# microsoft/GenerativeImage2Text

Hardware: AMD Instinct MI355X
Metric: captions/sec whole-node (GIT_BASE 224px bs=64/GPU greedy len=20) (higher is better)
Workload: dtype f16; 1 GPU; GIT_BASE 224px bs=64/GPU greedy max_len=20 frames=1; global_batch=64, parallelism=dp1, decode_steps_per_caption=19, seq_len_returned=20, hip_graph=True, contexts_in_flight=4, layernorm_folded=True, library=libgitmi_f16.so, encoder_chains=2, schedule=mixed

## Files before the change

### generativeimage2text_amd/csrc/abi_ops.hip

```cpp
#include "../../include/gitmi.h"
#include "abi_common.h"
#include "gitmi_common.h"
#include "launchers.h"

#include <hip/hip_runtime.h>

using namespace gitmi;

#ifdef GITMI_EXPERIMENT
#include "../../include/gitmi_experiment.h"
#define GITMI_EXP_EXPORT extern "C"
#else
#define GITMI_EXP_EXPORT [[maybe_unused]] static
#endif

static inline int round_up(int x, int m) { return (x + m - 1) / m * m; }

extern "C" int gitmi_operand_dtype(void);
static const char* dtype_name(int dtype) {
    return dtype == GITMI_DTYPE_F32 ? "fp32" : dtype == GITMI_DTYPE_BF16 ? "bf16" : dtype == GITMI_DTYPE_F16 ? "fp16" : "unknown";
}
static int check_dtype(const char* op, const char* arg, int dtype) {
    if (dtype == GITMI_DTYPE_F32 || dtype == gitmi_operand_dtype()) return 0;
    return fail("%s: %s is %s (%d), but this library's 16-bit operands are %s (libgitmi%s.so)", op, arg, dtype_name(dtype), dtype,
// ... 201 lines not shown

GITMI_EXP_EXPORT int gitmi_debug_gemm_form(const void* A, int lda, const void* W, const float* bias, const void* res, int ldr, void* C,
                                           int ldc, int M, int N, int K, int act, int in_dtype, int out_dtype, int shared,
                                           const float* ln_part, const float* colsum, float ln_eps, float* part_out,
                                           const float* res_part, const float* res_gamma, const float* res_beta, float res_eps,
                                           void* stream) {
    if (!A || !W || !C) return fail("debug_gemm_form: null argument (A, W, C)");
    if (M < 0 || N < 1 || K < 1) return fail("debug_gemm_form: M=%d N=%d K=%d", M, N, K);
    if (lda < K) return fail("debug_gemm_form: lda=%d < K=%d", lda, K);
    if (ldc < N) return fail("debug_gemm_form: ldc=%d < N=%d", ldc, N);
    if (res && ldr < N) return fail("debug_gemm_form: ldr=%d < N=%d", ldr, N);
    if (act < GITMI_ACT_NONE || act > GITMI_ACT_GELU_ERF) return fail("debug_gemm_form: act=%d", act);
    RCK(check_dtype("debug_gemm_form", "in_dtype", in_dtype));
    const bool in_f32 = in_dtype == GITMI_DTYPE_F32;
    if ((in_f32 && K % 16) || (!in_f32 && K % 64)) return fail("debug_gemm_form: K must be a multiple of %d (K=%d)", in_f32 ? 16 : 64, K);
    GemmArgs g{};
    g.A = A; g.W = W; g.bias = bias; g.res = (const float*)res; g.C = C;
    g.M = M; g.N = N; g.K = K; g.lda = lda; g.ldc = ldc; g.ldr = res ? ldr : 0; g.act = act;
    g.shared = shared ? 1 : 0;
    if (out_dtype == GITMI_DTYPE_F16_STREAM) {
        if (in_f32) return fail("debug_gemm_form: fp16 stream rows need 16-bit operands");
        g.out_f16 = 1;
    } else {
        RCK(check_dtype("debug_gemm_form", "out_dtype", out_dtype));
    }
    const bool out_f32 = out_dtype == GITMI_DTYPE_F32;
    const bool consumer = ln_part != nullptr, producer = part_out != nullptr || res_part != nullptr;
    if (colsum && !consumer) return fail("debug_gemm_form: colsum without ln_part");
    if ((res_gamma || res_beta) && !res_part) return fail("debug_gemm_form: res_gamma / res_beta without res_part");
    if (consumer || producer) {
#ifndef GITMI_OPS_F16
        return fail("debug_gemm_form: the folded-LayerNorm forms are built into the fp16-operand library only");
#endif
        if (consumer && producer) return fail("debug_gemm_form: consumer (ln_part) and producer (part_out / res_part) arguments in one launch");
        if (consumer) {
            if (!colsum) return fail("debug_gemm_form: ln_part without colsum");
            if (res || in_f32 || out_f32 || g.out_f16) return fail("debug_gemm_form: the consumer writes operand-type rows and takes no residual");
            if (K > 1024) return fail("debug_gemm_form: row partials cover K <= 1024 (K=%d)", K);
            g.ln_part = (const float2*)ln_part; g.ln_nparts = (K + 255) / 256; g.ln_colsum = colsum; g.ln_inv_d = 1.0f / (float)K; g.ln_eps = ln_eps;
        } else {
            if (!g.out_f16 || act != GITMI_ACT_NONE) return fail("debug_gemm_form: the producer writes fp16 stream rows and has no activation");
            if (N > 1024) return fail("debug_gemm_form: row partials cover N <= 1024 (N=%d)", N);
            g.part_out = (float2*)part_out;
            if (res_part) {
                if (!res || !res_gamma || !res_beta) return fail("debug_gemm_form: res_part without res / res_gamma / res_beta");
                g.res_part = (const float2*)res_part; g.res_nparts = (N + 255) / 256; g.res_gamma = res_gamma; g.res_beta = res_beta;
                g.res_inv_d = 1.0f / (float)N; g.res_eps = res_eps;
            }
        }
        if (!gemm_uses_p8(g, false, false))
            return fail("debug_gemm_form: the folded forms exist in gemm_p8_kernel only (more than 512 rows, N %% 256 == 0, K >= 128, 16-byte aligned rows)");
    }
    HIPCK(launch_gemm(g, in_f32, out_f32, (hipStream_t)stream));
    return 0;
}

extern "C" int gitmi_op_attn_decode(const void* qkv, const void* img_k, const void* img_v, void* txt_k, void* txt_v,
                                    const int* kv_src, void* out, int B, int H, int N_img, int T_max, int pos, int beams,
                                    int dtype, int dbg, void* stream) {
    RCK(check_dtype("op_attn_decode", "dtype", dtype));
    AttnDecodeArgs a{};
    a.qkv = qkv; a.img_k = img_k; a.img_v = img_v; a.txt_k = txt_k; a.txt_v = txt_v; a.out = out;
    a.kv_src = kv_src; a.ld_src = T_max; a.d = H * 64; a.N_img = N_img; a.T_max = T_max; a.pos = pos; a.beams = beams;
    a.scale = 0.125f; a.dbg = dbg & 0xffff; a.waves_per_pair = (dbg >> 16) & 3; a.stream_wgs = dbg >> 18;
    if (dtype == GITMI_DTYPE_F32) {
        HIPCK(launch_attn_decode(a, B, H, (hipStream_t)stream));
        return 0;
    }
    a.N_pad = round_up(N_img, 32);
    HIPCK(launch_attn_decode_mfma(a, B, H, (hipStream_t)stream));
    return 0;
}
extern "C" int gitmi_op_kv_repack(const void* qkv_rows, void* kf, void* vt, int B, int N, int H, void* stream) {
    HIPCK(launch_kv_repack_frag(qkv_rows, kf, vt, B, N, round_up(N, 32), H, H * 64, (hipStream_t)stream));
    return 0;
}

GITMI_EXP_EXPORT int gitmi_debug_attention_ragged(const void* qkv, void* out, const int* ntok, int B, int N, int H, int dtype, int impl,
                                                  void* stream) {
    if (!ntok) return fail("debug_attention_ragged: ntok is required");
    const size_t esz = dtype == GITMI_DTYPE_F32 ? 4 : 2;
    const int D = H * 64;
    AttnFullArgs a{};
    a.q = qkv;
    a.k = (const char*)qkv + (size_t)D * esz;
    a.v = (const char*)qkv + (size_t)2 * D * esz;
    a.out = out;
    a.ldq = a.ldk = a.ldv = 3 * D;
    a.ldo = D;
    a.N = N; a.H = H; a.scale = 0.125f; a.ntok = ntok;
    HIPCK(launch_attn_full(a, B, dtype == GITMI_DTYPE_F32, impl, (hipStream_t)stream));
    return 0;
}
GITMI_EXP_EXPORT int gitmi_debug_attn_decode_form(const void* qkv, const void* img_k, const void* img_v, void* txt_k, void* txt_v,
                                                  const int* kv_src, void* out, const int* ntok, const int* img_of, int n_images,
                                                  int B, int H, int N_img, int T_max, int pos, int beams, int dtype, int out_frag,
                                                  int pairs_per_wg, int waves_per_pair, int stream_wgs, void* stream) {
    RCK(check_dtype("debug_attn_decode_form", "dtype", dtype));
    if (!qkv || !img_k || !img_v || !txt_k || !txt_v || !kv_src || !out) return fail("debug_attn_decode_form: null argument");
    if (beams < 1 || beams > 8) return fail("debug_attn_decode_form: beams=%d outside [1, 8]", beams);
    if (n_images < 1) return fail("debug_attn_decode_form: n_images=%d", n_images);
    if (B < 1 || H < 1 || N_img < 1 || pos < 0 || pos >= T_max)
        return fail("debug_attn_decode_form: B=%d H=%d N_img=%d pos=%d T_max=%d", B, H, N_img, pos, T_max);
    if (out_frag && dtype == GITMI_DTYPE_F32) return fail("debug_attn_decode_form: out_frag needs 16-bit rows");
    if (ntok && stream_wgs > 0) return fail("debug_attn_decode_form: the streaming kernel does not serve ragged batches (ntok)");
    AttnDecodeArgs a{};
// ... 214 lines not shown
```

### generativeimage2text_amd/csrc/engine.hip

```cpp
#include "../../include/gitmi.h"
#include "engine_state.h"

#include <algorithm>
#include <cmath>
#include <cstdarg>
#include <cstdio>
#include <cstring>

using namespace gitmi;

#ifdef GITMI_EXPERIMENT
#include "../../include/gitmi_experiment.h"
#define GITMI_EXP_EXPORT extern "C"
#else
#define GITMI_EXP_EXPORT [[maybe_unused]] static
#endif

static thread_local char g_err[1024] = "";
int gitmi::fail(const char* fmt, ...) {
    va_list ap;
    va_start(ap, fmt);
    vsnprintf(g_err, sizeof(g_err), fmt, ap);
    va_end(ap);
    return 1;
// ... 10 lines not shown
struct SpanGuard {
    gitmi_engine* e; hipStream_t s; size_t idx; bool on;
    SpanGuard(gitmi_engine* e_, hipStream_t s_, int tag, double flops) : e(e_), s(s_), idx(0), on(e_->profiling) {
        if (!on) return;
        TimedSpan sp{get_event(e), get_event(e), tag, flops};
        hipEventRecord(sp.a, s);
        idx = e->spans.size();
        e->spans.push_back(sp);
    }
    ~SpanGuard() { if (on) hipEventRecord(e->spans[idx].b, s); }
};

static bool gemm_tall_tiles(const gitmi_engine* e, int N) {
    if (!e->pol.shared_device) return false;
    return e->pol.gemm_tall == 1 || (e->pol.gemm_tall == 2 && N >= 2048) || (e->pol.gemm_tall == 3 && N < 2048);
}

static double gemm_flops(int M, int N, int K) { return 2.0 * (double)M * (double)N * (double)K; }
static GemmArgs gemm_args(const void* A, int lda, const void* W, const float* bias, const void* res, int ldr, void* C, int ldc,
                          int M, int N, int K, int act) {
    GemmArgs g{};
    g.A = A; g.W = W; g.bias = bias; g.res = (const float*)res; g.C = C;
    g.M = M; g.N = N; g.K = K; g.lda = lda; g.ldc = ldc; g.ldr = ldr; g.act = act;
    return g;
}
static int gemm_run(gitmi_engine* e, hipStream_t s, GemmArgs g, bool in_f32, bool out_f32, int tag) {
    g.shared = gemm_tall_tiles(e, g.N) ? 1 : 0;
    SpanGuard sp(e, s, tag, gemm_flops(g.M, g.N, g.K));
    HIPCK(launch_gemm(g, in_f32, out_f32, s));
    return 0;
}
static int gemm(gitmi_engine* e, hipStream_t s, const void* A, int lda, const void* W, const float* bias,
                const float* res, int ldr, void* C, int ldc, bool out_f32, int M, int N, int K, int act, int tag) {
    return gemm_run(e, s, gemm_args(A, lda, W, bias, res, ldr, C, ldc, M, N, K, act), e->pol.f32, out_f32, tag);
}
static bool on_p8(const void* A, int lda, const void* W, const void* C, int ldc, int M, int N, int K, bool stream_out) {
    GemmArgs g = gemm_args(A, lda, W, nullptr, nullptr, 0, const_cast<void*>(C), ldc, M, N, K, 0);
    g.out_f16 = stream_out ? 1 : 0;
    return gemm_uses_p8(g, false, false);
}
struct Stream {
    void* x = nullptr; int M = 0, D = 0, tag = 0;
    bool fold = false;
    void* t = nullptr;
    float* xn = nullptr;
    float2* parts[2] = {nullptr, nullptr};
    const float2* part = nullptr; const float* gamma = nullptr; const float* beta = nullptr; float eps = 0.f;
};
static float2* stream_part_out(const Stream& st) { return st.part == st.parts[0] ? st.parts[1] : st.parts[0]; }
static void stream_written(Stream& st, const float2* part, const float* gamma, const float* beta, float eps) {
    st.part = part; st.gamma = gamma; st.beta = beta; st.eps = eps;
}
static int ln_gemm(gitmi_engine* e, hipStream_t s, const Stream& st, const Folded& f, const void* W, const float* bias, void* C,
                   int ldc, int col0, int N, int act) {
    const int D = st.D;
    const size_t woff = (size_t)col0 * D * e->pol.esz;
    C = (char*)C + (size_t)col0 * e->pol.esz;
    if (st.fold) {
        GemmArgs g = gemm_args(st.x, D, (const char*)f.w + woff, f.bias + col0, nullptr, 0, C, ldc, st.M, N, D, act);
        g.ln_part = st.part; g.ln_nparts = D / 256; g.ln_colsum = f.colsum + col0; g.ln_inv_d = 1.0f / (float)D; g.ln_eps = st.eps;
        return gemm_run(e, s, g, false, false, st.tag);
    }
    if (e->pol.stream_f16)
        HIPCK(launch_layernorm_s16(st.x, D, st.gamma, st.beta, st.eps, nullptr, st.t, D, false, st.xn, st.xn ? D : 0, st.M, D, 0, 0, 0, s));
    else
        HIPCK(launch_layernorm((const float*)st.x, D, st.gamma, st.beta, st.eps, nullptr, st.t, D, e->pol.f32, st.xn, st.xn ? D : 0, st.M,
                               D, 0, 0, 0, s));
    return gemm(e, s, st.t, D, (const char*)W + woff, bias + col0, nullptr, 0, C, ldc, e->pol.f32, st.M, N, D, act, st.tag);
}
static int gemm_to_stream(gitmi_engine* e, hipStream_t s, Stream& st, const void* A, int lda, const void* W, const float* bias, int K,
                          bool residual, const float* gamma, const float* beta, float eps) {
    const int D = st.D;
    float2* part = gamma ? stream_part_out(st) : nullptr;
    const void* res = !residual ? nullptr : st.xn && !st.fold ? st.xn : st.x;
    GemmArgs g = gemm_args(A, lda, W, bias, res, residual ? D : 0, st.x, D, st.M, D, K, 0);
    g.out_f16 = e->pol.stream_f16 ? 1 : 0;
    if (st.fold) {
        g.part_out = part;
        if (residual && st.xn) {
            g.res_part = st.part; g.res_nparts = D / 256; g.res_gamma = st.gamma; g.res_beta = st.beta;
            g.res_inv_d = 1.0f / (float)D; g.res_eps = st.eps;
        }
    }
    RCK(gemm_run(e, s, g, e->pol.f32, !e->pol.stream_f16, st.tag));
    stream_written(st, part, gamma, beta, eps);
    return 0;
}
static int attn_full_packed(gitmi_engine* e, const void* qkv, void* out, int width, int heads, int N, int batch, const int* ntok,
                            hipStream_t s) {
    AttnFullArgs a{};
    a.q = qkv;
    a.k = (const char*)qkv + (size_t)width * e->pol.esz;
    a.v = (const char*)qkv + (size_t)2 * width * e->pol.esz;
    a.out = out;
    a.ldq = a.ldk = a.ldv = 3 * width;
    a.ldo = width;
    a.N = N; a.H = heads; a.scale = 0.125f;
    a.ntok = ntok;
    HIPCK(launch_attn_full(a, batch, e->pol.f32, e->pol.attn_impl, s));
    return 0;
}
static int dec_layer_tail(gitmi_engine* e, hipStream_t s, const DecLayerW& L, const void* ctx, float* hf, void* ht, float* y, void* u,
                          int M) {
    const int d = e->cfg.dec_hidden, ffn = e->cfg.dec_ffn;
    RCK(gemm(e, s, ctx, d, L.wo, L.bo, hf, d, y, d, true, M, d, d, 0, TAG_GEMM_OTHER));
    HIPCK(launch_layernorm(y, d, L.lnag, L.lnab, 1e-12f, nullptr, ht, d, e->pol.f32, hf, d, M, d, 0, 0, 0, s));
    RCK(gemm(e, s, ht, d, L.w1, L.b1, nullptr, 0, u, ffn, e->pol.f32, M, ffn, d, 2, TAG_GEMM_OTHER));
    RCK(gemm(e, s, u, ffn, L.w2, L.b2, hf, d, y, d, true, M, d, ffn, 0, TAG_GEMM_OTHER));
    HIPCK(launch_layernorm(y, d, L.lnog, L.lnob, 1e-12f, nullptr, ht, d, e->pol.f32, hf, d, M, d, 0, 0, 0, s));
    return 0;
}

extern "C" int gitmi_abi_version(void) { return GITMI_ABI_VERSION; }
extern "C" int gitmi_operand_dtype(void) {
#ifdef GITMI_OPS_F16
    return GITMI_DTYPE_F16;
#else
    return GITMI_DTYPE_BF16;
#endif
}
extern "C" const char* gitmi_last_error(void) { return g_err; }

extern "C" int gitmi_create(const gitmi_config* cfg, int device, gitmi_engine** out) {
    if (!cfg || !out) return fail("gitmi_create: null argument");
    int ndev = 0;
    if (hipGetDeviceCount(&ndev) != hipSuccess || ndev <= 0)
        return fail("gitmi_create: no HIP device available (this engine has no CPU fallback)");
    if (device < 0 || device >= ndev) return fail("gitmi_create: device %d out of range (%d devices)", device, ndev);
    HIPCK(hipSetDevice(device));
    hipDeviceProp_t prop;
    HIPCK(hipGetDeviceProperties(&prop, device));
    if (strncmp(prop.gcnArchName, "gfx950", 6) != 0)
        return fail("gitmi_create: device %d is %s; this library is built for gfx950 (MI355X) only", device,
                    prop.gcnArchName);
    const gitmi_config& c = *cfg;
    if (c.vit_width % c.vit_heads || c.vit_width / c.vit_heads != 64) return fail("ViT head_dim must be 64");
    if (c.dec_hidden % c.dec_heads || c.dec_hidden / c.dec_heads != 64) return fail("decoder head_dim must be 64");
    if (c.image_size % c.patch) return fail("image_size must be a multiple of patch");
    if (c.max_image_pixels < 0 || c.max_image_tokens < 0) return fail("negative image capacity");
    if (c.vit_width > 1024 || c.dec_hidden > 1024) return fail("hidden sizes above 1024 are not supported");
    if (c.vit_width % 64 || c.dec_hidden % 64 || c.dec_ffn % 64) return fail("hidden sizes must be multiples of 64");
    if (c.max_batch < 1 || c.max_beams < 1 || c.max_beams > 8 || c.max_frames < 1 || c.max_text_len < 2)
        return fail("bad capacity (max_batch>=1, 1<=max_beams<=8, max_frames>=1, max_text_len>=2)");
    if (c.max_text_len > c.max_pos) return fail("max_text_len exceeds max_pos");
    if (c.precision != GITMI_PREC_BF16 && c.precision != GITMI_PREC_F32) return fail("bad precision");

    gitmi_engine* e = new gitmi_engine();
    e->cfg = c;
    e->device = device;
    e->pol.f32 = c.precision == GITMI_PREC_F32;
    e->pol.esz = e->pol.f32 ? 4 : 2;
    e->pol.attn_impl = e->pol.f32 ? 0 : 1;
    init_geometry(e);
    e->pol.stream_f16 = !e->pol.f32;
#ifdef GITMI_OPS_F16
    e->pol.ln_fold = !e->pol.f32 && c.vit_width % 256 == 0 && c.dec_hidden % 256 == 0;
#endif
#ifdef GITMI_EXPERIMENT
    if (const char* env = getenv("GITMI_ATTN_IMPL")) e->pol.attn_impl = e->pol.f32 ? 0 : atoi(env);
    if (const char* env = getenv("GITMI_GRAPH")) e->pol.use_graph = atoi(env) != 0;
    if (const char* env = getenv("GITMI_ATTN_DBG")) e->pol.attn_dbg = atoi(env);
    if (const char* env = getenv("GITMI_ATTN_PW")) e->pol.attn_pw = atoi(env);
    if (const char* env = getenv("GITMI_ATTN_NH")) e->pol.attn_nh = atoi(env);
    if (const char* env = getenv("GITMI_ATTN_STREAM")) e->pol.attn_stream = atoi(env);
    if (const char* env = getenv("GITMI_DECODE_SKIP")) e->pol.decode_skip = atoi(env);
    if (const char* env = getenv("GITMI_GEMM_TALL")) e->pol.gemm_tall = atoi(env);
    if (const char* env = getenv("GITMI_DGEMM_ROWS")) e->pol.dgemm_rows = atoi(env);
    if (const char* env = getenv("GITMI_DGEMM_STRIPS")) e->pol.dgemm_strips = atoi(env);
    if (const char* env = getenv("GITMI_DGEMM_NO_ROW_WALK")) e->pol.dgemm_no_row_walk = atoi(env);
    if (const char* env = getenv("GITMI_DGEMM_DBG")) e->pol.dgemm_dbg = atoi(env);
    if (const char* env = getenv("GITMI_VOCAB_WGS")) e->pol.vocab_wgs = atoi(env);
    if (const char* env = getenv("GITMI_SKINNY")) e->pol.skinny = atoi(env) != 0;
    if (const char* env = getenv("GITMI_STREAM_F16")) e->pol.stream_f16 = !e->pol.f32 && atoi(env) != 0;
    if (const char* env = getenv("GITMI_GEMM_IMPL")) set_gemm_impl(atoi(env));
#endif
    e->pol.ln_fold = e->pol.ln_fold && e->pol.stream_f16;
    e->pol.ln_fold_ready = e->pol.ln_fold;
    *out = e;
    return 0;
}

int CapturedGraph::capture(hipStream_t s, const std::function<int()>& fn) {
    reset();
    HIPCK(hipStreamBeginCapture(s, hipStreamCaptureModeThreadLocal));
    const int rc = fn();
    const hipError_t ce = hipStreamEndCapture(s, &graph);
    if (rc != 0 || ce != hipSuccess) reset();
    RCK(rc);
    HIPCK(ce);
    HIPCK(hipGraphInstantiate(&exec, graph, nullptr, nullptr, 0));
    return 0;
}
static void destroy_graph(gitmi_engine* e) {
    for (CapturedGraph* g : {&e->graph_full, &e->graph_decode, &e->graph_follow}) g->reset();
    e->full_slot.valid = e->follow_slot.valid = false;
}
static void drop_resident(gitmi_engine* e) { e->have_feats = e->have_prefill = false; }
static void set_resident(gitmi_engine* e, int B, int F_eff, int stride = 0) {
    e->cur_B = B; e->cur_F = F_eff; e->cur_Nimg = stride > 0 ? stride : F_eff * e->N;
    e->have_feats = true; e->have_prefill = false;
    e->keyed = e->ragged; e->has_context = false;
}
static void set_context(gitmi_engine* e) { e->keyed = e->has_context = true; }
static const int* key_counts(const gitmi_engine* e) { return e->keyed ? e->rg_ntok : nullptr; }
static void set_prefilled(gitmi_engine* e) { e->have_prefill = true; }
static int settle_residency(gitmi_engine* e, const Request& rq, int rc) {
    if (rc != 0 && rq.frames) drop_resident(e);
    return rc;
}

extern "C" void gitmi_destroy(gitmi_engine* e) {
    if (!e) return;
    hipSetDevice(e->device);
    hipDeviceSynchronize();
    if (e->enc_after) {
        auto& w = e->enc_after->enc_watchers;
        w.erase(std::remove(w.begin(), w.end(), e), w.end());
    }
    for (gitmi_engine* w : e->enc_watchers) w->enc_after = nullptr;
    destroy_graph(e);
    if (e->own_stream) hipStreamDestroy(e->own_stream);
    if (e->fence_in) hipEventDestroy(e->fence_in);
    if (e->fence_out) hipEventDestroy(e->fence_out);
    for (auto ev : e->gev)
        if (ev) hipEventDestroy(ev);
    if (e->enc_done) hipEventDestroy(e->enc_done);
    for (auto ev : e->event_pool) hipEventDestroy(ev);
    for (void* p : e->allocs) hipFree(p);
    for (void* p : e->sc_allocs) hipFree(p);
    hipFree(e->at_out); hipFree(e->at_stats); hipFree(e->ctx_tab);
    if (e->trie_off) hipFree(e->trie_off);
    if (e->trie_tok) hipFree(e->trie_tok);
    if (e->trie_child) hipFree(e->trie_child);
    delete e;
}

extern "C" int gitmi_set_image_shape(gitmi_engine* e, int H, int W, void* stream) {
    if (!e) return fail("null engine");
    if (!e->finalized) return fail("weights not finalized");
    const gitmi_config& c = e->cfg;
    if (H == 0 && W == 0) {
        if (!e->ragged) {
            e->ragged = true;
            e->H = e->W = e->gh = e->gw = 0;
            e->N = e->Nmax;
            drop_resident(e);
        }
        return 0;
    }
    if (H < c.patch || W < c.patch) return fail("image %dx%d is smaller than one %d-pixel patch", H, W, c.patch);
    const int gh = H / c.patch, gw = W / c.patch;
    if ((size_t)H * W > e->max_pixels)
        return fail("image %dx%d exceeds the max_image_pixels capacity (%zu)", H, W, e->max_pixels);
    if (gh * gw + 1 > e->Nmax)
        return fail("a %dx%d token grid exceeds the max_image_tokens capacity (%d)", gh, gw, e->Nmax);
    if (H == e->H && W == e->W && !e->ragged) return 0;
    e->ragged = false;
    HIPCK(hipSetDevice(e->device));
    if (gh == e->g_nat && gw == e->g_nat) {
        e->pos_cur = e->w.pos;
    } else {
        HIPCK(launch_pos_bicubic(e->w.pos, e->pos_var, e->g_nat, gh, gw, c.vit_width, (hipStream_t)stream));
        e->pos_cur = e->pos_var;
    }
    e->H = H; e->W = W; e->gh = gh; e->gw = gw; e->N = gh * gw + 1;
    drop_resident(e);
    return 0;
}

static Stream vit_stream(gitmi_engine* e, int M) {
    const int D = e->cfg.vit_width;
    const VitLayerW& L = e->w.vit[0];
    Stream st;
    st.x = e->v_x; st.M = M; st.D = D; st.tag = TAG_GEMM_VIT; st.t = e->v_h;
    st.fold = e->pol.ln_fold && on_p8(e->v_x, D, L.qkv_f.w, e->v_qkv, 3 * D, M, 3 * D, D, false) &&
              on_p8(e->v_x, D, L.ffn1_f.w, e->v_u, 4 * D, M, 4 * D, D, false) && on_p8(e->v_ctx, D, L.wo, e->v_x, D, M, D, D, true) &&
              on_p8(e->v_u, 4 * D, L.w2, e->v_x, D, M, D, 4 * D, true);
    if (st.fold) st.parts[0] = st.parts[1] = e->v_part;
    return st;
}
static Stream prefill_stream(gitmi_engine* e, int M) {
    const int d = e->cfg.dec_hidden, ffn = e->cfg.dec_ffn, D = e->cfg.vit_width;
    const DecLayerW& L = e->w.dec[0];
    Stream st;
    st.x = e->p_y; st.M = M; st.D = d; st.tag = TAG_GEMM_OTHER; st.t = e->p_ht; st.xn = e->p_hf;
    st.fold = e->pol.ln_fold && on_p8(e->feats, D, e->w.vp_w, e->p_y, d, M, d, D, true) &&
              on_p8(e->p_y, d, L.qkv_pf.w, e->img_kv[0], 3 * d, M, 3 * d, d, false) &&
              on_p8(e->p_y, d, L.qkv_pf.w, e->img_kv[0], 3 * d, M, 2 * d, d, false) &&
              (e->cfg.dec_layers < 2 || (on_p8(e->p_y, d, L.ffn1_pf.w, e->p_u, ffn, M, ffn, d, false) &&
                                         on_p8(e->p_ctx, d, L.wo, e->p_y, d, M, d, d, true) && on_p8(e->p_u, ffn, L.w2, e->p_y, d, M, d, ffn, true)));
    if (st.fold) { st.parts[0] = e->p_part[0]; st.parts[1] = e->p_part[1]; }
    return st;
}

static int encode_frames_impl(gitmi_engine* e, const float* const* frames, int F, int B, float* feats_out,
                              hipStream_t s, int stride = 0) {
    const gitmi_config& c = e->cfg;
    const int D = c.vit_width, N = e->N;
    const int F_eff = c.num_frames > 0 ? std::min(F, c.num_frames) : F;
    const int Nimg = stride > 0 ? stride : F_eff * N;
    drop_resident(e);
    SpanGuard phase(e, s, TAG_VIT, 0);
    const int BI = F_eff * B;
    const int M = BI * N;
    const int g2 = N - 1;
    const size_t slot = (size_t)3 * e->max_pixels;
    if (e->ragged)
        HIPCK(launch_im2col_ragged(e->frame_stage[0], slot, e->rg_meta, e->patches, e->pol.f32, B, N, c.patch, e->Kp, e->Kp_pad, s));
    else
    for (int fr = 0; fr < F_eff; ++fr)
        HIPCK(launch_im2col(frames[fr], (char*)e->patches + (size_t)fr * B * g2 * e->Kp_pad * e->pol.esz, e->pol.f32, B,
                            e->H, e->W, c.patch, e->Kp, e->Kp_pad, s));
    RCK(gemm(e, s, e->patches, e->Kp_pad, e->w.conv_w, nullptr, nullptr, 0, e->patch_out, D, true, BI * g2, D, e->Kp_pad, 0,
             TAG_GEMM_VIT));
    Stream x = vit_stream(e, M);
    float2* part = stream_part_out(x);
    if (e->ragged)
        HIPCK(launch_vit_assemble_ragged(e->patch_out, e->w.cls, e->w.pos, e->g_nat, e->rg_meta, e->w.lnpre_g, e->w.lnpre_b, 1e-5f, e->v_x,
                                         e->pol.stream_f16, BI, N, c.patch, D, part, s));
    else
    HIPCK(launch_vit_assemble_ln(e->patch_out, e->w.cls, e->pos_cur, e->w.lnpre_g, e->w.lnpre_b, 1e-5f, e->v_x, e->pol.stream_f16, BI, N, D,
                                 part, D / 256, s));
    stream_written(x, part, e->w.vit[0].ln1g, e->w.vit[0].ln1b, 1e-5f);
    for (int l = 0; l < c.vit_layers; ++l) {
        const VitLayerW& L = e->w.vit[l];
        const VitLayerW* Ln = l + 1 < c.vit_layers ? &e->w.vit[l + 1] : nullptr;
        RCK(ln_gemm(e, s, x, L.qkv_f, L.wqkv, L.bqkv, e->v_qkv, 3 * D, 0, 3 * D, 0));
        RCK(attn_full_packed(e, e->v_qkv, e->v_ctx, D, c.vit_heads, N, BI, e->ragged ? e->rg_ntok : nullptr, s));
        RCK(gemm_to_stream(e, s, x, e->v_ctx, D, L.wo, L.bo, D, true, L.ln2g, L.ln2b, 1e-5f));
        RCK(ln_gemm(e, s, x, L.ffn1_f, L.w1, L.b1, e->v_u, 4 * D, 0, 4 * D, 1));
        RCK(gemm_to_stream(e, s, x, e->v_u, 4 * D, L.w2, L.b2, 4 * D, true, Ln ? Ln->ln1g : nullptr, Ln ? Ln->ln1b : nullptr, 1e-5f));
    }
    for (int fr = 0; fr < F_eff; ++fr) {
        const float* te = (c.num_frames > 0 && e->pol.use_temb) ? e->w.temb[fr] : nullptr;
        if (e->pol.stream_f16) {
            const char* xs = (const char*)e->v_x + (size_t)fr * B * N * D * 2;
            HIPCK(launch_layernorm_s16(xs, D, e->w.lnpost_g, e->w.lnpost_b, 1e-5f, te, e->feats, D, false, nullptr, 0, B * N, D, N,
                                       Nimg, fr * N, s));
            if (feats_out)
                HIPCK(launch_layernorm_s16(xs, D, e->w.lnpost_g, e->w.lnpost_b, 1e-5f, te, feats_out, D, true, nullptr, 0, B * N, D,
                                           N, Nimg, fr * N, s));
        } else {
            HIPCK(launch_layernorm(e->v_x + (size_t)fr * B * N * D, D, e->w.lnpost_g, e->w.lnpost_b, 1e-5f, te, e->feats, D, e->pol.f32,
                                   feats_out, D, B * N, D, N, Nimg, fr * N, s));
        }
    }
    if (e->ragged) {
        HIPCK(launch_zero_pad_rows(e->feats, e->pol.f32, D, e->rg_ntok, B, N, s));
        if (feats_out) HIPCK(launch_zero_pad_rows(feats_out, true, D, e->rg_ntok, B, N, s));
    }

    set_resident(e, B, F_eff, stride);
    return 0;
}

static int kv_repack(gitmi_engine* e, int l, int B, int Nimg, hipStream_t s) {
    const gitmi_config& c = e->cfg;
    void* kh = e->img_kh[l];
    void* vh = e->img_vh[l];
    if (e->pol.f32) HIPCK(launch_kv_repack(e->img_kv[l], kh, vh, B, Nimg, c.dec_heads, c.dec_hidden, s));
    else HIPCK(launch_kv_repack_frag(e->img_kv[l], kh, vh, B, Nimg, round_up(Nimg, 32), c.dec_heads, c.dec_hidden, s));
    return 0;
}

static int prefill_impl(gitmi_engine* e, hipStream_t s) {
    const gitmi_config& c = e->cfg;
    const int d = c.dec_hidden, ffn = c.dec_ffn, D = c.vit_width;
    const int B = e->cur_B, Nimg = e->cur_Nimg, M = B * Nimg;
    e->have_prefill = false;
    SpanGuard phase(e, s, TAG_PREFILL, 0);
    Stream y = prefill_stream(e, M);
    RCK(gemm_to_stream(e, s, y, e->feats, D, e->w.vp_w, e->w.vp_b, D, false, e->w.vp_lng, e->w.vp_lnb, 1e-5f));
    for (int l = 0; l < c.dec_layers; ++l) {
        const DecLayerW& L = e->w.dec[l];
        const bool last = l + 1 == c.dec_layers;
        const int col0 = last ? d : 0;
        RCK(ln_gemm(e, s, y, L.qkv_pf, L.wqkv, L.bqkv, e->img_kv[l], 3 * d, col0, 3 * d - col0, 0));
        RCK(kv_repack(e, l, B, Nimg, s));
        if (last) break;
        RCK(attn_full_packed(e, e->img_kv[l], e->p_ctx, d, c.dec_heads, Nimg, B, key_counts(e), s));
        RCK(gemm_to_stream(e, s, y, e->p_ctx, d, L.wo, L.bo, d, true, L.lnag, L.lnab, 1e-12f));
        RCK(ln_gemm(e, s, y, L.ffn1_pf, L.w1, L.b1, e->p_u, ffn, 0, ffn, 2));
        RCK(gemm_to_stream(e, s, y, e->p_u, ffn, L.w2, L.b2, ffn, true, L.lnog, L.lnob, 1e-12f));
    }
    set_prefilled(e);
    return 0;
}

#ifdef GITMI_EXPERIMENT
#define GITMI_SKIPPED(e, bit) (((e)->pol.decode_skip & (bit)) != 0)
#else
#define GITMI_SKIPPED(e, bit) false
#endif
static int dgemm(gitmi_engine* e, hipStream_t s, const DGemmArgs& g_in) {
    DGemmArgs g = g_in;
    g.dbg = e->pol.dgemm_dbg;
    g.no_row_walk = e->pol.dgemm_no_row_walk >= 0 ? e->pol.dgemm_no_row_walk : e->pol.shared_device ? 0 : 1;
    g.strips_per_wg = e->pol.dgemm_strips >= 0 ? e->pol.dgemm_strips : e->pol.shared_device ? 2 : 1;
    g.rows_per_wg = e->pol.dgemm_rows > 0 ? e->pol.dgemm_rows : g.M > 64 ? 64 : e->pol.shared_device ? 32 : 16;
    SpanGuard sp(e, s, TAG_GEMM_OTHER, gemm_flops(g.M, g.N, g.K));
    HIPCK(launch_dgemm(g, s));
    return 0;
}

static DGemmArgs dgemm_ln(const void* A, const Folded& f, const DLn* ln, void* C, int c_frag, int act, int M, int N, int K) {
    return dgemm_ln(A, f.w, f.bias, f.colsum, ln, C, c_frag, act, M, N, K);
}

static int decode_layers_impl(gitmi_engine* e, const int* kv_src, int ld_ids, int pos, int R, int beams, hipStream_t s) {
    const gitmi_config& c = e->cfg;
    const int d = c.dec_hidden, ffn = c.dec_ffn;
    const int B = R / beams;
    const bool chain = e->pol.skinny && !e->pol.f32;
    for (int l = 0; l < c.dec_layers; ++l) {
        const DecLayerW& L = e->w.dec[l];
        const DecLayerW* Lp = l > 0 ? &e->w.dec[l - 1] : nullptr;
        const DLn ln_prev{e->stats_o, d / 16, 1.0f / (float)d, 1e-12f, Lp ? Lp->lnog : nullptr, Lp ? Lp->lnob : nullptr};
        const DLn ln_a{e->stats_a, d / 16, 1.0f / (float)d, 1e-12f, L.lnag, L.lnab};
        const DLn* ln_o = Lp ? &ln_prev : nullptr;
        if (chain) {
            if (!GITMI_SKIPPED(e, 2)) RCK(dgemm(e, s, dgemm_ln(l == 0 ? e->d_ht : e->xo_b, L.qkv_f, ln_o, e->d_qkv, 0, 0, R, 3 * d, d)));
        } else {
            RCK(gemm(e, s, e->d_ht, d, L.wqkv, L.bqkv, nullptr, 0, e->d_qkv, 3 * d, e->pol.f32, R, 3 * d, d, 0, TAG_GEMM_OTHER));
        }
        AttnDecodeArgs a{};
        a.qkv = e->d_qkv; a.img_k = e->img_kh[l]; a.img_v = e->img_vh[l]; a.txt_k = e->txt_k[l]; a.txt_v = e->txt_v[l]; a.out = e->d_ctx;
        a.kv_src = kv_src; a.ld_src = ld_ids; a.d = d; a.N_img = e->cur_Nimg; a.T_max = c.max_text_len;
        a.img_of = e->img_identity ? nullptr : e->img_of_dev;
        a.pos = pos; a.beams = beams; a.scale = 0.125f;
        a.out_frag = chain ? 1 : 0;
        a.N_pad = round_up(e->cur_Nimg, 32);
        a.dbg = e->pol.attn_dbg;
        a.waves_per_pair = e->pol.attn_nh;
        a.pairs_per_wg = e->pol.attn_pw > 0 ? e->pol.attn_pw : e->pol.shared_device ? 8 : 4;
        const bool stream_ok = !e->pol.shared_device && a.N_pad <= 8 * 32 && B * c.dec_heads >= 384 && e->pol.attn_nh != 2;
        a.stream_wgs = e->pol.attn_stream >= 0 ? e->pol.attn_stream : stream_ok ? 192 : 0;
        if (e->keyed) { a.ntok = e->rg_ntok; a.stream_wgs = 0; }
        if (e->pol.f32) HIPCK(launch_attn_decode(a, B, c.dec_heads, s));
// ... 329 lines not shown
    RCK(check_ready(e));
    if (!done_out) return fail("search_done_count: null argument");
    int h = 0;
    HIPCK(hipMemcpyAsync(&h, e->ss.info, sizeof(int), hipMemcpyDeviceToHost, (hipStream_t)stream));
    HIPCK(hipStreamSynchronize((hipStream_t)stream));
    *done_out = h;
    return 0;
}

extern "C" int gitmi_search_finish(gitmi_engine* e, int64_t* tokens_out, float* logprob_out, int32_t* info_out,
                                   void* stream) {
    RCK(check_ready(e));
    const SearchState& st = e->ss;
    HIPCK(launch_search_finish(st, e->ss_cur, e->ss_len, (long long*)tokens_out, logprob_out, info_out, nullptr,
                               (hipStream_t)stream));
    return 0;
}

GITMI_EXP_EXPORT int gitmi_debug_search_begin_prefixed(gitmi_engine* e, const gitmi_search* sp, int B, const int64_t* start_host,
                                                       int ld, const int32_t* plen_host, int vocab, void* stream) {
    if (!plen_host) return fail("debug_search_begin_prefixed: null prefix lengths");
    return search_begin_host(e, "debug_search_begin_prefixed", sp, B, start_host, ld, plen_host, vocab, stream);
}
GITMI_EXP_EXPORT int gitmi_debug_search_advance_lists(gitmi_engine* e, const float* part_val, const int* part_idx,
                                                      const float* part_lse, int nparts, int slots, int embed, void* stream) {
    RCK(check_ready(e));
    if (!part_val || !part_idx || !part_lse) return fail("debug_search_advance_lists: null argument");
    const SearchState& st = e->ss;
    if (st.B < 1 || st.T < 1) return fail("debug_search_advance_lists: no search has begun");
    if (st.sampled || e->trie_search) return fail("debug_search_advance_lists: the sampling and trie searches select from whole logit rows");
    if (nparts < 1 || nparts > 256) return fail("debug_search_advance_lists: nparts=%d outside [1,256]", nparts);
    if (slots != 1 && slots != 2 && slots != 4 && slots != 8 && slots != 16)
        return fail("debug_search_advance_lists: slots=%d is not one of 1, 2, 4, 8, 16", slots);
    if (slots < search_mtop(st)) return fail("debug_search_advance_lists: slots=%d, but the step reads %d candidates per row", slots, search_mtop(st));
    const StepCands cands{part_val, part_idx, (const float2*)part_lse, nparts, slots};
    return search_step_impl(e, cands, embed != 0, (hipStream_t)stream);
}
GITMI_EXP_EXPORT int gitmi_debug_read_hidden(gitmi_engine* e, int R, float* hf_out, void* ht_out, int* ht_frag, int* ht_dtype,
                                             void* stream) {
    RCK(check_ready(e));
    const gitmi_config& c = e->cfg;
    if (R < 1 || R > c.max_batch * c.max_beams) return fail("debug_read_hidden: R=%d outside the capacity", R);
    if (!hf_out || !ht_out || !ht_frag || !ht_dtype) return fail("debug_read_hidden: null argument");
    hipStream_t s = (hipStream_t)stream;
    const size_t D = (size_t)c.dec_hidden, Rp = (size_t)(R + 15) / 16 * 16;
    HIPCK(hipMemcpyAsync(hf_out, e->d_hf, (size_t)R * D * sizeof(float), hipMemcpyDefault, s));
    HIPCK(hipMemcpyAsync(ht_out, e->d_ht, Rp * D * e->pol.esz, hipMemcpyDefault, s));
    HIPCK(hipStreamSynchronize(s));
    *ht_frag = (e->pol.skinny && !e->pol.f32) ? 1 : 0;
    *ht_dtype = e->pol.f32 ? GITMI_DTYPE_F32 : gitmi_operand_dtype();
    return 0;
}

static int generate_encode(gitmi_engine* e, const Request& rq, hipStream_t s) {
    RCK(encode_frames_impl(e, rq.frames, rq.F, rq.B, nullptr, s));
    return prefill_impl(e, s);
}
static int images_ready(gitmi_engine* e, const Request& rq, hipStream_t s) {
    if (rq.frames) return generate_encode(e, rq, s);
    return e->have_prefill ? 0 : prefill_impl(e, s);
}

static int generate_decode(gitmi_engine* e, const Request& rq, hipStream_t s, bool allow_poll) {
    const gitmi_config& c = e->cfg;
    const gitmi_search* sp = rq.sp;
    RCK(search_begin_impl(e, rq, c.vocab, s));
    const int Q = rq.Q, minP = rq.minP, maxP = rq.maxP, T = sp->max_steps, k = sp->beam_size, R = Q * k;
    const SearchState& st = e->ss;
    const int M = search_mtop(st);
    const int suppress = sp->kind != GITMI_SEARCH_GENERATOR ? 1 : 0;
    {
        SpanGuard phase(e, s, TAG_DECODE, 0);
        RCK(embed_position(e, st.ids[0], T, 0, R, s));
        e->ss_len = 1;
        StepCands cands{e->part_val, e->part_idx, e->part_lse, 1, 1};
        while (e->ss_len < T) {
            const int cur_len = e->ss_len;
            SpanGuard step(e, s, TAG_STEP, 0);
            RCK(decode_layers_impl(e, st.kv_src[e->ss_cur], T, cur_len - 1, R, k, s));
            if (cur_len >= minP)
                RCK(decode_head_impl(e, st.ids[e->ss_cur], T, cur_len, R, k, suppress, M, nullptr, 0, s, &cands));
            RCK(search_step_impl(e, cands, true, s));
            if (allow_poll && e->ss_len > maxP && (e->ss_len - maxP) % 8 == 0 && e->ss_len < T) {
                int h[4];
                HIPCK(hipMemcpyAsync(h, st.info, sizeof(h), hipMemcpyDeviceToHost, s));
                HIPCK(hipStreamSynchronize(s));
                if (h[0] >= Q) break;
            }
        }
    }
    HIPCK(launch_search_finish(st, e->ss_cur, e->ss_len, rq.tokens, rq.logprob, rq.info, rq.sent, s));
    if (e->ragged)
        HIPCK(launch_ragged_report(e->rg_meta, e->img_identity ? nullptr : e->img_of_dev, Q, keep_best(*sp), rq.logprob, rq.info,
                                   nullptr, s));
    const double kv = (double)Q * c.dec_layers * 2.0 * ((double)e->cur_Nimg + k * 0.5 * (minP + T)) * c.dec_hidden * e->pol.esz;
    e->last_decode_step_bytes = e->w.dec_weight_bytes + kv;
    return 0;
}

static int generate_body(gitmi_engine* e, const Request& rq, hipStream_t s, bool allow_poll) {
    SpanGuard total(e, s, 99, 0);
    RCK(images_ready(e, rq, s));
    return generate_decode(e, rq, s, allow_poll);
}

static GraphKey graph_key_of(const gitmi_engine* e, const Request& rq, int F_eff) {
    const gitmi_search& sp = *rq.sp;
    const bool resident = rq.frames == nullptr;
    return {rq.B, rq.Q, F_eff, rq.minP, sp.kind, sp.beam_size, sp.per_node_beam_size, sp.max_steps, e->H, e->W,
            rq.prefixed ? 1 : 0, e->img_identity ? 1 : 0, e->pol.use_temb ? 1 : 0, resident ? 1 : 0,
            resident ? e->cur_Nimg : 0, resident && e->keyed ? 1 : 0, sp.length_penalty,
            sp.do_sample, sp.top_k, keep_best(sp), sp.top_p, sp.temperature, sp.repetition_penalty, sp.seed};
}
// ... 13 lines not shown
        else if (e->enc_done && !e->enc_watchers.empty()) HIPCK(hipEventRecord(e->enc_done, x));
    }
    if (dec) HIPCK(dec->launch(x));
    if (!timed) return 0;
    HIPCK(hipEventRecord(e->gev[2], x));
    HIPCK(hipStreamSynchronize(x));
    float a = 0, b = 0;
    if (enc) HIPCK(hipEventElapsedTime(&a, e->gev[0], e->gev[1]));
    HIPCK(hipEventElapsedTime(&b, e->gev[1], e->gev[2]));
    e->split_encode_ms += a; e->split_decode_ms += b; e->split_calls += 1; e->split_steps += rq.sp->max_steps - 1;
    return 0;
}

static int generate_graphed(gitmi_engine* e, const Request& rq, hipStream_t s) {
    const gitmi_config& c = e->cfg;
    const bool resident = rq.frames == nullptr;
    hipStream_t x = s ? s : e->own_stream;
    if (x != s) {
        HIPCK(hipEventRecord(e->fence_in, s));
        HIPCK(hipStreamWaitEvent(x, e->fence_in, 0));
    }
    const size_t frame_bytes = (size_t)rq.B * 3 * e->H * e->W * sizeof(float);
    const int F_eff = resident ? e->cur_F : c.num_frames > 0 ? std::min(rq.F, c.num_frames) : rq.F;
    if (!e->ragged && !resident)
    for (int f = 0; f < F_eff; ++f)
        HIPCK(hipMemcpyAsync(e->frame_stage[f], rq.frames[f], frame_bytes, hipMemcpyDeviceToDevice, x));
    Request own = rq;
    if (!resident) { own.frames = e->frame_stage.data(); own.F = F_eff; }
    own.tokens = e->out_tokens; own.logprob = e->out_lp; own.info = e->out_info; own.sent = e->out_sent;
    const GraphKey key = graph_key_of(e, rq, F_eff);
    const CapturedGraph *enc = nullptr, *dec = nullptr;
    if (resident) {
        RCK(images_ready(e, rq, x));
        if (!e->follow_slot.valid || !(key == e->follow_slot.key)) {
            e->follow_slot.valid = false;
            RCK(e->graph_follow.capture(x, [&] { return generate_decode(e, own, x, false); }));
            e->follow_slot = {key, true};
        }
        dec = &e->graph_follow;
    } else {
        const bool split = e->profile_mode == 2 || e->enc_after != nullptr || !e->enc_watchers.empty();
        if (!e->full_slot.valid || !(key == e->full_slot.key) || split != e->graph_is_split) {
            e->full_slot.valid = false;
            e->graph_decode.reset();
            if (!split) {
                RCK(e->graph_full.capture(x, [&] { return generate_body(e, own, x, false); }));
            } else {
                RCK(e->graph_full.capture(x, [&] { return generate_encode(e, own, x); }));
                RCK(e->graph_decode.capture(x, [&] { return generate_decode(e, own, x, false); }));
            }
            e->full_slot = {key, true}; e->graph_is_split = split;
        } else {
            set_resident(e, rq.B, F_eff);
            set_prefilled(e);
        }
        enc = &e->graph_full;
        if (split) dec = &e->graph_decode;
    }
    RCK(replay(e, rq, x, enc, dec));
    const size_t nout = (size_t)rq.Q * (size_t)keep_best(*rq.sp);
    HIPCK(hipMemcpyAsync(rq.tokens, e->out_tokens, nout * rq.sp->max_steps * sizeof(long long), hipMemcpyDefault, x));
    HIPCK(hipMemcpyAsync(rq.logprob, e->out_lp, nout * sizeof(float), hipMemcpyDefault, x));
    HIPCK(hipMemcpyAsync(rq.info, e->out_info, 4 * sizeof(int), hipMemcpyDefault, x));
    if (rq.sent != e->out_sent) HIPCK(hipMemcpyAsync(rq.sent, e->out_sent, (size_t)rq.Q * 2 * sizeof(int), hipMemcpyDefault, x));
    if (x != s) {
        HIPCK(hipEventRecord(e->fence_out, x));
        HIPCK(hipStreamWaitEvent(s, e->fence_out, 0));
    }
    return 0;
}

static int generate_run(gitmi_engine* e, const Request& rq, hipStream_t s) {
    const bool long_budget = rq.sp->max_steps - rq.minP > 32;
    const bool graph = e->pol.use_graph && !e->profiling && !long_budget;
    return settle_residency(e, rq, graph ? generate_graphed(e, rq, s) : generate_body(e, rq, s, long_budget && !e->profiling));
}

extern "C" int gitmi_generate(gitmi_engine* e, const float* const* frames, int F, int B, const int64_t* prefix, int P,
                              const gitmi_search* sp, int64_t* tokens_out, float* logprob_out, int32_t* info_out,
                              void* stream) {
    RCK(check_ready(e));
    const gitmi_config& c = e->cfg;
    if (sp && sp->kind == GITMI_SEARCH_SCORE) return fail("generate: GITMI_SEARCH_SCORE scores given sentences: call gitmi_generate_prefixed");
    if (sp && sp->kind == GITMI_SEARCH_ATTEND) return fail("generate: GITMI_SEARCH_ATTEND maps given sentences: call gitmi_generate_prefixed");
    if (sp && sp->kind == GITMI_SEARCH_CONTEXT) return fail("generate: GITMI_SEARCH_CONTEXT takes context segments: call gitmi_generate_prefixed");
    if (!frames) RCK(check_resident(e, "generate", B));
    if (!sp || !tokens_out || !logprob_out || !info_out) return fail("generate: null argument");
    if (frames) RCK(check_frames(e, "generate", frames, F, B));
    if (!prefix) P = 1;
    if (P < 1 || P > c.max_text_len) return fail("generate: prefix length %d outside [1,%d]", P, c.max_text_len);
    if (sp->max_steps < P || sp->max_steps > c.max_text_len) return fail("generate: max_steps %d outside [P,%d]", sp->max_steps, c.max_text_len);
    hipStream_t s = (hipStream_t)stream;
    if (frames) RCK(ragged_prepare(e, frames, F, B, s));
    RCK(fill_uniform_sentences(e, B, (const long long*)prefix, P, s));
    const Request rq{frames, F, B, B, P, P, false, sp, (long long*)tokens_out, logprob_out, info_out, e->out_sent};
    return generate_run(e, rq, s);
}

static void score_free(gitmi_engine* e) {
    for (void* p : e->sc_allocs) hipFree(p);
    e->sc_allocs.clear();
    e->sc_rows = 0;
}
static int score_alloc(gitmi_engine* e, size_t rows_needed) {
    const size_t rows = (size_t)round_up((int)rows_needed, 128);
    if (e->sc_rows >= rows) return 0;
    score_free(e);
// ... 23 lines not shown
    e->sc_rows = rows;
    return 0;
}

static int attend_alloc(gitmi_engine* e, size_t floats, size_t stat_rows) {
    if (e->at_floats < floats) {
        hipFree(e->at_out);
        e->at_out = nullptr; e->at_floats = 0;
        if (hipMalloc(&e->at_out, floats * sizeof(float)) != hipSuccess) {
            (void)hipGetLastError();
            return fail("attend: out of device memory for the %zu floats of the maps", floats);
        }
        e->at_floats = floats;
    }
    if (e->at_stat_rows < stat_rows) {
        hipFree(e->at_stats);
        e->at_stats = nullptr; e->at_stat_rows = 0;
        if (hipMalloc(&e->at_stats, stat_rows * sizeof(float2)) != hipSuccess) {
            (void)hipGetLastError();
            return fail("attend: out of device memory for the softmax statistics of %zu rows", stat_rows);
        }
        e->at_stat_rows = stat_rows;
    }
    return 0;
}
static int call_Nimg(const gitmi_engine* e, const float* const* frames, int F) {
    if (!frames) return e->cur_Nimg;
    return (e->cfg.num_frames > 0 ? std::min(F, (int)e->cfg.num_frames) : F) * e->N;
}

static int score_head_impl(gitmi_engine* e, int M, hipStream_t s, int* ntiles) {
    const gitmi_config& c = e->cfg;
    const int d = c.dec_hidden, V = c.vocab;
    *ntiles = 1;
    if (e->pol.f32) {
        const int chunk = round_up(c.max_batch * c.max_beams, 64);
        for (int r0 = 0; r0 < M; r0 += chunk) {
            const int rows = std::min(chunk, M - r0);
            RCK(gemm(e, s, (const float*)e->sc_ht + (size_t)r0 * d, d, e->w.out_w, e->w.out_b, nullptr, 0, e->logits, e->ldl, true, rows,
                     V, d, 0, TAG_GEMM_OTHER));
            HIPCK(launch_score_rowstats(e->logits, e->ldl, V, e->sc_tgt, r0, rows, e->sc_part, e->sc_zt, s));
        }
    } else {
        SpanGuard sp(e, s, TAG_GEMM_OTHER, gemm_flops(M, V, d));
        *ntiles = score_head_tiles(V);
        HIPCK(launch_score_head(e->sc_ht, d, e->w.out_w, e->w.out_b, e->sc_tgt, M, V, d, e->sc_part, e->sc_zt, s));
    }
    return 0;
}
static int text_pass_impl(gitmi_engine* e, const Request& rq, const long long* tokens, int ld, hipStream_t s) {
    const gitmi_config& c = e->cfg;
    const int d = c.dec_hidden, V = c.vocab, Q = rq.Q, L = c.dec_layers;
    const bool attend = rq.sp->kind == GITMI_SEARCH_ATTEND;
    RCK(images_ready(e, rq, s));
    const int Lp = round_up(rq.maxP, 16), M = Q * Lp;
    const int Nk = e->cur_Nimg, Kc = Nk + ld;
    void* const out = attend ? (void*)e->at_out : (void*)e->sc_out;
    const size_t out_bytes = attend ? (size_t)Q * ld * L * Kc * sizeof(float) : (size_t)Q * ld * sizeof(float2);
    auto zero_outputs = [&]() -> int {
        HIPCK(hipMemsetAsync(out, 0, out_bytes, s));
        HIPCK(hipMemsetAsync(e->sc_bad, 0, (size_t)Q * sizeof(int), s));
        return 0;
    };
    SpanGuard phase(e, s, TAG_DECODE, 0);
    if (attend) RCK(zero_outputs());
    HIPCK(launch_score_embed_ln(tokens, ld, Q, Lp, e->w.words_f, e->w.positions_f, e->w.emb_lng, e->w.emb_lnb, 1e-8f, e->sc_hf, e->sc_ht,
                                e->pol.f32, d, V, c.max_pos, s));
    const int* ntok = key_counts(e);
    for (int l = 0; l < L; ++l) {
        const DecLayerW& W = e->w.dec[l];
        RCK(gemm(e, s, e->sc_ht, d, W.wqkv, W.bqkv, nullptr, 0, e->sc_qkv, 3 * d, e->pol.f32, M, 3 * d, d, 0, TAG_GEMM_OTHER));
        HIPCK(launch_score_attn(e->sc_qkv, e->img_kv[l], e->sc_img, e->sc_ctx, Q, c.dec_heads, d, Nk, Lp, 0.125f, e->pol.f32, s, ntok,
                                attend ? e->at_stats : nullptr));
        if (attend)
            HIPCK(launch_score_attn_map(e->sc_qkv, e->img_kv[l], e->sc_img, ntok, e->at_stats, e->sc_lens, e->at_out + (size_t)l * Kc,
                                        (size_t)ld * L * Kc, (size_t)L * Kc, ld, Q, c.dec_heads, Nk, Lp, 0.125f, e->pol.f32, e->sc_bad, s));
        if (!attend || l + 1 < L) RCK(dec_layer_tail(e, s, W, e->sc_ctx, e->sc_hf, e->sc_ht, e->sc_y, e->sc_u, M));
    }
    if (int ntiles = 1; !attend) {
        HIPCK(launch_score_targets(tokens, ld, Lp, e->sc_lens, V, M, e->sc_tgt, s));
        RCK(score_head_impl(e, M, s, &ntiles));
        RCK(zero_outputs());
        HIPCK(launch_score_combine(e->sc_part, ntiles, e->sc_zt, e->sc_tgt, M, Lp, ld, V, e->sc_out, e->sc_bad, s));
    }
    if (e->ragged) HIPCK(launch_ragged_report(e->rg_meta, e->sc_img, Q, 0, nullptr, nullptr, e->sc_bad, s));
    HIPCK(launch_score_info(e->sc_bad, Q, ld, e->sc_info, s, attend ? Kc : 0, attend ? L : 0));
    HIPCK(hipMemcpyAsync(rq.logprob, out, out_bytes, hipMemcpyDefault, s));
    HIPCK(hipMemcpyAsync(rq.info, e->sc_info, 4 * sizeof(int), hipMemcpyDefault, s));
    return 0;
}

struct SentenceSpan { int minP, maxP; bool ident; };
static int read_sentences(gitmi_engine* e, const char* who, const int32_t* plen, const int32_t* image_of, int ld, int B, int Q,
                          int Qmax, const char* cap, SentenceSpan* span) {
    if (Q < 1 || Q > Qmax) return fail("%s: Q=%d sentences outside [1,%d] (%s)", who, Q, Qmax, cap);
    if (!image_of && Q != B) return fail("%s: without image_of, Q must equal B", who);
    *span = {1 << 30, 0, true};
    e->plen_host.assign(plen, plen + Q);
    e->img_of_host.resize(Q);
    for (int q = 0; q < Q; ++q) {
        const int p = plen[q];
        if (p < 1 || p > ld) return fail("%s: length %d of sentence %d outside [1,%d]", who, p, q, ld);
        span->minP = std::min(span->minP, p); span->maxP = std::max(span->maxP, p);
        const int im = image_of ? image_of[q] : q;
        if (im < 0 || im >= B) return fail("%s: sentence %d names image %d of %d", who, q, im, B);
        e->img_of_host[q] = im;
        span->ident = span->ident && im == q;
// ... 166 lines not shown
    e->pol.use_graph = on != 0;
    return 0;
}
extern "C" int gitmi_profile_read(gitmi_engine* e, gitmi_profile* out) {
    if (!e || !out) return fail("null argument");
    HIPCK(hipSetDevice(e->device));
    HIPCK(hipDeviceSynchronize());
    memset(out, 0, sizeof(*out));
    if (e->profile_mode == 2) {
        const double n = e->split_calls ? (double)e->split_calls : 1.0;
        out->vit_ms = (float)(e->split_encode_ms / n);
        out->decode_ms = (float)(e->split_decode_ms / n);
        out->total_ms = out->vit_ms + out->decode_ms;
        out->decode_steps = e->split_calls ? e->split_steps / e->split_calls : 0;
        out->decode_step_ms = e->split_steps ? (float)(e->split_decode_ms / e->split_steps) : 0.f;
        out->decode_step_bytes = e->last_decode_step_bytes;
        e->split_encode_ms = e->split_decode_ms = 0; e->split_calls = e->split_steps = 0;
        return 0;
    }
    double step_ms = 0;
    for (const TimedSpan& sp : e->spans) {
        float ms = 0;
        if (hipEventElapsedTime(&ms, sp.a, sp.b) != hipSuccess) continue;
        switch (sp.tag) {
            case TAG_VIT: out->vit_ms += ms; break;
            case TAG_PREFILL: out->prefill_ms += ms; break;
            case TAG_DECODE: out->decode_ms += ms; break;
            case 99: out->total_ms += ms; break;
            case TAG_STEP: step_ms += ms; out->decode_steps += 1; break;
            case TAG_GEMM_VIT:
                out->vit_gemm_ms += ms; out->vit_gemm_launches += 1; out->vit_gemm_flops += sp.flops;
            case TAG_GEMM_OTHER:
                out->gemm_ms += ms; out->gemm_launches += 1; out->gemm_flops += sp.flops;
                break;
            default: break;
        }
    }
    out->decode_step_ms = out->decode_steps ? (float)(step_ms / out->decode_steps) : 0.f;
    out->decode_step_bytes = e->last_decode_step_bytes;
    e->spans.clear();
    e->event_next = 0;
    return 0;
}

GITMI_EXP_EXPORT int gitmi_debug_import_stage(gitmi_engine* dst, gitmi_engine* src, int stage, void* stream) {
    RCK(check_ready(dst));
    if (!src || !src->finalized) return fail("debug_import_stage: bad source");
    if (stage != 1 && stage != 2) return fail("debug_import_stage: stage must be 1 or 2");
    const gitmi_config &a = dst->cfg, &b = src->cfg;
    if (a.vit_width != b.vit_width || a.dec_hidden != b.dec_hidden || a.dec_layers != b.dec_layers || a.dec_heads != b.dec_heads)
        return fail("debug_import_stage: the two contexts are different models");
    if (!src->have_feats || (stage == 2 && !src->have_prefill)) return fail("debug_import_stage: the source has not run that stage");
    if (src->has_context) return fail("debug_import_stage: the source's resident images carry context rows");
    if (src->cur_B > a.max_batch || src->cur_F > a.max_frames || src->N != dst->N) return fail("debug_import_stage: capacity / resolution mismatch");
    hipStream_t s = (hipStream_t)stream;
    const size_t M = (size_t)src->cur_B * src->cur_Nimg;
    HIPCK(launch_convert(src->feats, src->pol.f32, dst->feats, dst->pol.f32, M * a.vit_width, s));
    set_resident(dst, src->cur_B, src->cur_F);
    if (stage == 2) {
        for (int l = 0; l < a.dec_layers; ++l) {
            HIPCK(launch_convert(src->img_kv[l], src->pol.f32, dst->img_kv[l], dst->pol.f32, M * 3 * a.dec_hidden, s));
            RCK(kv_repack(dst, l, dst->cur_B, dst->cur_Nimg, s));
        }
        set_prefilled(dst);
    }
    return 0;
}
GITMI_EXP_EXPORT int gitmi_debug_head_from(gitmi_engine* dst, gitmi_engine* src, int R, float* logits_out, void* stream) {
    RCK(check_ready(dst));
    if (!src || !src->pol.f32 || !logits_out) return fail("debug_head_from: the source must be an fp32 context");
    if (dst->pol.f32 || !dst->pol.skinny) return fail("debug_head_from: the destination must run the bf16 decode chain");
    const gitmi_config& c = dst->cfg;
    if (c.dec_hidden != src->cfg.dec_hidden || c.vocab != src->cfg.vocab) return fail("debug_head_from: different models");
    if (R < 1 || R > c.max_batch * c.max_beams) return fail("debug_head_from: R outside the capacity");
    hipStream_t s = (hipStream_t)stream;
    HIPCK(launch_chain_input(src->d_y, dst->xo_b, dst->stats_o, R, c.dec_hidden, s));
    StepCands cands{};
    return decode_head_impl(dst, nullptr, c.max_text_len, 1, R, 1, 0, 1, logits_out, c.vocab, s, &cands);
}
```

### generativeimage2text_amd/csrc/engine_state.h

```cpp
#pragma once
#include "../../include/gitmi.h"
#include "abi_common.h"
#include "launchers.h"

#include <hip/hip_runtime.h>

#include <functional>
#include <map>
#include <string>
#include <tuple>
#include <vector>

static inline int round_up(int x, int m) { return (x + m - 1) / m * m; }
static inline int keep_best(const gitmi_search& sp) { return sp.num_keep_best > 1 ? sp.num_keep_best : 1; }

struct HostTensor {
    std::vector<float> data;
    std::vector<int64_t> shape;
    float amax = 0.f;
    size_t numel() const { size_t n = 1; for (auto s : shape) n *= (size_t)s; return n; }
};

struct Folded { void* w = nullptr; float* bias = nullptr; float* colsum = nullptr; };

// ... 34 lines not shown
    void reset() {
        if (exec) hipGraphExecDestroy(exec);
        if (graph) hipGraphDestroy(graph);
        exec = nullptr, graph = nullptr;
    }
    int capture(hipStream_t s, const std::function<int()>& fn);
    hipError_t launch(hipStream_t s) const { return hipGraphLaunch(exec, s); }
};

struct Request {
    const float* const* frames;
    int F, B, Q, minP, maxP;
    bool prefixed;
    const gitmi_search* sp;
    long long* tokens; float* logprob; int32_t* info;
    int32_t* sent;
};

struct ModelWeights {
    void* conv_w = nullptr;
    float *cls = nullptr, *pos = nullptr, *lnpre_g = nullptr, *lnpre_b = nullptr, *lnpost_g = nullptr, *lnpost_b = nullptr;
    std::vector<VitLayerW> vit;
    std::vector<float*> temb;
    void* vp_w = nullptr;
    float *vp_b = nullptr, *vp_lng = nullptr, *vp_lnb = nullptr;
    float *words_f = nullptr, *positions_f = nullptr, *emb_lng = nullptr, *emb_lnb = nullptr;
    std::vector<DecLayerW> dec;
    void* out_w = nullptr;
    float* out_b = nullptr;
    Folded out_f;
    double dec_weight_bytes = 0;
};

struct Policy {
    bool f32 = false;
    size_t esz = 2;
    int attn_impl = 1;
    bool stream_f16 = false;
    bool ln_fold = false;
    bool ln_fold_ready = false;
    bool skinny = true;
    bool use_graph = true;
    bool use_temb = true;
    bool shared_device = false;
    int attn_dbg = 0, dgemm_dbg = 0;
    int attn_pw = 0;
    int attn_nh = 0;
    int attn_stream = -1;
    int dgemm_no_row_walk = -1;
    int dgemm_strips = -1;
    int vocab_wgs = -1;
    int gemm_tall = 1;
    int dgemm_rows = 0;
    int decode_skip = 0;
};

struct gitmi_engine {
    gitmi_config cfg{};
    ModelWeights w;
    Policy pol;
    int device = 0;
    bool finalized = false;
    gitmi_engine* parent = nullptr;

    std::map<std::string, HostTensor> host_w;
    std::vector<void*> allocs;

    int N = 0, gh = 0, gw = 0, H = 0, W = 0, Kp = 0, Kp_pad = 0;
    int N_nat = 0, g_nat = 0, Nmax = 0;
    size_t max_pixels = 0;
    float* pos_var = nullptr;
    const float* pos_cur = nullptr;
    bool ragged = false;
    int4* rg_meta = nullptr;
    int* rg_ntok = nullptr;
    bool keyed = false;
    bool has_context = false;
    int* ctx_tab = nullptr;
    size_t ctx_tab_ints = 0;

    void *patches = nullptr, *v_h = nullptr, *v_qkv = nullptr, *v_ctx = nullptr, *v_u = nullptr;
    float *patch_out = nullptr, *v_x = nullptr;
    void* feats = nullptr;
    float *p_y = nullptr, *p_hf = nullptr;
    void *p_ht = nullptr, *p_ctx = nullptr, *p_u = nullptr;
    std::vector<void*> img_kv;
    std::vector<void*> img_kh, img_vh;
    float *d_y = nullptr, *d_hf = nullptr, *logits = nullptr;
    void *d_ht = nullptr, *d_qkv = nullptr, *d_ctx = nullptr, *d_u = nullptr;
    std::vector<void*> txt_k, txt_v;
    int ldl = 0;
    float *xa_f = nullptr, *xo_f = nullptr;
    void *xa_b = nullptr, *xo_b = nullptr;
    float2 *stats_a = nullptr, *stats_o = nullptr;
    float* part_val = nullptr; int* part_idx = nullptr; float2* part_lse = nullptr;
    int vocab_cols = 128, vocab_nparts = 1;
    gitmi::SearchState ss{};
    int ss_cur = 0, ss_len = 0;
    long long* start_dev = nullptr;
    int *plen_dev = nullptr, *img_of_dev = nullptr;
    bool img_identity = true;
    int *trie_off = nullptr, *trie_tok = nullptr, *trie_child = nullptr, *trie_cursor = nullptr;
    bool trie_search = false;
    gitmi_search sample{};
    std::vector<int> plen_host, img_of_host;

    int cur_B = 0, cur_F = 0, cur_Nimg = 0;
    bool have_feats = false, have_prefill = false;

    int profile_mode = 0;
    bool profiling = false;
    float2 *v_part = nullptr, *p_part[2] = {nullptr, nullptr};
    hipEvent_t gev[3] = {nullptr, nullptr, nullptr};
    gitmi_engine* enc_after = nullptr;
    std::vector<gitmi_engine*> enc_watchers;
    hipEvent_t enc_done = nullptr;
    double split_encode_ms = 0, split_decode_ms = 0;
    int split_calls = 0, split_steps = 0;
    std::vector<TimedSpan> spans;
    std::vector<hipEvent_t> event_pool;
    size_t event_next = 0;
    double last_decode_step_bytes = 0;

    CapturedGraph graph_full, graph_decode, graph_follow;
    GraphSlot full_slot, follow_slot;
    bool graph_is_split = false;
    std::vector<float*> frame_stage;
    long long* out_tokens = nullptr;
    float* out_lp = nullptr;
    int* out_info = nullptr;
    int* out_sent = nullptr;
    hipStream_t own_stream = nullptr;
    hipEvent_t fence_in = nullptr, fence_out = nullptr;

    size_t sc_rows = 0;
    std::vector<void*> sc_allocs;
    float *sc_hf = nullptr, *sc_y = nullptr, *sc_zt = nullptr;
    void *sc_ht = nullptr, *sc_qkv = nullptr, *sc_ctx = nullptr, *sc_u = nullptr;
    float4* sc_part = nullptr;
    int *sc_tgt = nullptr, *sc_lens = nullptr, *sc_img = nullptr, *sc_bad = nullptr, *sc_info = nullptr;
    float2* sc_out = nullptr;
    size_t at_floats = 0, at_stat_rows = 0;
    float* at_out = nullptr;
    float2* at_stats = nullptr;
};

namespace gitmi {
void init_geometry(gitmi_engine* e);
}
```

### generativeimage2text_amd/csrc/kernels_attn.hip

```cpp
#include "gitmi_common.h"
#include "launchers.h"
#include <type_traits>

namespace gitmi {

constexpr int HD = 64;

template <typename T>
__global__ __launch_bounds__(256) void attn_full_valu_kernel(AttnFullArgs a) {
    __shared__ float Ks[64][HD + 1];
    __shared__ float Vs[64][HD + 1];
    __shared__ float qs[16][HD];
    __shared__ float ps[16][64];

    const int tid = threadIdx.x, lane = tid & 63, wave = tid >> 6;
    const int h = blockIdx.y, b = blockIdx.z;
    const int q0 = blockIdx.x * 16;
    const T* Q = reinterpret_cast<const T*>(a.q);
    const T* K = reinterpret_cast<const T*>(a.k);
    const T* V = reinterpret_cast<const T*>(a.v);
    T* O = reinterpret_cast<T*>(a.out);
    const size_t base_row = (size_t)b * a.N;
    const int n = a.ntok ? a.ntok[b] : a.N;
    if (q0 >= n) {
// ... 149 lines not shown
                    const float p = fast_exp(s_acc[st_][r] - m_new);
                    s_acc[st_][r] = p;
                    psum += p;
                }
            psum += __shfl_xor(psum, 16, 64);
            psum += __shfl_xor(psum, 32, 64);
            l_run[t] = l_run[t] * alpha + psum;
            m_run[t] = m_new;
#pragma unroll
            for (int dt = 0; dt < 4; ++dt)
#pragma unroll
                for (int r = 0; r < 4; ++r) o_acc[t][dt][r] *= alpha;

#pragma unroll
            for (int hf = 0; hf < 2; ++hf) {
                bf16x8_t pf;
                {
                    union { bf16x8_t v; uint32_t u[4]; } pk;
                    pk.u[0] = pack2bf(s_acc[2 * hf][0], s_acc[2 * hf][1]);
                    pk.u[1] = pack2bf(s_acc[2 * hf][2], s_acc[2 * hf][3]);
                    pk.u[2] = pack2bf(s_acc[2 * hf + 1][0], s_acc[2 * hf + 1][1]);
                    pk.u[3] = pack2bf(s_acc[2 * hf + 1][2], s_acc[2 * hf + 1][3]);
                    pf = pk.v;
                }
#pragma unroll
                for (int dt = 0; dt < 4; ++dt) {
                    union { bf16x8_t v; uint2 h2[2]; } vf;
                    const bf16_t* vp = Vt + (dt * 16 + l15) * FA_LDV + hf * 32 + lg * 4;
                    vf.h2[0] = *reinterpret_cast<const uint2*>(vp);
                    vf.h2[1] = *reinterpret_cast<const uint2*>(vp + 16);
                    o_acc[t][dt] = mfma16(vf.v, pf, o_acc[t][dt]);
                }
            }
        }
    }

#pragma unroll
    for (int t = 0; t < QT; ++t) {
        const int qr = qbase + (t * 4 + wave) * 16 + l15;
        if (qr < a.N) {
            const float inv = qr < n ? 1.0f / l_run[t] : 0.f;
            bf16_t* op = O + (base_row + qr) * a.ldo + h * HD;
#pragma unroll
            for (int dt = 0; dt < 4; ++dt) {
                uint2 tt;
                tt.x = pack2bf(o_acc[t][dt][0] * inv, o_acc[t][dt][1] * inv);
                tt.y = pack2bf(o_acc[t][dt][2] * inv, o_acc[t][dt][3] * inv);
                *reinterpret_cast<uint2*>(op + dt * 16 + lg * 4) = tt;
            }
        }
    }
}

template <int NSUB, bool RAGGED = false>
__global__ __launch_bounds__(256, 2) void attn_full_mfma_short_kernel(AttnFullArgs a) {
    constexpr int NK = NSUB * 16;
    constexpr int NB = (NSUB + 1) / 2;
    constexpr int LDV = NB * 32 + 8;
    static_assert((LDV / 8) % 2 == 1, "V^T row stride must be an odd multiple of 16 bytes");
    __shared__ __attribute__((aligned(16))) bf16_t Ks[NK * FA_LDK];
    __shared__ __attribute__((aligned(16))) bf16_t Vt[HD * LDV];

    const int tid = threadIdx.x, lane = tid & 63, wave = tid >> 6;
    const int l15 = lane & 15, lg = lane >> 4;
    const int h = blockIdx.x, b = blockIdx.y;
    const bf16_t* Q = reinterpret_cast<const bf16_t*>(a.q);
    const bf16_t* K = reinterpret_cast<const bf16_t*>(a.k);
    const bf16_t* V = reinterpret_cast<const bf16_t*>(a.v);
    bf16_t* O = reinterpret_cast<bf16_t*>(a.out);
    const size_t base_row = (size_t)b * a.N;
    const int n = RAGGED ? a.ntok[b] : a.N;
    if constexpr (RAGGED) {
        for (int i = tid; i < (a.N - n) * 8; i += 256) {
            const int qr = n + (i >> 3);
            *reinterpret_cast<u32x4_t*>(O + (base_row + qr) * a.ldo + h * HD + (i & 7) * 8) = u32x4_t{0u, 0u, 0u, 0u};
        }
    }

#pragma unroll
    for (int it = 0; it < (NK * 8 + 255) / 256; ++it) {
        int idx = tid + it * 256;
        const bool ok = idx < NK * 8;
        idx = ok ? idx : NK * 8 - 1;
        const int key = idx >> 3, c = idx & 7;
        const int kr = key < n ? key : n - 1;
        const u32x4_t kc = *reinterpret_cast<const u32x4_t*>(K + (base_row + kr) * a.ldk + h * HD + c * 8);
        if (ok) *reinterpret_cast<u32x4_t*>(Ks + key * FA_LDK + c * 8) = kc;
    }
#pragma unroll
    for (int it = 0; it < (NB * 8 * 8 + 255) / 256; ++it) {
        int task = tid + it * 256;
        const bool ok = task < NB * 8 * 8;
        task = ok ? task : NB * 8 * 8 - 1;
        const int kg = task % (NB * 8), c = task / (NB * 8);
        u32x4_t vc[4];
#pragma unroll
        for (int e = 0; e < 4; ++e) {
            const int key = kg * 4 + e;
            const int kr = key < n ? key : n - 1;
            vc[e] = *reinterpret_cast<const u32x4_t*>(V + (base_row + kr) * a.ldv + h * HD + c * 8);
            if (key >= n) vc[e] = u32x4_t{0u, 0u, 0u, 0u};
        }
        if (ok) {
#pragma unroll
            for (int w = 0; w < 4; ++w) {
                uint2 even, odd;
                even.x = (vc[0][w] & 0xffffu) | (vc[1][w] << 16);
                even.y = (vc[2][w] & 0xffffu) | (vc[3][w] << 16);
                odd.x = (vc[0][w] >> 16) | (vc[1][w] & 0xffff0000u);
                odd.y = (vc[2][w] >> 16) | (vc[3][w] & 0xffff0000u);
                *reinterpret_cast<uint2*>(Vt + (c * 8 + 2 * w) * LDV + kg * 4) = even;
                *reinterpret_cast<uint2*>(Vt + (c * 8 + 2 * w + 1) * LDV + kg * 4) = odd;
            }
        }
    }
    __syncthreads();

    const int nqt = (n + 15) >> 4;
    const float c2 = a.scale * 1.4426950408889634f;

    auto process = [&](auto nt_c, int t0) {
        constexpr int NT = decltype(nt_c)::value;
        bf16x8_t qf[NT][2];
#pragma unroll
        for (int u = 0; u < NT; ++u) {
            int qr = (t0 + 4 * u) * 16 + l15;
            qr = qr < n ? qr : n - 1;
            const bf16_t* qp = Q + (base_row + qr) * a.ldq + h * HD + lg * 8;
            qf[u][0] = *reinterpret_cast<const bf16x8_t*>(qp);
            qf[u][1] = *reinterpret_cast<const bf16x8_t*>(qp + 32);
        }
        f32x4_t sacc[NT][NSUB];
#pragma unroll
        for (int st_ = 0; st_ < NSUB; ++st_) {
            const bf16x8_t kf0 = *reinterpret_cast<const bf16x8_t*>(Ks + (st_ * 16 + l15) * FA_LDK + lg * 8);
            const bf16x8_t kf1 = *reinterpret_cast<const bf16x8_t*>(Ks + (st_ * 16 + l15) * FA_LDK + 32 + lg * 8);
#pragma unroll
            for (int u = 0; u < NT; ++u) {
                sacc[u][st_] = mfma16(kf0, qf[u][0], f32x4_t{0.f, 0.f, 0.f, 0.f});
                sacc[u][st_] = mfma16(kf1, qf[u][1], sacc[u][st_]);
            }
            if constexpr (NSUB > 13) { if (st_ % 4 == 3) __builtin_amdgcn_sched_barrier(0); }
        }
        float inv_l[NT];
#pragma unroll
        for (int u = 0; u < NT; ++u) {
            if constexpr (RAGGED) {
#pragma unroll
                for (int st_ = 0; st_ < NSUB; ++st_)
#pragma unroll
                    for (int r = 0; r < 4; ++r)
                        if (st_ * 16 + lg * 4 + r >= n) sacc[u][st_][r] = -INFINITY;
            } else {
#pragma unroll
                for (int r = 0; r < 4; ++r)
                    if ((NSUB - 1) * 16 + lg * 4 + r >= a.N) sacc[u][NSUB - 1][r] = -INFINITY;
            }
            float m = -INFINITY;
#pragma unroll
            for (int st_ = 0; st_ < NSUB; ++st_)
#pragma unroll
                for (int r = 0; r < 4; ++r) m = fmaxf(m, sacc[u][st_][r]);
            m = fmaxf(m, __shfl_xor(m, 16, 64));
            m = fmaxf(m, __shfl_xor(m, 32, 64));
            const float mc = m * c2;
            float psum = 0.f;
#pragma unroll
            for (int st_ = 0; st_ < NSUB; ++st_)
#pragma unroll
                for (int r = 0; r < 4; ++r) {
                    const float p = __builtin_amdgcn_exp2f(sacc[u][st_][r] * c2 - mc);
                    sacc[u][st_][r] = p;
                    psum += p;
                }
            psum += __shfl_xor(psum, 16, 64);
            psum += __shfl_xor(psum, 32, 64);
            inv_l[u] = 1.0f / psum;
        }
        uint32_t pk2[NT][NSUB][2];
#pragma unroll
        for (int u = 0; u < NT; ++u)
#pragma unroll
            for (int st_ = 0; st_ < NSUB; ++st_) {
                pk2[u][st_][0] = pack2bf(sacc[u][st_][0], sacc[u][st_][1]);
                pk2[u][st_][1] = pack2bf(sacc[u][st_][2], sacc[u][st_][3]);
            }
        f32x4_t o_acc[NT][4];
#pragma unroll
        for (int u = 0; u < NT; ++u)
#pragma unroll
            for (int dt = 0; dt < 4; ++dt) o_acc[u][dt] = f32x4_t{0.f, 0.f, 0.f, 0.f};
#pragma unroll
        for (int blk = 0; blk < NB; ++blk) {
            bf16x8_t pf[NT];
#pragma unroll
            for (int u = 0; u < NT; ++u) {
                union { bf16x8_t v; uint32_t w[4]; } pk;
                pk.w[0] = pk2[u][2 * blk][0];
                pk.w[1] = pk2[u][2 * blk][1];
                const bool has1 = 2 * blk + 1 < NSUB;
                const int s1 = has1 ? 2 * blk + 1 : 0;
                pk.w[2] = has1 ? pk2[u][s1][0] : 0u;
                pk.w[3] = has1 ? pk2[u][s1][1] : 0u;
                pf[u] = pk.v;
            }
#pragma unroll
            for (int dt = 0; dt < 4; ++dt) {
                union { bf16x8_t v; uint2 h2[2]; } vf;
                const bf16_t* vp = Vt + (dt * 16 + l15) * LDV + blk * 32 + lg * 4;
                vf.h2[0] = *reinterpret_cast<const uint2*>(vp);
                vf.h2[1] = *reinterpret_cast<const uint2*>(vp + 16);
#pragma unroll
                for (int u = 0; u < NT; ++u)
                    o_acc[u][dt] = mfma16(vf.v, pf[u], o_acc[u][dt]);
            }
        }
#pragma unroll
        for (int u = 0; u < NT; ++u) {
            const int qr = (t0 + 4 * u) * 16 + l15;
            if (qr < n) {
                bf16_t* op = O + (base_row + qr) * a.ldo + h * HD;
#pragma unroll
                for (int dt = 0; dt < 4; ++dt) {
                    uint2 tt;
                    tt.x = pack2bf(o_acc[u][dt][0] * inv_l[u], o_acc[u][dt][1] * inv_l[u]);
                    tt.y = pack2bf(o_acc[u][dt][2] * inv_l[u], o_acc[u][dt][3] * inv_l[u]);
                    *reinterpret_cast<uint2*>(op + dt * 16 + lg * 4) = tt;
                }
            }
        }
    };

    for (int t0 = wave; t0 < nqt; t0 += 8) {
        if (t0 + 4 < nqt) process(std::integral_constant<int, 2>{}, t0);
        else process(std::integral_constant<int, 1>{}, t0);
    }
}

template <typename T>
__global__ void kv_repack_kernel(const T* __restrict__ qkv, T* __restrict__ kh, T* __restrict__ vh, int B, int N, int H,
                                 int d) {
    constexpr int CH = 16 / (int)sizeof(T);
    constexpr int CPH = HD / CH;
    const size_t per = (size_t)B * H * N * CPH;
    for (size_t i = blockIdx.x * (size_t)blockDim.x + threadIdx.x; i < 2 * per; i += (size_t)gridDim.x * blockDim.x) {
        const int kv = i >= per;
        size_t r = kv ? i - per : i;
        const int c = (int)(r % CPH); r /= CPH;
        const int n = (int)(r % N); r /= N;
        const int h = (int)(r % H);
        const int b = (int)(r / H);
        const T* src = qkv + ((size_t)b * N + n) * 3 * d + (kv ? 2 : 1) * d + h * HD + c * CH;
        T* dst = (kv ? vh : kh) + (((size_t)b * H + h) * N + n) * HD + c * CH;
        *reinterpret_cast<u32x4_t*>(dst) = *reinterpret_cast<const u32x4_t*>(src);
    }
}

template <typename T> struct Raw8;
template <> struct Raw8<bf16_t> {
    u32x4_t r;
    __device__ __forceinline__ void load(const bf16_t* p) { r = *reinterpret_cast<const u32x4_t*>(p); }
    __device__ __forceinline__ void load_nt(const bf16_t* p) { r = __builtin_nontemporal_load(reinterpret_cast<const u32x4_t*>(p)); }
    __device__ __forceinline__ void store(bf16_t* p) const { *reinterpret_cast<u32x4_t*>(p) = r; }
    __device__ __forceinline__ void zero() { r = u32x4_t{0u, 0u, 0u, 0u}; }
// ... 197 lines not shown
            const int srow = KB == 1 ? row0 : a.kv_src[(size_t)(row0 + j) * a.ld_src + sidx];
            ld8(TK + ((size_t)srow * a.T_max + sidx) * a.d + h * HD + sub * 8, kv);
            ld8(TV + ((size_t)srow * a.T_max + sidx) * a.d + h * HD + sub * 8, vv);
        }
        text_item(j, kv, vv);
    }

#pragma unroll
    for (int j = 0; j < KB; ++j) {
#pragma unroll
        for (int off = 8; off < 64; off <<= 1) {
            const float m2 = __shfl_xor(m[j], off, 64);
            const float l2 = __shfl_xor(l[j], off, 64);
            const float mn = fmaxf(m[j], m2);
            const float a1 = m[j] == -INFINITY ? 0.f : fast_exp(m[j] - mn);
            const float a2 = m2 == -INFINITY ? 0.f : fast_exp(m2 - mn);
            l[j] = l[j] * a1 + l2 * a2;
#pragma unroll
            for (int e = 0; e < 8; ++e) {
                const float o2 = __shfl_xor(o[j][e], off, 64);
                o[j][e] = o[j][e] * a1 + o2 * a2;
            }
            m[j] = mn;
        }
        if ((tid & 63) < 8 && j < k) {
#pragma unroll
            for (int e = 0; e < 8; ++e) part[wave][j][sub * 8 + e] = o[j][e];
            if (sub == 0) { part[wave][j][HD] = m[j]; part[wave][j][HD + 1] = l[j]; }
        }
    }
    __syncthreads();
    for (int i = tid; i < k * HD; i += 256) {
        const int j = i / HD, dd = i % HD;
        float mm = -INFINITY;
#pragma unroll
        for (int w = 0; w < 4; ++w) mm = fmaxf(mm, part[w][j][HD]);
        float num = 0.f, den = 0.f;
#pragma unroll
        for (int w = 0; w < 4; ++w) {
            const float mw = part[w][j][HD];
            const float aw = mw == -INFINITY ? 0.f : fast_exp(mw - mm);
            num += aw * part[w][j][dd];
            den += aw * part[w][j][HD + 1];
        }
        if constexpr (sizeof(T) == 2) {
            if (a.out_frag) { O[frag_offset(row0 + j, h * HD + dd, a.d >> 5)] = f2bf(num / den); continue; }
        }
        st<T>(O + (size_t)(row0 + j) * a.d + h * HD + dd, num / den);
    }
}

hipError_t launch_attn_full(const AttnFullArgs& a, int B, bool is_f32, int impl, hipStream_t s) {
    if (B <= 0 || a.N <= 0) return hipSuccess;
    if (impl == 1) {
        if (is_f32) return hipErrorInvalidValue;
        const int nsub = (a.N + 15) / 16;
        if (nsub == 13 && a.ntok) hipLaunchKernelGGL((attn_full_mfma_short_kernel<13, true>), dim3(a.H, B), dim3(256), 0, s, a);
        else if (nsub == 13) hipLaunchKernelGGL(attn_full_mfma_short_kernel<13>, dim3(a.H, B), dim3(256), 0, s, a);
        else if (nsub == 17 && a.ntok) hipLaunchKernelGGL((attn_full_mfma_short_kernel<17, true>), dim3(a.H, B), dim3(256), 0, s, a);
        else if (nsub == 17) hipLaunchKernelGGL(attn_full_mfma_short_kernel<17>, dim3(a.H, B), dim3(256), 0, s, a);
        else hipLaunchKernelGGL(attn_full_mfma_kernel, dim3((a.N + 255) / 256, a.H, B), dim3(256), 0, s, a);
    } else if (impl == 2) {
        if (is_f32) return hipErrorInvalidValue;
        hipLaunchKernelGGL(attn_full_mfma_kernel, dim3((a.N + 255) / 256, a.H, B), dim3(256), 0, s, a);
    } else if (is_f32) {
        hipLaunchKernelGGL(attn_full_valu_kernel<float>, dim3((a.N + 15) / 16, a.H, B), dim3(256), 0, s, a);
    } else {
        hipLaunchKernelGGL(attn_full_valu_kernel<bf16_t>, dim3((a.N + 15) / 16, a.H, B), dim3(256), 0, s, a);
    }
    return hipGetLastError();
}

hipError_t launch_kv_repack(const void* qkv, void* kh, void* vh, int B, int N, int H, int d, hipStream_t s) {
    if (B <= 0 || N <= 0) return hipSuccess;
    const size_t total = 2 * (size_t)B * H * N * 16;
    size_t grid = (total + 255) / 256;
    grid = grid > 8192 ? 8192 : grid;
    hipLaunchKernelGGL(kv_repack_kernel<float>, dim3((int)grid), dim3(256), 0, s, (const float*)qkv, (float*)kh, (float*)vh, B, N,
                       H, d);
    return hipGetLastError();
}

hipError_t launch_attn_decode(const AttnDecodeArgs& a, int B, int H, hipStream_t s) {
    if (B <= 0) return hipSuccess;
    if (a.beams > 8) return hipErrorInvalidValue;
    if (a.beams <= 1) hipLaunchKernelGGL((attn_decode_kernel<float, 1>), dim3(H, B), dim3(256), 0, s, a);
    else if (a.beams <= 2) hipLaunchKernelGGL((attn_decode_kernel<float, 2>), dim3(H, B), dim3(256), 0, s, a);
    else if (a.beams <= 4) hipLaunchKernelGGL((attn_decode_kernel<float, 4>), dim3(H, B), dim3(256), 0, s, a);
    else hipLaunchKernelGGL((attn_decode_kernel<float, 8>), dim3(H, B), dim3(256), 0, s, a);
    return hipGetLastError();
}

}
```

### generativeimage2text_amd/csrc/kernels_gemm10.hip

```cpp
#include "gitmi_common.h"
#include "launchers.h"
#include <type_traits>

namespace gitmi {

namespace {

constexpr int BN = 256, BK = 64;
constexpr int HALF_BYTES = 128 * BK * 2;
constexpr int BUF_BYTES = 4 * HALF_BYTES;
constexpr int LDS_BYTES = 2 * BUF_BYTES;
constexpr int SLOT_A0 = 0, SLOT_A1 = HALF_BYTES, SLOT_B0 = 2 * HALF_BYTES, SLOT_B1 = 3 * HALF_BYTES;

typedef __attribute__((address_space(3))) void lds_void_t;

#define P8_BARRIER()                           \
    do {                                       \
        __builtin_amdgcn_sched_barrier(0);     \
        __builtin_amdgcn_s_barrier();          \
        asm volatile("" ::: "memory");         \
        __builtin_amdgcn_sched_barrier(0);     \
    } while (0)

__device__ __forceinline__ float add_unfused(float a, float b) {
#pragma clang fp contract(off)
    return a + b;
}

__device__ __forceinline__ void half_wave_sum2_hi(float& a, float& b) {
    asm volatile(
        "s_nop 1\n\t"
        "v_add_f32_dpp %0, %0, %0 quad_perm:[1,0,3,2] row_mask:0xf bank_mask:0xf\n\t"
        "v_add_f32_dpp %1, %1, %1 quad_perm:[1,0,3,2] row_mask:0xf bank_mask:0xf\n\t"
        "s_nop 0\n\t"
        "v_add_f32_dpp %0, %0, %0 quad_perm:[2,3,0,1] row_mask:0xf bank_mask:0xf\n\t"
        "v_add_f32_dpp %1, %1, %1 quad_perm:[2,3,0,1] row_mask:0xf bank_mask:0xf\n\t"
        "s_nop 0\n\t"
        "v_add_f32_dpp %0, %0, %0 row_ror:4 row_mask:0xf bank_mask:0xf\n\t"
        "v_add_f32_dpp %1, %1, %1 row_ror:4 row_mask:0xf bank_mask:0xf\n\t"
        "s_nop 0\n\t"
        "v_add_f32_dpp %0, %0, %0 row_ror:8 row_mask:0xf bank_mask:0xf\n\t"
        "v_add_f32_dpp %1, %1, %1 row_ror:8 row_mask:0xf bank_mask:0xf\n\t"
        "s_nop 0\n\t"
        "v_add_f32_dpp %0, %0, %0 row_bcast:15 row_mask:0xa bank_mask:0xf\n\t"
        "v_add_f32_dpp %1, %1, %1 row_bcast:15 row_mask:0xa bank_mask:0xf\n\t"
        "s_nop 1"
        : "+v"(a), "+v"(b));
}

#define P8_LDS_BARRIER()                                   \
    do {                                                   \
        asm volatile("s_waitcnt lgkmcnt(0)" ::: "memory"); \
        __builtin_amdgcn_s_barrier();                      \
        asm volatile("" ::: "memory");                     \
    } while (0)

template <typename T> __device__ __forceinline__ uint32_t pack2o(float lo, float hi) {
    if constexpr (std::is_same<T, f16_t>::value) return pack2h(lo, hi);
    else return pack2bf(lo, hi);
}
template <typename T> __device__ __forceinline__ void unpack2o(uint32_t u, float& lo, float& hi) {
    if constexpr (std::is_same<T, f16_t>::value) unpack2h(u, lo, hi);
    else unpack2op(u, lo, hi);
}

template <int N> __device__ __forceinline__ void wait_vm() {
    if constexpr (N == 8) asm volatile("s_waitcnt vmcnt(8)" ::: "memory");
    else if constexpr (N == 4) asm volatile("s_waitcnt vmcnt(4)" ::: "memory");
    else if constexpr (N == 2) asm volatile("s_waitcnt vmcnt(2)" ::: "memory");
    else if constexpr (N == 0) asm volatile("s_waitcnt vmcnt(0)" ::: "memory");
}

template <typename TOut, int ACT, int DBG = 0, int MH = 128, int EPI = 1, int MH1 = MH, int LNF = 0>
__global__ __launch_bounds__(512) void gemm_p8_kernel(GemmArgs g) {
    static_assert(LNF == 0 || sizeof(TOut) == 2, "LayerNorm folding: 16-bit outputs only");
    static_assert(MH % 32 == 0 && MH1 % 32 == 0 && MH1 <= MH && MH <= 128, "half tiles: multiples of 32 rows, second <= first");
    constexpr int BM = MH + MH1, MI = MH / 32, MI1 = MH1 / 32;
    __shared__ __attribute__((aligned(16))) unsigned char smem[LDS_BYTES];

    const int tid = threadIdx.x;
    const int lane = tid & 63;
    const int wave = __builtin_amdgcn_readfirstlane(tid >> 6);
    const int grp = wave >> 2, wc = wave & 3;
    const int l15 = lane & 15, lg = lane >> 4;
    uint64_t ts[8];
    auto stamp = [&](int i) {
        if constexpr ((DBG & 16) != 0) {
            __builtin_amdgcn_sched_barrier(0);
            ts[2 * i] = __builtin_amdgcn_s_memtime();
            ts[2 * i + 1] = __builtin_amdgcn_s_memrealtime();
            __builtin_amdgcn_sched_barrier(0);
        }
    };
    auto stamps_out = [&]() {
        if constexpr ((DBG & 16) != 0) {
            if (tid == 0) {
                uint64_t* o = reinterpret_cast<uint64_t*>(const_cast<float*>(g.res)) + (size_t)blockIdx.x * 8;
#pragma unroll
                for (int i = 0; i < 8; ++i) o[i] = ts[i];
            }
        }
    };
    stamp(0);

    int tile_m, tile_n;
    {
        const int x = blockIdx.x & 7, idx = blockIdx.x >> 3;
        const int ng = g.ng, mg = 8 / ng;
        const int gn = x % ng, gm = x / ng;
        const int tiles_m = (g.M + BM - 1) / BM;
        const int n_lo = gn * g.tiles_n / ng, n_hi = (gn + 1) * g.tiles_n / ng;
        const int nn = n_hi - n_lo;
        const int tg = tiles_m * nn;
        const int lo_t = gm * tg / mg, hi_t = (gm + 1) * tg / mg;
        if (idx >= hi_t - lo_t) return;
        const int L = lo_t + idx;
        tile_m = L / nn;
        tile_n = n_lo + L % nn;
    }
    const int m0 = tile_m * BM, n0 = tile_n * BN;

    const char* __restrict__ Ab = reinterpret_cast<const char*>(g.A);
    const char* __restrict__ Wb = reinterpret_cast<const char*>(g.W);

    const int Rl = lane >> 4, hi = (lane >> 3) & 1, lo = lane & 7;
    uint32_t a_off[2][2], w_off[2][2];
#pragma unroll
    for (int h = 0; h < 2; ++h)
// ... 185 lines not shown
            for (int j = 0; j < 2; ++j)
                cs4[qn][j] = *reinterpret_cast<const f32x4_t*>(g.ln_colsum + n0 + qn * 128 + wc * 32 + j * 16 + lg * 4);
    }
    auto ln_apply = [&](float a, int qm, int qn, int j, int i, int r) -> float {
        if constexpr (LNF == 1) return lrstd[qm][i] * fmaf(-lmean[qm][i], cs4[qn][j][r], a);
        else return a;
    };

    if constexpr (sizeof(TOut) == 4 && EPI == 1) {
        float* Cf = reinterpret_cast<float*>(g.C);
        const float* R = g.res;
        const int col0 = n0 + wc * 32 + lg * 4;
        const bool has_res = R != nullptr && !(DBG & 1);
#pragma unroll
        for (int qm = 0; qm < 2; ++qm) {
            const int MIq = qm ? MI1 : MI, MHq = qm ? MH1 : MH;
            f32x4_t rr[MI][2][2];
            if (has_res) {
#pragma unroll
                for (int i = 0; i < MIq; ++i) {
                    const int m = m0 + qm * MH + grp * (MHq / 2) + i * 16 + l15;
                    const int mc = m < g.M ? m : g.M - 1;
                    const float* rp = R + (size_t)mc * g.ldr + col0;
#pragma unroll
                    for (int qn = 0; qn < 2; ++qn)
#pragma unroll
                        for (int j = 0; j < 2; ++j)
                            rr[i][qn][j] = *reinterpret_cast<const f32x4_t*>(rp + qn * 128 + j * 16);
                }
            }
#pragma unroll
            for (int i = 0; i < MIq; ++i) {
                const int m = m0 + qm * MH + grp * (MHq / 2) + i * 16 + l15;
                float* cp = Cf + (size_t)m * g.ldc + col0;
                const bool ok = m < g.M && !(DBG & 1);
#pragma unroll
                for (int qn = 0; qn < 2; ++qn)
#pragma unroll
                    for (int j = 0; j < 2; ++j) {
                        f32x4_t v;
#pragma unroll
                        for (int r = 0; r < 4; ++r) v[r] = apply_act_t<ACT>(acc[qm][qn][j][i][r] + bias4[qn][j][r]);
                        if (has_res) {
#pragma unroll
                            for (int r = 0; r < 4; ++r) v[r] = add_unfused(v[r], rr[i][qn][j][r]);
                        }
                        if (ok) *reinterpret_cast<f32x4_t*>(cp + qn * 128 + j * 16) = v;
                    }
            }
        }
        return;
    }

    float rgm[8], rbt[8];
    if constexpr (LNF == 2) {
        if (g.res_part) {
            ld8(g.res_gamma + n0 + (tid & 31) * 8, rgm);
            ld8(g.res_beta + n0 + (tid & 31) * 8, rbt);
        }
    }
#pragma unroll
    for (int qm = 0; qm < 2; ++qm)
#pragma unroll
        for (int s = 0; s < 2 / NQN; ++s) {
            const int MIq = qm ? MI1 : MI, MHq = qm ? MH1 : MH;
#pragma unroll
            for (int u = 0; u < NQN; ++u) {
                const int qn = s * NQN + u;
#pragma unroll
                for (int j = 0; j < 2; ++j) {
                    const int nl = u * 128 + wc * 32 + j * 16 + lg * 4;
#pragma unroll
                    for (int i = 0; i < MIq; ++i) {
                        float v[4];
#pragma unroll
                        for (int r = 0; r < 4; ++r) v[r] = apply_act_t<ACT>(ln_apply(acc[qm][qn][j][i][r], qm, qn, j, i, r) + bias4[qn][j][r]);
                        TOut* p = ep + (grp * (MHq / 2) + i * 16 + l15) * EPS + nl;
                        if constexpr (sizeof(TOut) == 4) {
                            *reinterpret_cast<f32x4_t*>(p) = f32x4_t{v[0], v[1], v[2], v[3]};
                        } else {
                            uint2 t2;
                            t2.x = pack2o<TOut>(v[0], v[1]);
                            t2.y = pack2o<TOut>(v[2], v[3]);
                            *reinterpret_cast<uint2*>(p) = t2;
                        }
                    }
                }
            }
            P8_LDS_BARRIER();
#pragma unroll 4
            for (int q = 0; q < MHq * CPR / 512; ++q) {
                const int chunk = tid + q * 512;
                const int row = chunk / CPR, cc = chunk % CPR;
                const int m = m0 + qm * MH + row;
                const int n = n0 + s * WCOL + cc * EPC;
                if (m < g.M && !(DBG & 1)) {
                    if constexpr (sizeof(TOut) == 4) {
                        f32x4_t v = *reinterpret_cast<const f32x4_t*>(ep + row * EPS + cc * EPC);
                        if (g.res && !(DBG & 16)) {
                            const f32x4_t rr = *reinterpret_cast<const f32x4_t*>(g.res + (size_t)m * g.ldr + n);
                            v[0] += rr[0]; v[1] += rr[1]; v[2] += rr[2]; v[3] += rr[3];
                        }
                        *reinterpret_cast<f32x4_t*>(C + (size_t)m * g.ldc + n) = v;
                    } else if constexpr (LNF == 2) {
                    } else {
                        u32x4_t v = *reinterpret_cast<const u32x4_t*>(ep + row * EPS + cc * EPC);
                        if (g.res && !(DBG & 16)) {
                            float f[8], rs[8];
#pragma unroll
                            for (int e = 0; e < 4; ++e) unpack2o<TOut>(v[e], f[2 * e], f[2 * e + 1]);
                            if constexpr (std::is_same<TOut, f16_t>::value) {
                                const u32x4_t rr = *reinterpret_cast<const u32x4_t*>(reinterpret_cast<const f16_t*>(g.res) + (size_t)m * g.ldr + n);
#pragma unroll
                                for (int e = 0; e < 4; ++e) unpack2h(rr[e], rs[2 * e], rs[2 * e + 1]);
                            } else {
                                const float* rp = g.res + (size_t)m * g.ldr + n;
                                const f32x4_t r0 = *reinterpret_cast<const f32x4_t*>(rp);
                                const f32x4_t r1 = *reinterpret_cast<const f32x4_t*>(rp + 4);
#pragma unroll
                                for (int e = 0; e < 4; ++e) { rs[e] = r0[e]; rs[4 + e] = r1[e]; }
                            }
#pragma unroll
                            for (int e = 0; e < 8; ++e) f[e] += rs[e];
#pragma unroll
                            for (int e = 0; e < 4; ++e) v[e] = pack2o<TOut>(f[2 * e], f[2 * e + 1]);
                        }
                        TOut* cp = C + (size_t)m * g.ldc + n;
                        if (g.dbg & 512)
                            *reinterpret_cast<u32x4_t*>(cp) = v;
                        else
                            asm volatile("global_store_dwordx4 %0, %1, off sc1\n\ts_nop 1" ::"v"(cp), "v"(v) : "memory");
                    }
                }
                if constexpr (LNF == 2) {
                    static_assert(LNF != 2 || CPR == 32, "one stream row per half wave");
                    const bool ok = m < g.M;
                    const int mc = ok ? m : g.M - 1;
                    u32x4_t v = *reinterpret_cast<const u32x4_t*>(ep + row * EPS + cc * EPC);
                    float f[8];
#pragma unroll
                    for (int e = 0; e < 4; ++e) unpack2h(v[e], f[2 * e], f[2 * e + 1]);
                    if (g.res) {
                        float rs[8];
                        const u32x4_t rr = *reinterpret_cast<const u32x4_t*>(reinterpret_cast<const f16_t*>(g.res) + (size_t)mc * g.ldr + n);
#pragma unroll
                        for (int e = 0; e < 4; ++e) unpack2h(rr[e], rs[2 * e], rs[2 * e + 1]);
                        if (g.res_part) {
                            const f32x4_t* pp = reinterpret_cast<const f32x4_t*>(g.res_part + (size_t)mc * 4);
                            const f32x4_t p0 = pp[0], p1 = pp[1];
                            const float mean = ((p0[0] + p0[2]) + (p1[0] + p1[2])) * g.res_inv_d;
                            const float rstd = rsqrtf(fmaxf(((p0[1] + p0[3]) + (p1[1] + p1[3])) * g.res_inv_d - mean * mean, 0.f) + g.res_eps);
#pragma unroll
                            for (int e = 0; e < 8; ++e) rs[e] = fmaf((rs[e] - mean) * rstd, rgm[e], rbt[e]);
                        }
#pragma unroll
                        for (int e = 0; e < 8; ++e) f[e] += rs[e];
#pragma unroll
                        for (int e = 0; e < 4; ++e) v[e] = pack2h(f[2 * e], f[2 * e + 1]);
                    }
                    if (g.part_out) {
                        typedef __attribute__((ext_vector_type(2))) float f32x2_t;
                        f32x2_t s2 = {0.f, 0.f}, q2 = {0.f, 0.f};
#pragma unroll
                        for (int e = 0; e < 4; ++e) {
                            float x0, x1;
                            unpack2h(v[e], x0, x1);
                            const f32x2_t x = {x0, x1};
                            s2 += x;
                            q2 = __builtin_elementwise_fma(x, x, q2);
                        }
                        float sx = s2[0] + s2[1], sq = q2[0] + q2[1];
                        half_wave_sum2_hi(sx, sq);
                        if (ok && cc == 16 && !(DBG & 1)) g.part_out[(size_t)m * 4 + tile_n] = float2{sx, sq};
                    }
                    if (ok && !(DBG & 1)) {
                        TOut* cp = C + (size_t)m * g.ldc + n;
                        asm volatile("global_store_dwordx4 %0, %1, off sc1\n\ts_nop 1" ::"v"(cp), "v"(v) : "memory");
                    }
                }
            }
            P8_LDS_BARRIER();
        }
    if constexpr ((DBG & 16) != 0) {
        asm volatile("s_waitcnt vmcnt(0)" ::: "memory");
        stamp(3);
        stamps_out();
    }
}

}

template <typename TOut, int MH, int EPI = 1, int MH1 = MH, int LNF = 0>
static void launch_p8_t(const GemmArgs& g, hipStream_t s) {
    if constexpr (LNF == 2) {
        hipLaunchKernelGGL((gemm_p8_kernel<TOut, GITMI_ACT_NONE, 0, MH, EPI, MH1, LNF>), dim3(g.nwg), dim3(512), 0, s, g);
        return;
    } else {
    if (g.dbg && LNF == 0) {
        if constexpr (MH == 128 && MH1 == 128) {
            switch (g.dbg) {
                case 1: hipLaunchKernelGGL((gemm_p8_kernel<TOut, 0, 1>), dim3(g.nwg), dim3(512), 0, s, g); return;
                case 2: hipLaunchKernelGGL((gemm_p8_kernel<TOut, 0, 2>), dim3(g.nwg), dim3(512), 0, s, g); return;
                case 6: hipLaunchKernelGGL((gemm_p8_kernel<TOut, 0, 6>), dim3(g.nwg), dim3(512), 0, s, g); return;
                case 10: hipLaunchKernelGGL((gemm_p8_kernel<TOut, 0, 10>), dim3(g.nwg), dim3(512), 0, s, g); return;
#ifdef GITMI_PROBE
                case 16: hipLaunchKernelGGL((gemm_p8_kernel<TOut, 0, 16>), dim3(g.nwg), dim3(512), 0, s, g); return;
                case 17: hipLaunchKernelGGL((gemm_p8_kernel<TOut, 0, 17>), dim3(g.nwg), dim3(512), 0, s, g); return;
                case 18: hipLaunchKernelGGL((gemm_p8_kernel<TOut, 0, 18>), dim3(g.nwg), dim3(512), 0, s, g); return;
                case 22: hipLaunchKernelGGL((gemm_p8_kernel<TOut, 0, 22>), dim3(g.nwg), dim3(512), 0, s, g); return;
                case 26: hipLaunchKernelGGL((gemm_p8_kernel<TOut, 0, 26>), dim3(g.nwg), dim3(512), 0, s, g); return;
#endif
                default: break;
            }
        }
    }
    switch (g.act) {
        case GITMI_ACT_QUICKGELU:
            hipLaunchKernelGGL((gemm_p8_kernel<TOut, GITMI_ACT_QUICKGELU, 0, MH, EPI, MH1, LNF>), dim3(g.nwg), dim3(512), 0, s, g); break;
        case GITMI_ACT_GELU_ERF:
            hipLaunchKernelGGL((gemm_p8_kernel<TOut, GITMI_ACT_GELU_ERF, 0, MH, EPI, MH1, LNF>), dim3(g.nwg), dim3(512), 0, s, g); break;
        default:
            hipLaunchKernelGGL((gemm_p8_kernel<TOut, GITMI_ACT_NONE, 0, MH, EPI, MH1, LNF>), dim3(g.nwg), dim3(512), 0, s, g); break;
    }
    }
}

bool gemm_p8_supports(const GemmArgs& g) {
    return g.K % BK == 0 && g.K >= 2 * BK && g.N % BN == 0 &&
           (double)g.M * g.lda * 2.0 < 4.0e9 && (double)g.N * g.K * 2.0 < 4.0e9;
}

static int p8_xcd_count(const GemmArgs& g, int bm, int ng, int* max_nn_out) {
    const int tiles_m = (g.M + bm - 1) / bm, tiles_n = g.N / BN, mg = 8 / ng;
    int max_cnt = 0, max_nn = 0;
    for (int x = 0; x < 8; ++x) {
        const int gn = x % ng, gm = x / ng;
        const int nn = (gn + 1) * tiles_n / ng - gn * tiles_n / ng;
        const int tg = tiles_m * nn;
        const int cnt = (gm + 1) * tg / mg - gm * tg / mg;
        max_cnt = cnt > max_cnt ? cnt : max_cnt;
        max_nn = nn > max_nn ? nn : max_nn;
    }
    if (max_nn_out) *max_nn_out = max_nn;
    return max_cnt;
}
static int p8_plan(const GemmArgs& g, int bm, int* ng_out, int* max_cnt_out) {
    const int tiles_n = g.N / BN;
    int best_ng = 1, best_rounds = 1 << 30, best_cnt = 0, best_panels = 1 << 30;
    for (int ng = 1; ng <= 8 && ng <= tiles_n; ng *= 2) {
        int max_nn = 0;
        const int max_cnt = p8_xcd_count(g, bm, ng, &max_nn);
        const int rounds = (max_cnt + 31) / 32;
        const int panels = (32 + max_nn - 1) / max_nn + (max_nn < 32 ? max_nn : 32);
        if (rounds < best_rounds || (rounds == best_rounds && panels < best_panels)) {
            best_ng = ng; best_rounds = rounds; best_cnt = max_cnt; best_panels = panels;
        }
    }
    if (ng_out) *ng_out = best_ng;
    if (max_cnt_out) *max_cnt_out = best_cnt;
    return best_rounds;
}

int gemm_p8_cost(const GemmArgs& g, int bm) {
    const int rounds = p8_plan(g, bm, nullptr, nullptr);
    const int ktile = 1450 * (90 + 166 * bm / 256) / 256;
    return rounds * (1450 + (g.K / BK) * ktile + 4700 * bm / 256);
}

template <int MH, int MH1>
static void launch_p8_height(const GemmArgs& g, bool out_f32, bool staged, hipStream_t s) {
#ifdef GITMI_OPS_F16
    if (g.ln_part) { launch_p8_t<bf16_t, MH, 1, MH1, 1>(g, s); return; }
    if (g.part_out || g.res_part) { launch_p8_t<f16_t, MH, 1, MH1, 2>(g, s); return; }
#endif
    if (g.out_f16) launch_p8_t<f16_t, MH, 1, MH1>(g, s);
    else if (!out_f32) launch_p8_t<bf16_t, MH, 1, MH1>(g, s);
    else if (staged) launch_p8_t<float, MH, 0, MH1>(g, s);
    else launch_p8_t<float, MH, 1, MH1>(g, s);
}

hipError_t launch_gemm_p8(GemmArgs g, bool out_f32, hipStream_t s) {
    if (g.ln_part || g.part_out || g.res_part) {
#ifndef GITMI_OPS_F16
        return hipErrorInvalidValue;
#endif
        if (g.ln_part && (out_f32 || g.out_f16 || g.res || !g.ln_colsum || g.ln_nparts < 1 || g.part_out || g.res_part)) return hipErrorInvalidValue;
        if ((g.part_out || g.res_part) && (!g.out_f16 || out_f32 || g.act != 0 || g.N > 1024)) return hipErrorInvalidValue;
        if (g.res_part && (!g.res || !g.res_gamma || !g.res_beta || g.res_nparts < 1)) return hipErrorInvalidValue;
    }
    static const int heights[5] = {256, 224, 192, 160, 128};
    int bm = 256;
    if (!g.shared) {
        int best = gemm_p8_cost(g, 256);
        for (int h = 1; h < 5; ++h) {
            const int c = gemm_p8_cost(g, heights[h]);
            if (c < best) { best = c; bm = heights[h]; }
        }
    }
    if (g.dbg & 64) bm = 192;
    if (g.dbg & 128) bm = 256;
    if (g.dbg & 16384) bm = 160;
    if (g.dbg & 32768) bm = 224;
    if (g.dbg & 65536) bm = 128;
    g.dbg &= ~(64 | 128 | 16384 | 32768 | 65536);
    g.tiles_n = g.N / BN;
    int max_cnt = 0;
    p8_plan(g, bm, &g.ng, &max_cnt);
    if (g.dbg & (1024 | 2048 | 4096 | 8192)) {
        const int ng = (g.dbg & 1024) ? 1 : (g.dbg & 2048) ? 2 : (g.dbg & 4096) ? 4 : 8;
        g.dbg &= ~(1024 | 2048 | 4096 | 8192);
        if (ng <= g.tiles_n) { g.ng = ng; max_cnt = p8_xcd_count(g, bm, ng, nullptr); }
    }
    g.nwg = 8 * max_cnt;
    const bool staged = (g.dbg & 256) != 0;
    g.dbg &= ~256;
    switch (bm) {
        case 224: launch_p8_height<128, 96>(g, out_f32, staged, s); break;
        case 192: launch_p8_height<96, 96>(g, out_f32, staged, s); break;
        case 160: launch_p8_height<96, 64>(g, out_f32, staged, s); break;
        case 128: launch_p8_height<64, 64>(g, out_f32, staged, s); break;
        default: launch_p8_height<128, 128>(g, out_f32, staged, s); break;
    }
    return hipGetLastError();
}

}
```

### generativeimage2text_amd/csrc/launchers.h

```cpp
#pragma once
#include <hip/hip_runtime.h>
#include <stddef.h>

namespace gitmi {

struct GemmArgs {
    const void* A; const void* W; const float* bias; const float* res; void* C;
    int M, N, K;
    int lda, ldc, ldr;
    int act;
    int tiles_n, nwg;
    int ng;
    int dbg;
    int out_f16;
    int shared;
    const float2* ln_part; int ln_nparts; const float* ln_colsum; float ln_inv_d, ln_eps;
    float2* part_out;
    const float2* res_part; int res_nparts; const float* res_gamma; const float* res_beta; float res_inv_d, res_eps;
};
bool gemm_uses_p8(const GemmArgs& g, bool in_f32, bool out_f32);
hipError_t launch_gemm(const GemmArgs& g, bool in_f32, bool out_f32, hipStream_t s);
hipError_t launch_gemm_p8(GemmArgs g, bool out_f32, hipStream_t s);
bool gemm_p8_supports(const GemmArgs& g);
int gemm_p8_cost(const GemmArgs& g, int bm);
bool set_gemm_impl(int impl);

struct DGemmArgs {
    const unsigned short* A; const unsigned short* W;
    const float* bias;
    const float* colsum;
    const float2* stats_in;
    int strips_in; float inv_d, eps_in;
    void* C;
    int c_frag;
    const float* res_x;
    const float2* res_stats; int res_strips; const float* res_gamma; const float* res_beta; float res_inv_d, res_eps;
    float* x_out; unsigned short* xb_out; float2* stats_out;
    int M, N, K, lda, ldc, act;
    int dbg;
    int rows_per_wg;
    int strips_per_wg;
    int no_row_walk;
};
hipError_t launch_dgemm(const DGemmArgs& g, hipStream_t s);
struct DLn { const float2* stats; int strips; float inv_d, eps; const float* gamma; const float* beta; };
inline DGemmArgs dgemm_ln(const void* A, const void* W, const float* bias, const float* colsum, const DLn* ln, void* C, int c_frag,
                          int act, int M, int N, int K) {
    DGemmArgs g{};
    g.A = (const unsigned short*)A; g.lda = K; g.W = (const unsigned short*)W; g.bias = bias;
    if (ln) { g.colsum = colsum; g.stats_in = ln->stats; g.strips_in = ln->strips; g.inv_d = ln->inv_d; g.eps_in = ln->eps; }
    g.C = C; g.ldc = N; g.c_frag = c_frag; g.act = act; g.M = M; g.N = N; g.K = K;
    return g;
}
inline DGemmArgs dgemm_to_stream(const void* A, const void* W, const float* bias, const float* res_x, const DLn* res_ln, float* x_out,
                                 void* xb_out, float2* stats_out, int M, int N, int K) {
    DGemmArgs g{};
    g.A = (const unsigned short*)A; g.lda = K; g.W = (const unsigned short*)W; g.bias = bias; g.res_x = res_x;
    if (res_ln) {
        g.res_stats = res_ln->stats; g.res_strips = res_ln->strips; g.res_gamma = res_ln->gamma; g.res_beta = res_ln->beta;
        g.res_inv_d = res_ln->inv_d; g.res_eps = res_ln->eps;
    }
    g.x_out = x_out; g.xb_out = (unsigned short*)xb_out; g.stats_out = stats_out; g.M = M; g.N = N; g.K = K;
    return g;
}

struct VocabArgs {
    const unsigned short* A; int lda; const unsigned short* W; const float* bias; const float* colsum;
    const float2* stats_in; int strips_in; float inv_d, eps_in;
    int M, N, K, cols_per_wg;
    const int* ids; int ld_ids, cur_len; const int* plen; int beams, suppress_kind;
    float rep_penalty;
    float* part_val; int* part_idx; float2* part_lse;
    float* logits_out; int ld_logits;
    int max_wgs;
    int nblk;
};
hipError_t launch_vocab_topm(const VocabArgs& g, int mtop, hipStream_t s);
int vocab_parts(int V, int cols_per_wg);
int vocab_mtop_slots(int mtop);

hipError_t launch_layernorm(const float* x, int ldx, const float* gamma, const float* beta, float eps,
                            const float* add_after, void* y_t, int ld_t, bool t_is_f32, float* y_f, int ld_f,
                            int rows, int D, int map_n_in, int map_n_out, int map_off, hipStream_t s);
hipError_t launch_im2col(const float* img, void* out, bool out_f32, int B, int H, int W, int p, int K, int Kpad,
                         hipStream_t s);
hipError_t launch_pos_bicubic(const float* pos, float* out, int g, int gh, int gw, int D, hipStream_t s);
hipError_t launch_ragged_stage(const float* src, float* dst, size_t slot, int4* meta, int* ntok, int B, int p, size_t max_pixels,
                               int Nmax, hipStream_t s);
hipError_t launch_im2col_ragged(const float* stage, size_t slot, const int4* meta, void* out, bool out_f32, int B, int Nmax,
                                int p, int K, int Kpad, hipStream_t s);
hipError_t launch_vit_assemble_ragged(const float* patch_out, const float* cls, const float* pos, int g, const int4* meta,
                                      const float* gamma, const float* beta, float eps, void* X, bool x_f16, int B, int Nmax,
                                      int p, int D, float2* part, hipStream_t s);
hipError_t launch_zero_pad_rows(void* x, bool is_f32, int ld, const int* ntok, int B, int Nmax, hipStream_t s);
hipError_t launch_ragged_report(const int4* meta, const int* image_of, int Q, int nout_per, float* logprob, int* info,
                                int* bad, hipStream_t s);
hipError_t launch_vit_assemble_ln(const float* patch_out, const float* cls, const float* pos, const float* gamma,
                                  const float* beta, float eps, void* X, bool x_f16, int B, int N, int D, float2* part,
                                  int nparts, hipStream_t s);
hipError_t launch_layernorm_s16(const void* x, int ldx, const float* gamma, const float* beta, float eps,
                                const float* add_after, void* y_t, int ld_t, bool t_is_f32, void* y_s, int ld_s,
                                int rows, int D, int map_n_in, int map_n_out, int map_off, hipStream_t s);
hipError_t launch_embed_ln(const int* ids, int ld_ids, int pos, const float* words, const float* positions,
                           const float* gamma, const float* beta, float eps, float* h_f, void* h_t, bool t_is_f32,
                           int R, int D, int vocab, bool frag, hipStream_t s);
hipError_t launch_context_embed(const long long* tokens, int ld, const int4* seg, int Q, const int* cnt, const float* words,
                                const float* positions, const float* gamma, const float* beta, float eps, void* feats, bool t_is_f32,
                                float* feats_f, int* ntok, int B, int n_img, int stride, int D, int vocab, int max_pos, hipStream_t s);
hipError_t launch_frag_pack(const void* src_bf16, void* dst_bf16, int rows, int rows_out, int K, hipStream_t s);
hipError_t launch_convert_pad(const float* src, void* dst, bool dst_f32, size_t rows, int K, int Kpad,
                              hipStream_t s);
hipError_t launch_convert(const void* src, bool src_f32, void* dst, bool dst_f32, size_t n, hipStream_t s);
hipError_t launch_chain_input(const float* x, void* xb_frag, float2* stats, int R, int d, hipStream_t s);
hipError_t launch_copy_f32(const float* src, int lds, float* dst, int ldd, int rows, int cols, hipStream_t s);
hipError_t launch_fill_i32(int* dst, int value, int n, hipStream_t s);

struct AttnFullArgs {
    const void* q; const void* k; const void* v; void* out;
    int ldq, ldk, ldv, ldo;
    int N, H;
    float scale;
    const int* ntok;
};
hipError_t launch_attn_full(const AttnFullArgs& a, int B, bool is_f32, int impl, hipStream_t s);

struct AttnDecodeArgs {
    const void* qkv; const void* img_k; const void* img_v; void* txt_k; void* txt_v; void* out;
    const int* kv_src;
    const int* img_of;
    int ld_src;
    int d;
    int N_img, T_max, pos, beams;
    int N_pad;
    int out_frag;
    float scale;
    int dbg;
    int pairs_per_wg;
    int stream_wgs;
    int waves_per_pair;
    int n_pairs;
    const int* ntok;
};
hipError_t launch_kv_repack(const void* qkv, void* kh, void* vh, int B, int N, int H, int d, hipStream_t s);
hipError_t launch_attn_decode(const AttnDecodeArgs& a, int B, int H, hipStream_t s);
hipError_t launch_kv_repack_frag(const void* qkv, void* kf, void* vt, int B, int N, int N_pad, int H, int d, hipStream_t s);
hipError_t launch_attn_decode_mfma(const AttnDecodeArgs& a, int B, int H, hipStream_t s);

constexpr int SS_NHMAX = 8;
struct SearchState {
    int B, k, pn, T, V, eos, kind;
    int prefixed;
    int sampled;
    double length_penalty;
    double* len_norm;
    const long long* start;
    int ld_start;
    const int* plen;
    int* ids[2];
    int* kv_src[2];
    float* score[2];
    int* done;
    int nh;
    int* hyp_n;
    int* hyp_cnt;
    double* hyp_worst;
    double* hyp_score;
    int* hyp_len;
    int* hyp_seq;
    int* hyp_tok;
    int* stop;
    int* early;
    int* info;
};
struct StepCands {
    const float* part_val; const int* part_idx; const float2* part_lse;
// ... 61 lines not shown
```

### generativeimage2text_amd/engine.py

```python
from __future__ import annotations

import ctypes as C
import os
from typing import Dict, List, Mapping, Optional, Sequence, Tuple

import torch

_HERE = os.path.dirname(os.path.abspath(__file__))
LIB_PATH = os.path.join(_HERE, "libgitmi.so")
LIB_PATH_F16 = os.path.join(_HERE, "libgitmi_f16.so")
LIB_PATH_EXP = os.path.join(_HERE, "libgitmi_exp.so")
LIB_PATH_F16_EXP = os.path.join(_HERE, "libgitmi_f16_exp.so")

PREC_BF16, PREC_F32 = 0, 1
DTYPE_F32, DTYPE_BF16, DTYPE_F16 = 0, 1, 2
DTYPE_F16_STREAM = 3
SEARCH_AUTOREGRESSIVE, SEARCH_GENERATOR, SEARCH_TRIE = 0, 1, 2
SEARCH_SCORE = 3
SEARCH_ATTEND = 4
SEARCH_CONTEXT = 5
ACT_NONE, ACT_QUICKGELU, ACT_GELU_ERF = 0, 1, 2

EXPORTED_SYMBOLS = [
    "gitmi_abi_version", "gitmi_last_error", "gitmi_create", "gitmi_destroy", "gitmi_load_tensor",
    "gitmi_finalize_weights", "gitmi_encode_frames", "gitmi_prefill", "gitmi_step_logits",
    "gitmi_generate", "gitmi_search_begin", "gitmi_search_rows", "gitmi_search_advance",
    "gitmi_search_finish", "gitmi_profile_enable", "gitmi_profile_read", "gitmi_set_graph",
    "gitmi_op_gemm", "gitmi_op_layernorm", "gitmi_op_attention", "gitmi_op_dgemm", "gitmi_op_dgemm_res",
    "gitmi_op_vocab_topm", "gitmi_clone", "gitmi_op_attn_decode", "gitmi_preprocess_image",
    "gitmi_set_image_shape", "gitmi_preprocess_image_to", "gitmi_generate_prefixed", "gitmi_set_temporal_embedding", "gitmi_op_kv_repack", "gitmi_set_encode_after", "gitmi_op_sample_rows",
    "gitmi_search_done_count", "gitmi_set_trie", "gitmi_operand_dtype", "gitmi_set_shared_device", "gitmi_preprocess_batch",
    "gitmi_set_ln_fold", "gitmi_op_gemm_ln",
]
EXPERIMENT_SYMBOLS = [
    "gitmi_debug_import_stage", "gitmi_debug_head_from", "gitmi_debug_set_gemm_impl", "gitmi_debug_set_dgemm",
    "gitmi_debug_score_attn", "gitmi_debug_score_head", "gitmi_debug_attention_ragged", "gitmi_debug_attn_decode_ragged",
    "gitmi_debug_vocab_topm_rules", "gitmi_debug_search_begin_prefixed", "gitmi_debug_search_advance_lists", "gitmi_debug_read_hidden",
    "gitmi_debug_im2col", "gitmi_debug_pos_resize", "gitmi_debug_vit_assemble", "gitmi_debug_ragged_front", "gitmi_debug_zero_pad_rows",
    "gitmi_debug_layernorm_map", "gitmi_debug_score_attn_map", "gitmi_debug_attn_decode_form", "gitmi_debug_dgemm_form",
    "gitmi_debug_gemm_form", "gitmi_debug_context_embed",
]


class GitmiConfig(C.Structure):
    _fields_ = [(n, C.c_int32) for n in (
        "image_size", "patch", "vit_width", "vit_layers", "vit_heads", "dec_hidden", "dec_layers",
        "dec_heads", "dec_ffn", "vocab", "max_pos", "num_frames", "sos", "eos", "precision",
        "max_batch", "max_beams", "max_frames", "max_text_len", "max_image_pixels", "max_image_tokens")]


class GitmiSearch(C.Structure):
    _fields_ = [("kind", C.c_int32), ("beam_size", C.c_int32), ("per_node_beam_size", C.c_int32),
                ("max_steps", C.c_int32), ("length_penalty", C.c_double),
                ("do_sample", C.c_int32), ("top_k", C.c_int32), ("top_p", C.c_double), ("temperature", C.c_double),
                ("seed", C.c_uint64), ("repetition_penalty", C.c_double),
                ("num_keep_best", C.c_int32), ("reserved_", C.c_int32)]


class GitmiProfile(C.Structure):
    _fields_ = [("vit_ms", C.c_float), ("prefill_ms", C.c_float), ("decode_ms", C.c_float),
                ("total_ms", C.c_float), ("gemm_ms", C.c_float), ("gemm_launches", C.c_int32),
                ("gemm_flops", C.c_double), ("vit_gemm_ms", C.c_float), ("vit_gemm_launches", C.c_int32),
                ("vit_gemm_flops", C.c_double), ("decode_step_ms", C.c_float), ("decode_steps", C.c_int32),
                ("decode_step_bytes", C.c_double)]

    def as_dict(self) -> Dict[str, float]:
        return {n: getattr(self, n) for n, _ in self._fields_}


class GitmiError(RuntimeError):
    pass


_libs: Dict[str, C.CDLL] = {}
_experiment = False
_MEASUREMENT_LIBS = ("exp", "f16_exp")
_gemm_impl = -1


def use_experiment_build(on: bool = True) -> None:
    global _experiment
    _experiment = bool(on)


def load_library(operands: str = "bf16") -> C.CDLL:
    if operands == "bf16" and _experiment:
        operands = "exp"
    if operands in _libs:
        return _libs[operands]
    path = {"bf16": LIB_PATH, "f16": LIB_PATH_F16, "exp": LIB_PATH_EXP, "f16_exp": LIB_PATH_F16_EXP}[operands]
    if not os.path.exists(path):
        raise GitmiError(
            f"{path} not found: build it with `python -c 'import __graft_entry__ as g; g.build()'` "
# ... 21 lines not shown
    lib.gitmi_profile_read.argtypes = [vp, C.POINTER(GitmiProfile)]
    lib.gitmi_set_graph.argtypes = [vp, i32]
    lib.gitmi_set_temporal_embedding.argtypes = [vp, i32]
    lib.gitmi_set_encode_after.argtypes = [vp, vp]
    lib.gitmi_set_shared_device.argtypes = [vp, i32]
    lib.gitmi_set_ln_fold.argtypes = [vp, i32]
    lib.gitmi_op_gemm.argtypes = [vp, vp, vp, vp, vp, i32, i32, i32, i32, i32, i32, i32, i32, vp]
    lib.gitmi_op_gemm_ln.argtypes = [vp, vp, vp, vp, vp, C.c_float, vp, vp, vp, vp, C.c_float, vp, vp, i32, i32, i32, i32, vp]
    lib.gitmi_op_layernorm.argtypes = [vp, vp, vp, C.c_float, vp, vp, i32, i32, i32, vp]
    lib.gitmi_op_attention.argtypes = [vp, vp, i32, i32, i32, i32, i32, vp]
    lib.gitmi_op_dgemm.argtypes = [vp, vp, vp, vp, vp, i32, C.c_float, vp, i32, i32, i32, i32, i32, i32, vp]
    lib.gitmi_op_dgemm_res.argtypes = [vp, vp, vp, vp, vp, i32, vp, vp, C.c_float, vp, vp, vp, i32, i32, i32, vp]
    lib.gitmi_op_vocab_topm.argtypes = [vp, vp, vp, vp, vp, i32, C.c_float, i32, i32, i32, i32, i32, vp, vp, vp, vp, vp, i32, vp]
    lib.gitmi_generate_prefixed.argtypes = [vp, C.POINTER(vp), i32, i32, vp, i32, C.POINTER(C.c_int32), C.POINTER(C.c_int32),
                                            i32, C.POINTER(GitmiSearch), vp, vp, vp, vp, vp]
    lib.gitmi_clone.argtypes = [vp, C.POINTER(vp)]
    lib.gitmi_preprocess_image.argtypes = [vp, i32, i32, i32, vp, C.c_size_t, vp, vp]
    lib.gitmi_preprocess_image_to.argtypes = [vp, i32, i32, i32, i32, vp, C.c_size_t, vp, vp]
    lib.gitmi_preprocess_batch.argtypes = [vp, C.c_size_t, i64p, i32, i32, vp, C.c_size_t, vp, vp]
    lib.gitmi_set_image_shape.argtypes = [vp, i32, i32, vp]
    lib.gitmi_op_attn_decode.argtypes = [vp, vp, vp, vp, vp, vp, vp, i32, i32, i32, i32, i32, i32, i32, i32, vp]
    lib.gitmi_op_kv_repack.argtypes = [vp, vp, vp, i32, i32, i32, vp]
    lib.gitmi_op_sample_rows.argtypes = [vp, i32, i32, C.c_float, i32, C.c_float, i32, C.c_uint64, i32, vp, vp, vp, vp]
    if operands in _MEASUREMENT_LIBS:
        lib.gitmi_debug_import_stage.argtypes = [vp, vp, i32, vp]
        lib.gitmi_debug_head_from.argtypes = [vp, vp, i32, vp, vp]
        lib.gitmi_debug_set_gemm_impl.argtypes = [i32]
        lib.gitmi_debug_set_dgemm.argtypes = [i32]
        lib.gitmi_debug_dgemm_form.argtypes = [vp, i32, vp, vp, vp, vp, i32, C.c_float, vp, i32, i32, vp, vp, i32, vp, vp, C.c_float,
                                               vp, vp, vp, i32, i32, i32, i32, i32, i32, vp]
        lib.gitmi_debug_gemm_form.argtypes = [vp, i32, vp, vp, vp, i32, vp, i32, i32, i32, i32, i32, i32, i32, i32, vp, vp, C.c_float,
                                              vp, vp, vp, vp, C.c_float, vp]
        lib.gitmi_debug_score_attn.argtypes = [vp, vp, vp, vp, i32, i32, i32, i32, i32, vp]
        lib.gitmi_debug_score_head.argtypes = [vp, vp, vp, vp, i32, i32, i32, i32, vp, vp]
        lib.gitmi_debug_score_attn_map.argtypes = [vp, vp, vp, vp, vp, i32, i32, i32, i32, i32, vp]
        lib.gitmi_debug_attention_ragged.argtypes = [vp, vp, vp, i32, i32, i32, i32, i32, vp]
        lib.gitmi_debug_attn_decode_ragged.argtypes = [vp, vp, vp, vp, vp, vp, vp, vp, i32, i32, i32, i32, i32, i32, i32, vp]
        lib.gitmi_debug_attn_decode_form.argtypes = [vp, vp, vp, vp, vp, vp, vp, vp, vp, i32, i32, i32, i32, i32, i32, i32, i32, i32,
                                                     i32, i32, i32, vp]
        lib.gitmi_debug_vocab_topm_rules.argtypes = [vp, vp, vp, vp, vp, i32, C.c_float, i32, i32, i32, i32, i32, vp, i32, i32, vp, i32,
                                                     i32, C.c_float, vp, vp, vp, vp, i32, vp]
        lib.gitmi_debug_search_begin_prefixed.argtypes = [vp, C.POINTER(GitmiSearch), i32, vp, i32, vp, i32, vp]
        lib.gitmi_debug_search_advance_lists.argtypes = [vp, vp, vp, vp, i32, i32, i32, vp]
        lib.gitmi_debug_read_hidden.argtypes = [vp, i32, vp, vp, C.POINTER(C.c_int), C.POINTER(C.c_int), vp]
        lib.gitmi_debug_im2col.argtypes = [vp, vp, i32, i32, i32, i32, i32, i32, i32, vp]
        lib.gitmi_debug_pos_resize.argtypes = [vp, vp, i32, i32, i32, i32, vp]
        lib.gitmi_debug_vit_assemble.argtypes = [vp, vp, vp, vp, vp, C.c_float, vp, i32, i32, i32, i32, vp, vp]
        lib.gitmi_debug_ragged_front.argtypes = [i32, vp, vp, vp, vp, vp, i32, vp, vp, vp, i32, vp, vp, C.c_float, vp, i32, vp, i32, i32,
                                                 C.c_longlong, i32, i32, i32, i32, vp]
        lib.gitmi_debug_zero_pad_rows.argtypes = [vp, i32, i32, vp, i32, i32, vp]
        lib.gitmi_debug_layernorm_map.argtypes = [vp, i32, vp, vp, C.c_float, vp, vp, i32, vp, i32, i32, i32, i32, i32, vp]
        lib.gitmi_debug_context_embed.argtypes = [vp, i32, vp, vp, i32, vp, i32, vp, i32, vp, vp, C.c_float, vp, i32, vp, vp, i32, i32,
                                                  i32, i32, vp]
    for name in EXPORTED_SYMBOLS + (EXPERIMENT_SYMBOLS if operands in _MEASUREMENT_LIBS else []):
        if name not in ("gitmi_last_error", "gitmi_destroy"):
            getattr(lib, name).restype = C.c_int
    if lib.gitmi_abi_version() != 10:
        raise GitmiError("libgitmi.so ABI version mismatch")
    lib.gitmi_operand_dtype.restype = C.c_int
    if lib.gitmi_operand_dtype() != {"bf16": DTYPE_BF16, "f16": DTYPE_F16, "exp": DTYPE_BF16, "f16_exp": DTYPE_F16}[operands]:
        raise GitmiError(f"{path} was not built for {operands} operands")
    if operands in _MEASUREMENT_LIBS and _gemm_impl != -1:
        _ck(lib.gitmi_debug_set_gemm_impl(_gemm_impl), lib)
    _libs[operands] = lib
    return lib


def _experiment_only(lib, name: str):
    try:
        return getattr(lib, name)
    except AttributeError:
        raise GitmiError(f"{name} is exported by the measurement build only (libgitmi_exp.so, libgitmi_f16_exp.so): call "
                         f"generativeimage2text_amd.engine.use_experiment_build() before creating the engine") from None


def _ck(rc: int, lib=None) -> None:
    if rc != 0:
        libs = [lib] if lib is not None else list(_libs.values())
        msgs = [m for m in ((l.gitmi_last_error() or b"").decode("utf-8", "replace") for l in libs) if m]
        raise GitmiError(" | ".join(msgs) or "gitmi call failed")


def _stream() -> int:
    return int(torch.cuda.current_stream().cuda_stream)


def _ptr(t: Optional[torch.Tensor]) -> Optional[int]:
    return None if t is None else int(t.data_ptr())


def _torch_dtype_code(t: torch.Tensor) -> int:
    return {torch.float32: DTYPE_F32, torch.bfloat16: DTYPE_BF16, torch.float16: DTYPE_F16}[t.dtype]


_OPERAND_LIBS = {torch.bfloat16: "bf16", torch.float16: "f16"}


def _op_library(*dtypes: torch.dtype, fp32_ok: bool = False) -> C.CDLL:
    dts = set(dtypes) - {torch.float32}
    if not dts and fp32_ok:
        return load_library()
    if len(dts) != 1 or next(iter(dts)) not in _OPERAND_LIBS:
        raise GitmiError(f"operands must all be bf16 or all fp16, got {sorted(str(d) for d in dts) or ['float32']}")
    return load_library(_OPERAND_LIBS[dts.pop()])


# ... 64 lines not shown
def context_capacity(image_size: int, patch: int, max_image_tokens: int, max_frames: int, max_context: int) -> int:
    if max_context <= 0:
        return int(max_image_tokens)
    n_nat = (int(image_size) // int(patch)) ** 2 + 1
    return max(n_nat, int(max_image_tokens)) + -(-int(max_context) // max(1, int(max_frames)))


class RaggedImages:

    def __init__(self, buffer: torch.Tensor, shapes: Sequence[Tuple[int, int]]):
        self.buffer, self.shapes = buffer, [tuple(int(v) for v in hw) for hw in shapes]

    def __len__(self) -> int:
        return len(self.shapes)


def pack_ragged(images: Sequence[torch.Tensor], patch: int, max_pixels: int, max_tokens: int, max_batch: int,
                device=None) -> RaggedImages:
    images = list(images)
    B = len(images)
    if not 1 <= B <= max_batch:
        raise ValueError(f"{B} images: a ragged call takes 1 .. max_batch={max_batch}")
    shapes = []
    for b, im in enumerate(images):
        if not isinstance(im, torch.Tensor) or im.dim() != 3 or int(im.shape[0]) != 3:
            raise ValueError(f"image {b}: expected a [3, h, w] tensor, got {getattr(im, 'shape', type(im))}")
        h, w = int(im.shape[1]), int(im.shape[2])
        if h < patch or w < patch:
            raise ValueError(f"image {b}: {h}x{w} is smaller than one {patch}-pixel patch")
        if h * w > max_pixels:
            raise ValueError(f"image {b}: {h}x{w} exceeds the max_image_pixels capacity ({max_pixels})")
        if (h // patch) * (w // patch) + 1 > max_tokens:
            raise ValueError(f"image {b}: a {h // patch}x{w // patch} token grid exceeds the max_image_tokens capacity "
                             f"({max_tokens})")
        shapes.append((h, w))
    desc_floats = (B * 16 + RAGGED_DESC_BYTES - 1) // RAGGED_DESC_BYTES * (RAGGED_DESC_BYTES // 4)
    offsets, off = [], desc_floats
    for h, w in shapes:
        offsets.append(off)
        off += (3 * h * w + 3) // 4 * 4
    dev = torch.device(device) if device is not None else images[0].device
    buf = torch.zeros(off, dtype=torch.float32, device=dev)
    desc = torch.tensor([[h, w, o, 0] for (h, w), o in zip(shapes, offsets)], dtype=torch.int32)
    buf[:4 * B].view(torch.int32).copy_(desc.reshape(-1))
    for im, (h, w), o in zip(images, shapes, offsets):
        buf[o:o + 3 * h * w].copy_(im.detach().to(dtype=torch.float32).reshape(-1))
    return RaggedImages(buf, shapes)


class Engine:

    def __init__(self, model_cfg, precision: str = "bf16", max_batch: int = 64, max_beams: int = 4,
                 max_frames: int = 1, max_text_len: int = 40, device: Optional[int] = None,
                 max_image_hw: Optional[Tuple[int, int]] = None, max_context: int = 0):
        if not torch.cuda.is_available():
            raise GitmiError("no GPU visible: the GIT engine runs on MI355X (gfx950) only, there is no CPU fallback")
        self.lib = load_library("f16" if precision in ("f16", "fp16") else "bf16")
        self.device = torch.cuda.current_device() if device is None else int(device)
        self.cfg = model_cfg
        self.precision = precision
        c = GitmiConfig()
        for name in ("image_size", "patch", "vit_width", "vit_layers", "vit_heads", "dec_hidden", "dec_layers",
                     "dec_heads", "dec_ffn", "vocab", "max_pos", "num_frames", "sos", "eos"):
            setattr(c, name, int(getattr(model_cfg, name)))
        c.precision = {"bf16": PREC_BF16, "f16": PREC_BF16, "fp16": PREC_BF16, "f32": PREC_F32, "fp32": PREC_F32}[precision]
        c.max_batch, c.max_beams = int(max_batch), int(max_beams)
        c.max_frames, c.max_text_len = int(max_frames), int(max_text_len)
        if max_image_hw is None:
            max_image_hw = getattr(model_cfg, "max_image_hw", None)
        if max_image_hw is not None:
            mh, mw = int(max_image_hw[0]), int(max_image_hw[1])
            c.max_image_pixels = mh * mw
            c.max_image_tokens = (mh // c.patch) * (mw // c.patch) + 1
        c.max_image_tokens = context_capacity(c.image_size, c.patch, c.max_image_tokens, c.max_frames, max_context)
        self.max_context = int(max_context)
        self.c = c
        self.n_tok = (c.image_size // c.patch) ** 2 + 1
        self._hw = (int(c.image_size), int(c.image_size))
        self._h = C.c_void_p()
        self._ck(self.lib.gitmi_create(C.byref(c), self.device, C.byref(self._h)))
        self._finalized = False
        self._init_resident()
        self._temb = True
        self._ln_fold = precision in ("f16", "fp16") and c.vit_width % 256 == 0 and c.dec_hidden % 256 == 0

    def _ck(self, rc: int) -> None:
        _ck(rc, self.lib)

    def clone(self) -> "Engine":
        other = object.__new__(Engine)
        other.lib, other.device, other.cfg, other.precision = self.lib, self.device, self.cfg, self.precision
        other.c = GitmiConfig.from_buffer_copy(self.c)
        other.max_context = self.max_context
        other.n_tok = (self.c.image_size // self.c.patch) ** 2 + 1
        other._hw = (int(self.c.image_size), int(self.c.image_size))
        other._h = C.c_void_p()
        self._ck(self.lib.gitmi_clone(self._h, C.byref(other._h)))
        other._finalized = True
        other._parent = self
        other._init_resident()
        other._temb, other._ln_fold = self._temb, self._ln_fold
        return other

    def _init_resident(self) -> None:
        self._resident: Optional[int] = None
        self._generation = 0
        self._geometry = self._call_geometry = None

    @property
    def resident(self) -> Optional[int]:
# ... 315 lines not shown
        off = torch.as_tensor(child_off, dtype=torch.int32).cpu().contiguous()
        tok = torch.as_tensor(child_tok, dtype=torch.int32).cpu().contiguous()
        node = torch.as_tensor(child_node, dtype=torch.int32).cpu().contiguous()
        assert off.numel() >= 2 and tok.numel() == node.numel() == int(off[-1])
        self._ck(self.lib.gitmi_set_trie(self._h, int(off.numel()) - 1, off.data_ptr(), tok.data_ptr() if tok.numel() else None,
                                    node.data_ptr() if node.numel() else None))

    def debug_import_stage(self, src: "Engine", stage: int) -> None:
        self._ck(_experiment_only(self.lib, "gitmi_debug_import_stage")(self._h, src._h, int(stage), _stream()))
        self._resident = src._resident
        self._generation += 1

    def debug_head_from(self, src: "Engine", R: int) -> torch.Tensor:
        out = torch.empty(R, self.c.vocab, device=f"cuda:{self.device}", dtype=torch.float32)
        self._ck(_experiment_only(self.lib, "gitmi_debug_head_from")(self._h, src._h, int(R), out.data_ptr(), _stream()))
        torch.cuda.current_stream().synchronize()
        return out

    def debug_search_begin_prefixed(self, search: GitmiSearch, prefixes: Sequence[Sequence[int]], vocab: int) -> None:
        start = id_table(prefixes)
        B, ld = start.shape
        plen = torch.tensor([len(p) for p in prefixes], dtype=torch.int32)
        self._ck(_experiment_only(self.lib, "gitmi_debug_search_begin_prefixed")(
            self._h, C.byref(search), B, start.data_ptr(), ld, plen.data_ptr(), vocab, _stream()))
        self._search_k, self._search_B, self._search_T, self._search_cfg = search.beam_size, B, search.max_steps, search

    def debug_search_advance_lists(self, part_val: torch.Tensor, part_idx: torch.Tensor, part_lse: torch.Tensor,
                                   embed: bool = False) -> None:
        dev = f"cuda:{self.device}"
        pv = part_val.to(device=dev, dtype=torch.float32).contiguous()
        pi = part_idx.to(device=dev, dtype=torch.int32).contiguous()
        pl = part_lse.to(device=dev, dtype=torch.float32).contiguous()
        R, nparts, slots = pv.shape
        if pi.shape != pv.shape or tuple(pl.shape) != (R, nparts, 2) or R != self._search_B * self._search_k:
            raise ValueError(f"candidate lists {tuple(pv.shape)} / {tuple(pi.shape)} / {tuple(pl.shape)} do not describe the "
                             f"{self._search_B * self._search_k} rows of the search")
        self._keep_lists = (pv, pi, pl)
        self._ck(_experiment_only(self.lib, "gitmi_debug_search_advance_lists")(
            self._h, pv.data_ptr(), pi.data_ptr(), pl.data_ptr(), nparts, slots, 1 if embed else 0, _stream()))

    def debug_read_hidden(self, R: int) -> Tuple[torch.Tensor, torch.Tensor]:
        D = int(self.c.dec_hidden)
        dev = f"cuda:{self.device}"
        Rp = (R + 15) // 16 * 16
        hf = torch.empty(R, D, device=dev, dtype=torch.float32)
        raw = torch.empty(Rp * D * 4, device=dev, dtype=torch.uint8)
        frag, dt = C.c_int(), C.c_int()
        self._ck(_experiment_only(self.lib, "gitmi_debug_read_hidden")(self._h, int(R), hf.data_ptr(), raw.data_ptr(),
                                                                       C.byref(frag), C.byref(dt), _stream()))
        tdt = {DTYPE_F32: torch.float32, DTYPE_BF16: torch.bfloat16, DTYPE_F16: torch.float16}[dt.value]
        ht = raw.view(tdt)[:Rp * D].reshape(Rp, D)
        return hf, (from_frag(ht, R) if frag.value else ht[:R].contiguous())

    def search_done_count(self) -> int:
        n = C.c_int()
        self._ck(self.lib.gitmi_search_done_count(self._h, C.byref(n), _stream()))
        return int(n.value)

    def search_finish(self):
        dev = f"cuda:{self.device}"
        tokens, logprobs, info = self._out(self._search_B, self._search_cfg, dev)
        self._ck(self.lib.gitmi_search_finish(self._h, tokens.data_ptr(), logprobs.data_ptr(), info.data_ptr(), _stream()))
        torch.cuda.current_stream().synchronize()
        return tokens, logprobs, info

    def profile_enable(self, on) -> None:
        self._ck(self.lib.gitmi_profile_enable(self._h, int(on)))

    def profile_read(self) -> Dict[str, float]:
        p = GitmiProfile()
        self._ck(self.lib.gitmi_profile_read(self._h, C.byref(p)))
        return p.as_dict()

    def set_shared_device(self, on: bool = True) -> None:
        self._ck(self.lib.gitmi_set_shared_device(self._h, 1 if on else 0))

    def set_encode_after(self, other: Optional["Engine"]) -> None:
        self._ck(self.lib.gitmi_set_encode_after(self._h, other._h if other is not None else None))

    def set_temporal_embedding(self, on: bool) -> None:
        self._ck(self.lib.gitmi_set_temporal_embedding(self._h, 1 if on else 0))
        if bool(on) != self._temb:
            self._temb = bool(on)
            self._drop_resident()

    def set_ln_fold(self, on: bool) -> None:
        self._ck(self.lib.gitmi_set_ln_fold(self._h, 1 if on else 0))
        if bool(on) != self._ln_fold:
            self._ln_fold = bool(on)
            self._drop_resident()

    def set_graph(self, on: bool) -> None:
        self._ck(self.lib.gitmi_set_graph(self._h, 1 if on else 0))


def op_context_embed(tokens: torch.Tensor, lengths: Sequence[int], image_of: Optional[Sequence[int]], words: torch.Tensor,
                     positions: torch.Tensor, gamma: torch.Tensor, beta: torch.Tensor, eps: float, feats: torch.Tensor,
                     n_img: int, want_f32: bool = False, operands: Optional[str] = None):
    assert tokens.is_cuda and tokens.dtype == torch.int64 and tokens.is_contiguous() and feats.is_cuda and feats.is_contiguous()
    B, stride, D = feats.shape
    Q, ld = tokens.shape
    lib = _exp_library(feats.dtype, operands=operands)
    fn = _experiment_only(lib, "gitmi_debug_context_embed")
    f32 = lambda t: t.to(device=feats.device, dtype=torch.float32).contiguous()
    words, positions, gamma, beta = f32(words), f32(positions), f32(gamma), f32(beta)
    ntok = torch.full((B,), -1, dtype=torch.int32, device=feats.device)
# ... 7 lines not shown

def op_gemm(A: torch.Tensor, W: torch.Tensor, bias: Optional[torch.Tensor] = None,
            residual: Optional[torch.Tensor] = None, act: int = ACT_NONE,
            out_dtype: torch.dtype = torch.float32, stream_rows: bool = False) -> torch.Tensor:
    assert A.is_cuda and W.is_cuda and A.dtype == W.dtype and A.is_contiguous() and W.is_contiguous()
    M, K = A.shape
    N = W.shape[0]
    if stream_rows:
        if A.dtype == torch.float32:
            raise GitmiError("op_gemm: fp16 stream rows need 16-bit operands")
        if residual is not None and (residual.dtype != torch.float16 or residual.shape != (M, N) or not residual.is_contiguous()):
            raise GitmiError("op_gemm: the stream form's residual is contiguous fp16 [M, N] rows")
        lib, out_code, out_dtype = _op_library(A.dtype), DTYPE_F16_STREAM, torch.float16
    else:
        if residual is not None and residual.dtype != torch.float32:
            raise GitmiError("op_gemm: the residual is fp32 (fp16 rows: stream_rows=True)")
        lib = _op_library(A.dtype, out_dtype, fp32_ok=True)
        out_code = {torch.float32: DTYPE_F32, torch.bfloat16: DTYPE_BF16, torch.float16: DTYPE_F16}[out_dtype]
    out = torch.empty(M, N, device=A.device, dtype=out_dtype)
    _ck(lib.gitmi_op_gemm(A.data_ptr(), W.data_ptr(), _ptr(bias), _ptr(residual), out.data_ptr(), M, N, K, K, N,
                          _torch_dtype_code(A), out_code, act, _stream()), lib)
    return out


def op_gemm_ln(A: torch.Tensor, W: torch.Tensor, bias: Optional[torch.Tensor], *, colsum: Optional[torch.Tensor] = None,
               ln_part: Optional[torch.Tensor] = None, ln_eps: float = 1e-5, residual: Optional[torch.Tensor] = None,
               res_part: Optional[torch.Tensor] = None, res_gamma: Optional[torch.Tensor] = None,
               res_beta: Optional[torch.Tensor] = None, res_eps: float = 1e-12, want_part: bool = False, act: int = ACT_NONE):
    lib = load_library("f16")
    assert A.dtype == torch.float16 and W.dtype == torch.float16 and A.is_contiguous() and W.is_contiguous()
    M, K = A.shape
    N = W.shape[0]
    out = torch.empty(M, N, device=A.device, dtype=torch.float16)
    part = torch.zeros(M, 4, 2, device=A.device, dtype=torch.float32) if want_part else None
    _ck(lib.gitmi_op_gemm_ln(A.data_ptr(), W.data_ptr(), _ptr(bias), _ptr(colsum), _ptr(ln_part), ln_eps, _ptr(residual),
                             _ptr(res_part), _ptr(res_gamma), _ptr(res_beta), res_eps, out.data_ptr(), _ptr(part), M, N, K, act,
                             _stream()), lib)
    return (out, part) if want_part else out


def op_gemm_form(A: torch.Tensor, W: torch.Tensor, C: torch.Tensor, M: int, N: int, K: int, *, lda: Optional[int] = None,
                 ldc: Optional[int] = None, bias=None, res=None, ldr: int = 0, act: int = ACT_NONE, stream_rows: bool = False,
                 shared: bool = False, ln_part=None, colsum=None, ln_eps: float = 1e-5, part_out=None, res_part=None,
                 res_gamma=None, res_beta=None, res_eps: float = 1e-5, operands: Optional[str] = None) -> None:
    if A.dtype != W.dtype:
        raise GitmiError(f"operands must share one type, got {A.dtype} / {W.dtype}")
    lib = _exp_library(A.dtype, *(() if stream_rows else (C.dtype,)), operands=operands)
    out_code = DTYPE_F16_STREAM if stream_rows else _torch_dtype_code(C)
    _ck(_experiment_only(lib, "gitmi_debug_gemm_form")(
        A.data_ptr(), int(K if lda is None else lda), W.data_ptr(), _ptr(bias), _ptr(res), int(ldr), C.data_ptr(),
        int(N if ldc is None else ldc), int(M), int(N), int(K), int(act), _torch_dtype_code(A), out_code, int(bool(shared)),
        _ptr(ln_part), _ptr(colsum), float(ln_eps), _ptr(part_out), _ptr(res_part), _ptr(res_gamma), _ptr(res_beta), float(res_eps),
        _stream()), lib)


def op_layernorm(x: torch.Tensor, gamma: torch.Tensor, beta: torch.Tensor, eps: float,
                 out_dtype: torch.dtype = torch.float32) -> torch.Tensor:
    lib = _op_library(out_dtype, fp32_ok=True)
    rows, D = x.shape
    out = torch.empty(rows, D, device=x.device, dtype=out_dtype)
    _ck(lib.gitmi_op_layernorm(x.data_ptr(), gamma.data_ptr(), beta.data_ptr(), eps, out.data_ptr(), None, rows, D,
                               _torch_dtype_code(out), _stream()), lib)
    return out


def op_attention(qkv: torch.Tensor, B: int, N: int, H: int, impl: int) -> torch.Tensor:
    lib = _op_library(qkv.dtype, fp32_ok=True)
    assert qkv.is_cuda and qkv.is_contiguous() and qkv.shape == (B * N, 3 * H * 64)
    out = torch.empty(B * N, H * 64, device=qkv.device, dtype=qkv.dtype)
    _ck(lib.gitmi_op_attention(qkv.data_ptr(), out.data_ptr(), B, N, H, _torch_dtype_code(qkv), impl, _stream()), lib)
    return out


def strip_stats(x: torch.Tensor) -> torch.Tensor:
    M, N = x.shape
    xs = x.float().reshape(M, N // 16, 16)
    return torch.stack([xs.sum(-1), (xs * xs).sum(-1)], dim=-1).permute(1, 0, 2).contiguous()


def to_frag(x: torch.Tensor, row_multiple: int = 16) -> torch.Tensor:
    R, K = x.shape
    Rp = (R + row_multiple - 1) // row_multiple * row_multiple
    xp = torch.zeros(Rp, K, dtype=x.dtype, device=x.device)
    xp[:R] = x
    return xp.reshape(Rp // 16, 16, K // 32, 4, 8).permute(0, 2, 3, 1, 4).contiguous().reshape(Rp, K)


def from_frag(xf: torch.Tensor, rows: int) -> torch.Tensor:
    Rp, K = xf.shape
    return xf.reshape(Rp // 16, K // 32, 4, 16, 8).permute(0, 3, 1, 2, 4).reshape(Rp, K)[:rows].contiguous()


def _pad_vec(v: Optional[torch.Tensor], n: int) -> Optional[torch.Tensor]:
    if v is None:
        return None
    out = torch.zeros(n, dtype=v.dtype, device=v.device)
    out[:v.numel()] = v
    return out


def op_dgemm(A: torch.Tensor, W: torch.Tensor, bias: torch.Tensor, colsum: Optional[torch.Tensor] = None,
             stats: Optional[torch.Tensor] = None, eps: float = 1e-12, act: int = ACT_NONE,
             frag_out: bool = False, packed: bool = False, strips_per_wg: int = 0) -> torch.Tensor:
    lib = _op_library(A.dtype, W.dtype)
    if packed:
        Af, Wf, M, N, K = A, W, int(A.shape[0]), int(bias.numel()), int(A.shape[1])
# ... 331 lines not shown
```

### include/gitmi_experiment.h

```cpp
#ifndef GITMI_EXPERIMENT_H_
#define GITMI_EXPERIMENT_H_
#include "gitmi.h"
#ifdef __cplusplus
extern "C" {
#endif

int  gitmi_debug_import_stage(gitmi_engine* dst, gitmi_engine* src, int stage, void* stream);
int  gitmi_debug_head_from(gitmi_engine* dst, gitmi_engine* src, int R, float* logits_out, void* stream);

int  gitmi_debug_set_gemm_impl(int impl);

int  gitmi_debug_set_dgemm(int dbg);

int  gitmi_debug_dgemm_form(const void* A, int a_rows, const void* W, const float* bias, const float* colsum, const float* stats,
                            int strips, float eps, void* C, int c_frag, int act, const float* res_x, const float* res_stats,
                            int res_strips, const float* res_gamma, const float* res_beta, float res_eps, float* x_out,
                            void* xb_out, float* stats_out, int M, int N, int K, int rows_per_wg, int strips_per_wg,
                            int no_row_walk, void* stream);

int  gitmi_debug_gemm_form(const void* A, int lda, const void* W, const float* bias, const void* res, int ldr, void* C, int ldc,
                           int M, int N, int K, int act, int in_dtype, int out_dtype, int shared, const float* ln_part,
                           const float* colsum, float ln_eps, float* part_out, const float* res_part, const float* res_gamma,
                           const float* res_beta, float res_eps, void* stream);

int  gitmi_debug_score_attn(const void* qkv, const void* img_kv, const int* image_of, void* out, int Q, int H, int N_img, int Lp,
                            int dtype, void* stream);
int  gitmi_debug_score_attn_map(const void* qkv, const void* img_kv, const int* image_of, const int* ntok, float* out, int Q, int H,
                                int N_img, int Lp, int dtype, void* stream);
int  gitmi_debug_score_head(const void* A, const void* W, const float* bias, const int* tgt, int M, int V, int K, int dtype,
                            float* out, void* stream);

int  gitmi_debug_attention_ragged(const void* qkv, void* out, const int* ntok, int B, int N, int H, int dtype, int impl, void* stream);
int  gitmi_debug_attn_decode_ragged(const void* qkv, const void* img_k, const void* img_v, void* txt_k, void* txt_v,
                                    const int* kv_src, void* out, const int* ntok, int B, int H, int N_img, int T_max, int pos,
                                    int beams, int dtype, void* stream);
int  gitmi_debug_attn_decode_form(const void* qkv, const void* img_k, const void* img_v, void* txt_k, void* txt_v,
                                  const int* kv_src, void* out, const int* ntok, const int* img_of, int n_images, int B, int H,
                                  int N_img, int T_max, int pos, int beams, int dtype, int out_frag, int pairs_per_wg,
                                  int waves_per_pair, int stream_wgs, void* stream);

int  gitmi_debug_vocab_topm_rules(const void* A, const void* W, const float* bias, const float* colsum, const float* stats,
                                  int strips, float eps, int M, int V, int K, int cols_per_wg, int mtop, const int* ids, int ld_ids,
                                  int cur_len, const int* plen, int beams, int suppress_kind, float rep_penalty, float* part_val,
                                  int* part_idx, float* part_lse, float* logits_out, int max_wgs, void* stream);
int  gitmi_debug_search_begin_prefixed(gitmi_engine* e, const gitmi_search* sp, int B, const int64_t* start_host, int ld,
                                       const int32_t* plen_host, int vocab, void* stream);
int  gitmi_debug_search_advance_lists(gitmi_engine* e, const float* part_val, const int* part_idx, const float* part_lse,
                                      int nparts, int slots, int embed, void* stream);
int  gitmi_debug_read_hidden(gitmi_engine* e, int R, float* hf_out, void* ht_out, int* ht_frag, int* ht_dtype, void* stream);

int  gitmi_debug_im2col(const float* img, void* out, int out_dtype, int B, int H, int W, int p, int K, int Kpad, void* stream);
int  gitmi_debug_pos_resize(const float* pos, float* out, int g, int gh, int gw, int D, void* stream);
int  gitmi_debug_vit_assemble(const float* patch_out, const float* cls, const float* pos, const float* gamma, const float* beta,
                              float eps, void* X, int x_f16, int B, int N, int D, float* part, void* stream);
int  gitmi_debug_ragged_front(int stage, const float* src, float* slots, int* meta, int* ntok, void* patches, int patches_dtype,
                              const float* patch_out, const float* cls, const float* pos, int g, const float* gamma,
                              const float* beta, float eps, void* X, int x_f16, float* part, int B, int p, long long max_pixels,
                              int Nmax, int K, int Kpad, int D, void* stream);
int  gitmi_debug_zero_pad_rows(void* x, int is_f32, int ld, const int* ntok, int B, int Nmax, void* stream);
int  gitmi_debug_layernorm_map(const void* x, int src_f16, const float* gamma, const float* beta, float eps, const float* add_after,
                               void* y_t, int out_dtype, void* y_s, int rows, int D, int map_n_in, int map_n_out, int map_off,
                               void* stream);

int  gitmi_debug_context_embed(const int64_t* tokens, int ld, const int32_t* len_host, const int32_t* image_of_host, int Q,
                               const float* words, int vocab, const float* positions, int max_pos, const float* gamma,
                               const float* beta, float eps, void* feats, int dtype, float* feats_f32, int* ntok, int B, int n_img,
                               int stride, int D, void* stream);

#ifdef __cplusplus
}
#endif
#endif
```

Baseline: 11410 captions/s.

## Emit decode K/V cache layout from prefill QKV GEMM epilogue and reuse it in attention

The prefill QKV GEMM (p8 kernel) gains an epilogue that writes the K and V columns directly into the per-head fragment/transposed cache layout used by decode attention. This removes the separate kv_repack pass. The full self-attention over image rows gains a CACHED variant that loads those pre-laid-out K/V blocks straight into LDS with global_load_lds, skipping the strided staging loads. The feature is gated on fp16, attn_impl 1, uniform batches, 193..208 image rows and p8 eligibility. It adds state tracking (have_kv_rows) so paths that need the packed row form of K/V can still rerun prefill without the emission.

New measurement: 11420 captions/s (median of 3 runs). Within noise of the previous version (+0.1%).

```diff
diff --git a/generativeimage2text_amd/csrc/abi_ops.hip b/generativeimage2text_amd/csrc/abi_ops.hip
--- a/generativeimage2text_amd/csrc/abi_ops.hip
+++ b/generativeimage2text_amd/csrc/abi_ops.hip
@@ -277,6 +277,42 @@
             return fail("debug_gemm_form: the folded forms exist in gemm_p8_kernel only (more than 512 rows, N %% 256 == 0, K >= 128, 16-byte aligned rows)");
     }
     HIPCK(launch_gemm(g, in_f32, out_f32, (hipStream_t)stream));
+    return 0;
+}
+
+GITMI_EXP_EXPORT int gitmi_debug_gemm_kv_emit(const void* A, int lda, const void* W, const float* bias, void* C, int ldc, int M, int N,
+                                              int K, int shared, const float* ln_part, const float* colsum, float ln_eps, void* kf,
+                                              void* vt, int n_img, int H, int k_col0, void* stream) {
+    if (!A || !W || !C || !kf || !vt) return fail("debug_gemm_kv_emit: null argument (A, W, C, kf, vt)");
+    if (M < 1 || N < 1 || K < 64 || K % 64 || lda < K || ldc < N) return fail("debug_gemm_kv_emit: M=%d N=%d K=%d lda=%d ldc=%d", M, N, K, lda, ldc);
+    if (n_img < 1 || M % n_img || H < 1 || H % 4) return fail("debug_gemm_kv_emit: whole images of n_img rows, heads a multiple of 4 (M=%d n_img=%d H=%d)", M, n_img, H);
+    if (k_col0 < 0 || k_col0 % 256 || k_col0 + 2 * H * 64 != N) return fail("debug_gemm_kv_emit: the output ends with K|V: k_col0 + 2 H 64 == N, k_col0 %% 256 == 0");
+    if ((ln_part != nullptr) != (colsum != nullptr)) return fail("debug_gemm_kv_emit: ln_part and colsum go together");
+    GemmArgs g{};
+    g.A = A; g.W = W; g.bias = bias; g.C = C; g.M = M; g.N = N; g.K = K; g.lda = lda; g.ldc = ldc; g.shared = shared ? 1 : 0;
+    if (ln_part) {
+#ifndef GITMI_OPS_F16
+        return fail("debug_gemm_kv_emit: the folded-LayerNorm forms are built into the fp16-operand library only");
+#endif
+        if (K > 1024) return fail("debug_gemm_kv_emit: row partials cover K <= 1024 (K=%d)", K);
+        g.ln_part = (const float2*)ln_part; g.ln_nparts = (K + 255) / 256; g.ln_colsum = colsum; g.ln_inv_d = 1.0f / (float)K; g.ln_eps = ln_eps;
+    }
+    g.kv.kf = kf; g.kv.vt = vt; g.kv.N = n_img; g.kv.N_pad = round_up(n_img, 32); g.kv.H = H; g.kv.k_col0 = k_col0; g.kv.v_col0 = k_col0 + H * 64;
+    if (!gemm_uses_p8(g, false, false))
+        return fail("debug_gemm_kv_emit: the emission exists in gemm_p8_kernel only (more than 512 rows, N %% 256 == 0, K >= 128, 16-byte aligned rows)");
+    HIPCK(launch_gemm(g, false, false, (hipStream_t)stream));
+    return 0;
+}
+GITMI_EXP_EXPORT int gitmi_debug_attention_cached(const void* qkv, const void* kf, const void* vt, void* out, int B, int N, int H,
+                                                  void* stream) {
+    if (!qkv || !kf || !vt || !out || B < 1 || H < 1) return fail("debug_attention_cached: bad argument");
+    if (N < 193 || N > 208) return fail("debug_attention_cached: the cached form serves 193..208 rows per image (N=%d)", N);
+    const int D = H * 64;
+    AttnFullArgs a{};
+    a.q = qkv; a.k = (const char*)qkv + (size_t)D * 2; a.v = (const char*)qkv + (size_t)2 * D * 2; a.out = out;
+    a.ldq = a.ldk = a.ldv = 3 * D; a.ldo = D; a.N = N; a.H = H; a.scale = 0.125f;
+    a.kf = kf; a.vt = vt; a.N_pad = round_up(N, 32);
+    HIPCK(launch_attn_full(a, B, false, 1, (hipStream_t)stream));
     return 0;
 }
 
diff --git a/generativeimage2text_amd/csrc/engine.hip b/generativeimage2text_amd/csrc/engine.hip
--- a/generativeimage2text_amd/csrc/engine.hip
+++ b/generativeimage2text_amd/csrc/engine.hip
@@ -86,13 +86,14 @@
     st.part = part; st.gamma = gamma; st.beta = beta; st.eps = eps;
 }
 static int ln_gemm(gitmi_engine* e, hipStream_t s, const Stream& st, const Folded& f, const void* W, const float* bias, void* C,
-                   int ldc, int col0, int N, int act) {
+                   int ldc, int col0, int N, int act, const KvEmit* kv = nullptr) {
     const int D = st.D;
     const size_t woff = (size_t)col0 * D * e->pol.esz;
     C = (char*)C + (size_t)col0 * e->pol.esz;
     if (st.fold) {
         GemmArgs g = gemm_args(st.x, D, (const char*)f.w + woff, f.bias + col0, nullptr, 0, C, ldc, st.M, N, D, act);
         g.ln_part = st.part; g.ln_nparts = D / 256; g.ln_colsum = f.colsum + col0; g.ln_inv_d = 1.0f / (float)D; g.ln_eps = st.eps;
+        if (kv) g.kv = *kv;
         return gemm_run(e, s, g, false, false, st.tag);
     }
     if (e->pol.stream_f16)
@@ -100,7 +101,9 @@
     else
         HIPCK(launch_layernorm((const float*)st.x, D, st.gamma, st.beta, st.eps, nullptr, st.t, D, e->pol.f32, st.xn, st.xn ? D : 0, st.M,
                                D, 0, 0, 0, s));
-    return gemm(e, s, st.t, D, (const char*)W + woff, bias + col0, nullptr, 0, C, ldc, e->pol.f32, st.M, N, D, act, st.tag);
+    GemmArgs g = gemm_args(st.t, D, (const char*)W + woff, bias + col0, nullptr, 0, C, ldc, st.M, N, D, act);
+    if (kv) g.kv = *kv;
+    return gemm_run(e, s, g, e->pol.f32, e->pol.f32, st.tag);
 }
 static int gemm_to_stream(gitmi_engine* e, hipStream_t s, Stream& st, const void* A, int lda, const void* W, const float* bias, int K,
                           bool residual, const float* gamma, const float* beta, float eps) {
@@ -121,7 +124,7 @@
     return 0;
 }
 static int attn_full_packed(gitmi_engine* e, const void* qkv, void* out, int width, int heads, int N, int batch, const int* ntok,
-                            hipStream_t s) {
+                            hipStream_t s, const KvEmit* kv = nullptr) {
     AttnFullArgs a{};
     a.q = qkv;
     a.k = (const char*)qkv + (size_t)width * e->pol.esz;
@@ -131,6 +134,7 @@
     a.ldo = width;
     a.N = N; a.H = heads; a.scale = 0.125f;
     a.ntok = ntok;
+    if (kv) { a.kf = kv->kf; a.vt = kv->vt; a.N_pad = kv->N_pad; }
     HIPCK(launch_attn_full(a, batch, e->pol.f32, e->pol.attn_impl, s));
     return 0;
 }
@@ -198,6 +202,7 @@
     if (const char* env = getenv("GITMI_ATTN_NH")) e->pol.attn_nh = atoi(env);
     if (const char* env = getenv("GITMI_ATTN_STREAM")) e->pol.attn_stream = atoi(env);
     if (const char* env = getenv("GITMI_DECODE_SKIP")) e->pol.decode_skip = atoi(env);
+    if (const char* env = getenv("GITMI_KV_EMIT")) e->pol.kv_emit = atoi(env) != 0;
     if (const char* env = getenv("GITMI_GEMM_TALL")) e->pol.gemm_tall = atoi(env);
     if (const char* env = getenv("GITMI_DGEMM_ROWS")) e->pol.dgemm_rows = atoi(env);
     if (const char* env = getenv("GITMI_DGEMM_STRIPS")) e->pol.dgemm_strips = atoi(env);
@@ -229,15 +234,15 @@
     for (CapturedGraph* g : {&e->graph_full, &e->graph_decode, &e->graph_follow}) g->reset();
     e->full_slot.valid = e->follow_slot.valid = false;
 }
-static void drop_resident(gitmi_engine* e) { e->have_feats = e->have_prefill = false; }
+static void drop_resident(gitmi_engine* e) { e->have_feats = e->have_prefill = e->have_kv_rows = false; }
 static void set_resident(gitmi_engine* e, int B, int F_eff, int stride = 0) {
     e->cur_B = B; e->cur_F = F_eff; e->cur_Nimg = stride > 0 ? stride : F_eff * e->N;
-    e->have_feats = true; e->have_prefill = false;
+    e->have_feats = true; e->have_prefill = e->have_kv_rows = false;
     e->keyed = e->ragged; e->has_context = false;
 }
 static void set_context(gitmi_engine* e) { e->keyed = e->has_context = true; }
 static const int* key_counts(const gitmi_engine* e) { return e->keyed ? e->rg_ntok : nullptr; }
-static void set_prefilled(gitmi_engine* e) { e->have_prefill = true; }
+static void set_prefilled(gitmi_engine* e, bool kv_rows) { e->have_prefill = true; e->have_kv_rows = kv_rows; }
 static int settle_residency(gitmi_engine* e, const Request& rq, int rc) {
     if (rc != 0 && rq.frames) drop_resident(e);
     return rc;
@@ -325,6 +330,16 @@
                                          on_p8(e->p_ctx, d, L.wo, e->p_y, d, M, d, d, true) && on_p8(e->p_u, ffn, L.w2, e->p_y, d, M, d, ffn, true)));
     if (st.fold) { st.parts[0] = e->p_part[0]; st.parts[1] = e->p_part[1]; }
     return st;
+}
+
+static bool kv_emit_gate(const gitmi_engine* e, int B, int Nimg, bool kv_rows) {
+    const int d = e->cfg.dec_hidden;
+    if (kv_rows || e->pol.kv_emit == 0 || e->pol.f32 || e->pol.attn_impl != 1 || e->keyed) return false;
+    if (Nimg > 208 || (Nimg + 15) / 16 != 13 || d % 256 != 0) return false;
+    const DecLayerW& L = e->w.dec[0];
+    const void* W = e->pol.ln_fold ? L.qkv_pf.w : L.wqkv;
+    return on_p8(e->p_y, d, W, e->img_kv[0], 3 * d, B * Nimg, 3 * d, d, false) &&
+           on_p8(e->p_y, d, W, e->img_kv[0], 3 * d, B * Nimg, 2 * d, d, false);
 }
 
 static int encode_frames_impl(gitmi_engine* e, const float* const* frames, int F, int B, float* feats_out,
@@ -397,11 +412,14 @@
     return 0;
 }
 
-static int prefill_impl(gitmi_engine* e, hipStream_t s) {
+static int prefill_impl(gitmi_engine* e, hipStream_t s, bool kv_rows = false) {
     const gitmi_config& c = e->cfg;
     const int d = c.dec_hidden, ffn = c.dec_ffn, D = c.vit_width;
     const int B = e->cur_B, Nimg = e->cur_Nimg, M = B * Nimg;
-    e->have_prefill = false;
+    e->have_prefill = e->have_kv_rows = false;
+    const bool emit = kv_emit_gate(e, B, Nimg, kv_rows);
+    KvEmit kv{};
+    if (emit) { kv.N = Nimg; kv.N_pad = round_up(Nimg, 32); kv.H = c.dec_heads; }
     SpanGuard phase(e, s, TAG_PREFILL, 0);
     Stream y = prefill_stream(e, M);
     RCK(gemm_to_stream(e, s, y, e->feats, D, e->w.vp_w, e->w.vp_b, D, false, e->w.vp_lng, e->w.vp_lnb, 1e-5f));
@@ -409,15 +427,16 @@
         const DecLayerW& L = e->w.dec[l];
         const bool last = l + 1 == c.dec_layers;
         const int col0 = last ? d : 0;
-        RCK(ln_gemm(e, s, y, L.qkv_pf, L.wqkv, L.bqkv, e->img_kv[l], 3 * d, col0, 3 * d - col0, 0));
-        RCK(kv_repack(e, l, B, Nimg, s));
+        if (emit) { kv.kf = e->img_kh[l]; kv.vt = e->img_vh[l]; kv.k_col0 = d - col0; kv.v_col0 = 2 * d - col0; }
+        RCK(ln_gemm(e, s, y, L.qkv_pf, L.wqkv, L.bqkv, e->img_kv[l], 3 * d, col0, 3 * d - col0, 0, emit ? &kv : nullptr));
+        if (!emit) RCK(kv_repack(e, l, B, Nimg, s));
         if (last) break;
-        RCK(attn_full_packed(e, e->img_kv[l], e->p_ctx, d, c.dec_heads, Nimg, B, key_counts(e), s));
+        RCK(attn_full_packed(e, e->img_kv[l], e->p_ctx, d, c.dec_heads, Nimg, B, key_counts(e), s, emit ? &kv : nullptr));
         RCK(gemm_to_stream(e, s, y, e->p_ctx, d, L.wo, L.bo, d, true, L.lnag, L.lnab, 1e-12f));
         RCK(ln_gemm(e, s, y, L.ffn1_pf, L.w1, L.b1, e->p_u, ffn, 0, ffn, 2));
         RCK(gemm_to_stream(e, s, y, e->p_u, ffn, L.w2, L.b2, ffn, true, L.lnog, L.lnob, 1e-12f));
     }
-    set_prefilled(e);
+    set_prefilled(e, !emit);
     return 0;
 }
 
@@ -853,13 +872,26 @@
     return 0;
 }
 
-static int generate_encode(gitmi_engine* e, const Request& rq, hipStream_t s) {
+GITMI_EXP_EXPORT int gitmi_debug_read_kv_cache(gitmi_engine* e, int layer, void* kf_out, void* vt_out, int* emitted, void* stream) {
+    RCK(check_ready(e));
+    if (e->pol.f32 || !e->have_prefill) return fail("debug_read_kv_cache: needs a 16-bit context with a current prefill");
+    if (layer < 0 || layer >= e->cfg.dec_layers || !kf_out || !vt_out || !emitted) return fail("debug_read_kv_cache: bad argument");
+    hipStream_t s = (hipStream_t)stream;
+    const size_t bytes = (size_t)e->cur_B * round_up(e->cur_Nimg, 32) * e->cfg.dec_hidden * 2;
+    HIPCK(hipMemcpyAsync(kf_out, e->img_kh[layer], bytes, hipMemcpyDefault, s));
+    HIPCK(hipMemcpyAsync(vt_out, e->img_vh[layer], bytes, hipMemcpyDefault, s));
+    HIPCK(hipStreamSynchronize(s));
+    *emitted = e->have_kv_rows ? 0 : 1;
+    return 0;
+}
+
+static int generate_encode(gitmi_engine* e, const Request& rq, hipStream_t s, bool kv_rows = false) {
     RCK(encode_frames_impl(e, rq.frames, rq.F, rq.B, nullptr, s));
-    return prefill_impl(e, s);
-}
-static int images_ready(gitmi_engine* e, const Request& rq, hipStream_t s) {
-    if (rq.frames) return generate_encode(e, rq, s);
-    return e->have_prefill ? 0 : prefill_impl(e, s);
+    return prefill_impl(e, s, kv_rows);
+}
+static int images_ready(gitmi_engine* e, const Request& rq, hipStream_t s, bool kv_rows = false) {
+    if (rq.frames) return generate_encode(e, rq, s, kv_rows);
+    return e->have_prefill && (!kv_rows || e->have_kv_rows) ? 0 : prefill_impl(e, s, kv_rows);
 }
 
 static int generate_decode(gitmi_engine* e, const Request& rq, hipStream_t s, bool allow_poll) {
@@ -979,7 +1011,7 @@
             e->full_slot = {key, true}; e->graph_is_split = split;
         } else {
             set_resident(e, rq.B, F_eff);
-            set_prefilled(e);
+            set_prefilled(e, !kv_emit_gate(e, e->cur_B, e->cur_Nimg, false));
         }
         enc = &e->graph_full;
         if (split) dec = &e->graph_decode;
@@ -1109,7 +1141,7 @@
     const gitmi_config& c = e->cfg;
     const int d = c.dec_hidden, V = c.vocab, Q = rq.Q, L = c.dec_layers;
     const bool attend = rq.sp->kind == GITMI_SEARCH_ATTEND;
-    RCK(images_ready(e, rq, s));
+    RCK(images_ready(e, rq, s, true));
     const int Lp = round_up(rq.maxP, 16), M = Q * Lp;
     const int Nk = e->cur_Nimg, Kc = Nk + ld;
     void* const out = attend ? (void*)e->at_out : (void*)e->sc_out;
@@ -1382,6 +1414,7 @@
         return fail("debug_import_stage: the two contexts are different models");
     if (!src->have_feats || (stage == 2 && !src->have_prefill)) return fail("debug_import_stage: the source has not run that stage");
     if (src->has_context) return fail("debug_import_stage: the source's resident images carry context rows");
+    if (stage == 2 && !src->have_kv_rows) RCK(prefill_impl(src, (hipStream_t)stream, true));
     if (src->cur_B > a.max_batch || src->cur_F > a.max_frames || src->N != dst->N) return fail("debug_import_stage: capacity / resolution mismatch");
     hipStream_t s = (hipStream_t)stream;
     const size_t M = (size_t)src->cur_B * src->cur_Nimg;
@@ -1392,7 +1425,7 @@
             HIPCK(launch_convert(src->img_kv[l], src->pol.f32, dst->img_kv[l], dst->pol.f32, M * 3 * a.dec_hidden, s));
             RCK(kv_repack(dst, l, dst->cur_B, dst->cur_Nimg, s));
         }
-        set_prefilled(dst);
+        set_prefilled(dst, true);
     }
     return 0;
 }
diff --git a/generativeimage2text_amd/csrc/engine_state.h b/generativeimage2text_amd/csrc/engine_state.h
--- a/generativeimage2text_amd/csrc/engine_state.h
+++ b/generativeimage2text_amd/csrc/engine_state.h
@@ -110,6 +110,7 @@
     int vocab_wgs = -1;
     int gemm_tall = 1;
     int dgemm_rows = 0;
+    int kv_emit = -1;
     int decode_skip = 0;
 };
 
@@ -165,6 +166,7 @@
 
     int cur_B = 0, cur_F = 0, cur_Nimg = 0;
     bool have_feats = false, have_prefill = false;
+    bool have_kv_rows = false;
 
     int profile_mode = 0;
     bool profiling = false;
diff --git a/generativeimage2text_amd/csrc/kernels_attn.hip b/generativeimage2text_amd/csrc/kernels_attn.hip
--- a/generativeimage2text_amd/csrc/kernels_attn.hip
+++ b/generativeimage2text_amd/csrc/kernels_attn.hip
@@ -225,7 +225,7 @@
     }
 }
 
-template <int NSUB, bool RAGGED = false>
+template <int NSUB, bool RAGGED = false, bool CACHED = false>
 __global__ __launch_bounds__(256, 2) void attn_full_mfma_short_kernel(AttnFullArgs a) {
     constexpr int NK = NSUB * 16;
     constexpr int NB = (NSUB + 1) / 2;
@@ -250,6 +250,20 @@
         }
     }
 
+    if constexpr (CACHED) {
+        static_assert(!RAGGED, "the cached form serves uniform batches");
+        static_assert(NK * HD <= NK * FA_LDK && NB * 32 * HD <= HD * LDV, "the cache blocks fit the LDS arrays");
+        typedef __attribute__((address_space(3))) void lds_void_t;
+        const size_t blk = ((size_t)b * a.H + h) * a.N_pad * HD;
+        const bf16_t* Kf = reinterpret_cast<const bf16_t*>(a.kf) + blk;
+        const bf16_t* Vc = reinterpret_cast<const bf16_t*>(a.vt) + blk;
+        const int wv = __builtin_amdgcn_readfirstlane(wave);
+        for (int c = wv; c < NK / 8; c += 4)
+            __builtin_amdgcn_global_load_lds((const void*)(Kf + c * 512 + lane * 8), (lds_void_t*)(Ks + c * 512), 16, 0, 0);
+        for (int c = wv; c < NB * 4; c += 4)
+            __builtin_amdgcn_global_load_lds((const void*)(Vc + c * 512 + lane * 8), (lds_void_t*)(Vt + c * 512), 16, 0, 0);
+        asm volatile("s_waitcnt vmcnt(0)" ::: "memory");
+    } else {
 #pragma unroll
     for (int it = 0; it < (NK * 8 + 255) / 256; ++it) {
         int idx = tid + it * 256;
@@ -287,6 +301,7 @@
             }
         }
     }
+    }
     __syncthreads();
 
     const int nqt = (n + 15) >> 4;
@@ -306,8 +321,8 @@
         f32x4_t sacc[NT][NSUB];
 #pragma unroll
         for (int st_ = 0; st_ < NSUB; ++st_) {
-            const bf16x8_t kf0 = *reinterpret_cast<const bf16x8_t*>(Ks + (st_ * 16 + l15) * FA_LDK + lg * 8);
-            const bf16x8_t kf1 = *reinterpret_cast<const bf16x8_t*>(Ks + (st_ * 16 + l15) * FA_LDK + 32 + lg * 8);
+            const bf16x8_t kf0 = *reinterpret_cast<const bf16x8_t*>(CACHED ? Ks + (st_ * 128 + lane) * 8 : Ks + (st_ * 16 + l15) * FA_LDK + lg * 8);
+            const bf16x8_t kf1 = *reinterpret_cast<const bf16x8_t*>(CACHED ? Ks + (st_ * 128 + 64 + lane) * 8 : Ks + (st_ * 16 + l15) * FA_LDK + 32 + lg * 8);
 #pragma unroll
             for (int u = 0; u < NT; ++u) {
                 sacc[u][st_] = mfma16(kf0, qf[u][0], f32x4_t{0.f, 0.f, 0.f, 0.f});
@@ -380,9 +395,13 @@
 #pragma unroll
             for (int dt = 0; dt < 4; ++dt) {
                 union { bf16x8_t v; uint2 h2[2]; } vf;
-                const bf16_t* vp = Vt + (dt * 16 + l15) * LDV + blk * 32 + lg * 4;
-                vf.h2[0] = *reinterpret_cast<const uint2*>(vp);
-                vf.h2[1] = *reinterpret_cast<const uint2*>(vp + 16);
+                if constexpr (CACHED) {
+                    vf.v = *reinterpret_cast<const bf16x8_t*>(Vt + ((blk * 4 + dt) * 64 + lane) * 8);
+                } else {
+                    const bf16_t* vp = Vt + (dt * 16 + l15) * LDV + blk * 32 + lg * 4;
+                    vf.h2[0] = *reinterpret_cast<const uint2*>(vp);
+                    vf.h2[1] = *reinterpret_cast<const uint2*>(vp + 16);
+                }
 #pragma unroll
                 for (int u = 0; u < NT; ++u)
                     o_acc[u][dt] = mfma16(vf.v, pf[u], o_acc[u][dt]);
@@ -686,9 +705,15 @@
 
 hipError_t launch_attn_full(const AttnFullArgs& a, int B, bool is_f32, int impl, hipStream_t s) {
     if (B <= 0 || a.N <= 0) return hipSuccess;
+    if (a.kf && impl != 1) return hipErrorInvalidValue;
     if (impl == 1) {
         if (is_f32) return hipErrorInvalidValue;
         const int nsub = (a.N + 15) / 16;
+        if (a.kf) {
+            if (nsub != 13 || a.ntok || !a.vt || a.N_pad != (a.N + 31) / 32 * 32 || a.N_pad != 224) return hipErrorInvalidValue;
+            hipLaunchKernelGGL((attn_full_mfma_short_kernel<13, false, true>), dim3(a.H, B), dim3(256), 0, s, a);
+            return hipGetLastError();
+        }
         if (nsub == 13 && a.ntok) hipLaunchKernelGGL((attn_full_mfma_short_kernel<13, true>), dim3(a.H, B), dim3(256), 0, s, a);
         else if (nsub == 13) hipLaunchKernelGGL(attn_full_mfma_short_kernel<13>, dim3(a.H, B), dim3(256), 0, s, a);
         else if (nsub == 17 && a.ntok) hipLaunchKernelGGL((attn_full_mfma_short_kernel<17, true>), dim3(a.H, B), dim3(256), 0, s, a);
diff --git a/generativeimage2text_amd/csrc/kernels_gemm10.hip b/generativeimage2text_amd/csrc/kernels_gemm10.hip
--- a/generativeimage2text_amd/csrc/kernels_gemm10.hip
+++ b/generativeimage2text_amd/csrc/kernels_gemm10.hip
@@ -71,9 +71,100 @@
     else if constexpr (N == 0) asm volatile("s_waitcnt vmcnt(0)" ::: "memory");
 }
 
-template <typename TOut, int ACT, int DBG = 0, int MH = 128, int EPI = 1, int MH1 = MH, int LNF = 0>
+__device__ __forceinline__ void kv_store16(unsigned short* p, const u32x4_t& v) {
+    asm volatile("global_store_dwordx4 %0, %1, off sc1\n\ts_nop 1" ::"v"(p), "v"(v) : "memory");
+}
+__device__ __forceinline__ void kv_emit_k_slab(const KvEmit& kv, int M, const unsigned short* ep, int eps, int tid, int row0, int nrows,
+                                               int head0) {
+    const int rows = nrows < M - row0 ? nrows : M - row0;
+    if (rows <= 0) return;
+    const int N = kv.N, ntiles = kv.N_pad >> 4;
+    const int r16 = tid & 15, cc = tid >> 4;
+    const int head = head0 + (cc >> 3), ch = cc & 7;
+    const int img_b = (row0 + rows - 1) / N, key_b = row0 + rows - 1 - img_b * N;
+    const int t_b = key_b == N - 1 ? ntiles - 1 : key_b >> 4;
+    int img = row0 / N, t = (row0 - img * N) >> 4;
+    for (;; ) {
+        const int key = t * 16 + r16, r = img * N + key - row0;
+        const int rl = img * N + N - 1 - row0;
+        unsigned short* dst = reinterpret_cast<unsigned short*>(kv.kf) + ((size_t)img * kv.H + head) * kv.N_pad * 64 +
+                              frag_tile(t, ch >> 2, 2, (ch & 3) * 16 + r16);
+        const u32x4_t v = *reinterpret_cast<const u32x4_t*>(ep + (r < 0 ? 0 : r < rows ? r : rows - 1) * eps + cc * 8);
+        if (key < N) {
+            if (r >= 0 && r < rows) kv_store16(dst, v);
+        } else if (rl >= 0 && rl < rows) {
+            kv_store16(dst, u32x4_t{0u, 0u, 0u, 0u});
+        }
+        if (img == img_b && t == t_b) break;
+        if (++t == ntiles) { t = 0; ++img; }
+    }
+}
+__device__ __forceinline__ void kv_emit_v_slab(const KvEmit& kv, int M, const unsigned short* ep, int eps, int tid, int row0, int nrows,
+                                               int head0) {
+    const int rows = nrows < M - row0 ? nrows : M - row0;
+    if (rows <= 0) return;
+    const int N = kv.N, nsteps = kv.N_pad >> 5;
+    const int lane = tid & 63, lg = lane >> 4, dtile0 = (tid >> 6) * 2;
+    unsigned short* const vt = reinterpret_cast<unsigned short*>(kv.vt);
+    const int img_b = (row0 + rows - 1) / N, s_b = (row0 + rows - 1 - img_b * N) >> 5;
+    int img = row0 / N, s = (row0 - img * N) >> 5;
+    for (;; ) {
+        const int rl = img * N + N - 1 - row0;
+        const bool owner = rl >= 0 && rl < rows;
+        int rc[2][4];
+        bool whole[2], ok[2][4], in[2][4];
+#pragma unroll
+        for (int q = 0; q < 2; ++q) {
+            const int k0 = s * 32 + q * 16 + lg * 4;
+            whole[q] = true;
+#pragma unroll
+            for (int e = 0; e < 4; ++e) {
+                const int r = img * N + k0 - row0 + e;
+                rc[q][e] = r < 0 ? 0 : r < rows ? r : rows - 1;
+                in[q][e] = k0 + e < N && r >= 0 && r < rows;
+                ok[q][e] = in[q][e] || (k0 + e >= N && owner);
+                whole[q] = whole[q] && ok[q][e];
+            }
+        }
+#pragma unroll
+        for (int j = 0; j < 2; ++j) {
+            const int col = (dtile0 + j) * 16 + (lane & 15);
+            const int head = head0 + (col >> 6), dt = (col >> 4) & 3;
+            unsigned short* dst = vt + (((size_t)img * kv.H + head) * kv.N_pad * 64 + (((s * 4 + dt) * 64 + lane) * 8));
+            uint32_t x[2][4];
+#pragma unroll
+            for (int q = 0; q < 2; ++q)
+#pragma unroll
+                for (int e = 0; e < 4; ++e) x[q][e] = ep[rc[q][e] * eps + col];
+#pragma unroll
+            for (int q = 0; q < 2; ++q)
+#pragma unroll
+                for (int e = 0; e < 4; ++e) x[q][e] = in[q][e] ? x[q][e] : 0u;
+            const uint32_t w[2][2] = {{x[0][0] | (x[0][1] << 16), x[0][2] | (x[0][3] << 16)}, {x[1][0] | (x[1][1] << 16), x[1][2] | (x[1][3] << 16)}};
+            if (whole[0] && whole[1]) {
+                kv_store16(dst, u32x4_t{w[0][0], w[0][1], w[1][0], w[1][1]});
+            } else {
+#pragma unroll
+                for (int q = 0; q < 2; ++q) {
+                    if (whole[q]) {
+                        *reinterpret_cast<uint2*>(dst + q * 4) = uint2{w[q][0], w[q][1]};
+                    } else {
+#pragma unroll
+                        for (int e = 0; e < 4; ++e)
+                            if (ok[q][e]) dst[q * 4 + e] = (unsigned short)x[q][e];
+                    }
+                }
+            }
+        }
+        if (img == img_b && s == s_b) break;
+        if (++s == nsteps) { s = 0; ++img; }
+    }
+}
+
+template <typename TOut, int ACT, int DBG = 0, int MH = 128, int EPI = 1, int MH1 = MH, int LNF = 0, int EMIT = 0>
 __global__ __launch_bounds__(512) void gemm_p8_kernel(GemmArgs g) {
     static_assert(LNF == 0 || sizeof(TOut) == 2, "LayerNorm folding: 16-bit outputs only");
+    static_assert(EMIT == 0 || (sizeof(TOut) == 2 && LNF != 2 && DBG == 0), "K/V emission: operand-type rows of the plain and consumer forms");
     static_assert(MH % 32 == 0 && MH1 % 32 == 0 && MH1 <= MH && MH <= 128, "half tiles: multiples of 32 rows, second <= first");
     constexpr int BM = MH + MH1, MI = MH / 32, MI1 = MH1 / 32;
     __shared__ __attribute__((aligned(16))) unsigned char smem[LDS_BYTES];
@@ -365,6 +456,11 @@
         return;
     }
 
+    int kv_kind = 0, kv_head0 = 0;
+    if constexpr (EMIT != 0) {
+        kv_kind = n0 >= g.kv.v_col0 ? 2 : n0 >= g.kv.k_col0 ? 1 : 0;
+        kv_head0 = (n0 - (kv_kind == 2 ? g.kv.v_col0 : g.kv.k_col0)) >> 6;
+    }
     float rgm[8], rbt[8];
     if constexpr (LNF == 2) {
         if (g.res_part) {
@@ -401,6 +497,15 @@
                 }
             }
             P8_LDS_BARRIER();
+            if constexpr (EMIT != 0) {
+                if (kv_kind != 0) {
+                    const unsigned short* eps16 = reinterpret_cast<const unsigned short*>(ep);
+                    if (kv_kind == 1) kv_emit_k_slab(g.kv, g.M, eps16, EPS, tid, m0 + qm * MH, MHq, kv_head0);
+                    else kv_emit_v_slab(g.kv, g.M, eps16, EPS, tid, m0 + qm * MH, MHq, kv_head0);
+                    P8_LDS_BARRIER();
+                    continue;
+                }
+            }
 #pragma unroll 4
             for (int q = 0; q < MHq * CPR / 512; ++q) {
                 const int chunk = tid + q * 512;
@@ -503,8 +608,12 @@
 
 }
 
-template <typename TOut, int MH, int EPI = 1, int MH1 = MH, int LNF = 0>
+template <typename TOut, int MH, int EPI = 1, int MH1 = MH, int LNF = 0, int EMIT = 0>
 static void launch_p8_t(const GemmArgs& g, hipStream_t s) {
+    if constexpr (EMIT != 0) {
+        hipLaunchKernelGGL((gemm_p8_kernel<TOut, GITMI_ACT_NONE, 0, MH, EPI, MH1, LNF, 1>), dim3(g.nwg), dim3(512), 0, s, g);
+        return;
+    } else
     if constexpr (LNF == 2) {
         hipLaunchKernelGGL((gemm_p8_kernel<TOut, GITMI_ACT_NONE, 0, MH, EPI, MH1, LNF>), dim3(g.nwg), dim3(512), 0, s, g);
         return;
@@ -583,9 +692,11 @@
 template <int MH, int MH1>
 static void launch_p8_height(const GemmArgs& g, bool out_f32, bool staged, hipStream_t s) {
 #ifdef GITMI_OPS_F16
+    if (g.ln_part && g.kv.kf) { launch_p8_t<bf16_t, MH, 1, MH1, 1, 1>(g, s); return; }
     if (g.ln_part) { launch_p8_t<bf16_t, MH, 1, MH1, 1>(g, s); return; }
     if (g.part_out || g.res_part) { launch_p8_t<f16_t, MH, 1, MH1, 2>(g, s); return; }
 #endif
+    if (g.kv.kf) { launch_p8_t<bf16_t, MH, 1, MH1, 0, 1>(g, s); return; }
     if (g.out_f16) launch_p8_t<f16_t, MH, 1, MH1>(g, s);
     else if (!out_f32) launch_p8_t<bf16_t, MH, 1, MH1>(g, s);
     else if (staged) launch_p8_t<float, MH, 0, MH1>(g, s);
@@ -600,6 +711,12 @@
         if (g.ln_part && (out_f32 || g.out_f16 || g.res || !g.ln_colsum || g.ln_nparts < 1 || g.part_out || g.res_part)) return hipErrorInvalidValue;
         if ((g.part_out || g.res_part) && (!g.out_f16 || out_f32 || g.act != 0 || g.N > 1024)) return hipErrorInvalidValue;
         if (g.res_part && (!g.res || !g.res_gamma || !g.res_beta || g.res_nparts < 1)) return hipErrorInvalidValue;
+    }
+    if (g.kv.kf) {
+        const KvEmit& kv = g.kv;
+        if (!kv.vt || out_f32 || g.out_f16 || g.res || g.act != 0 || g.part_out || g.res_part) return hipErrorInvalidValue;
+        if (kv.N < 1 || kv.H < 1 || g.M % kv.N != 0 || kv.N_pad != (kv.N + 31) / 32 * 32 || (kv.H * 64) % BN != 0) return hipErrorInvalidValue;
+        if (kv.k_col0 < 0 || kv.k_col0 % BN != 0 || kv.v_col0 != kv.k_col0 + kv.H * 64 || kv.v_col0 + kv.H * 64 != g.N) return hipErrorInvalidValue;
     }
     static const int heights[5] = {256, 224, 192, 160, 128};
     int bm = 256;
diff --git a/generativeimage2text_amd/csrc/launchers.h b/generativeimage2text_amd/csrc/launchers.h
--- a/generativeimage2text_amd/csrc/launchers.h
+++ b/generativeimage2text_amd/csrc/launchers.h
@@ -3,6 +3,12 @@
 #include <stddef.h>
 
 namespace gitmi {
+
+struct KvEmit {
+    void* kf; void* vt;
+    int N, N_pad, H;
+    int k_col0, v_col0;
+};
 
 struct GemmArgs {
     const void* A; const void* W; const float* bias; const float* res; void* C;
@@ -17,6 +23,7 @@
     const float2* ln_part; int ln_nparts; const float* ln_colsum; float ln_inv_d, ln_eps;
     float2* part_out;
     const float2* res_part; int res_nparts; const float* res_gamma; const float* res_beta; float res_inv_d, res_eps;
+    KvEmit kv;
 };
 bool gemm_uses_p8(const GemmArgs& g, bool in_f32, bool out_f32);
 hipError_t launch_gemm(const GemmArgs& g, bool in_f32, bool out_f32, hipStream_t s);
@@ -121,6 +128,7 @@
     int N, H;
     float scale;
     const int* ntok;
+    const void* kf; const void* vt; int N_pad;
 };
 hipError_t launch_attn_full(const AttnFullArgs& a, int B, bool is_f32, int impl, hipStream_t s);
 
diff --git a/generativeimage2text_amd/engine.py b/generativeimage2text_amd/engine.py
--- a/generativeimage2text_amd/engine.py
+++ b/generativeimage2text_amd/engine.py
@@ -38,7 +38,8 @@
     "gitmi_debug_vocab_topm_rules", "gitmi_debug_search_begin_prefixed", "gitmi_debug_search_advance_lists", "gitmi_debug_read_hidden",
     "gitmi_debug_im2col", "gitmi_debug_pos_resize", "gitmi_debug_vit_assemble", "gitmi_debug_ragged_front", "gitmi_debug_zero_pad_rows",
     "gitmi_debug_layernorm_map", "gitmi_debug_score_attn_map", "gitmi_debug_attn_decode_form", "gitmi_debug_dgemm_form",
-    "gitmi_debug_gemm_form", "gitmi_debug_context_embed",
+    "gitmi_debug_gemm_form", "gitmi_debug_context_embed", "gitmi_debug_gemm_kv_emit", "gitmi_debug_attention_cached",
+    "gitmi_debug_read_kv_cache",
 ]
 
 
@@ -166,6 +167,9 @@
         lib.gitmi_debug_layernorm_map.argtypes = [vp, i32, vp, vp, C.c_float, vp, vp, i32, vp, i32, i32, i32, i32, i32, vp]
         lib.gitmi_debug_context_embed.argtypes = [vp, i32, vp, vp, i32, vp, i32, vp, i32, vp, vp, C.c_float, vp, i32, vp, vp, i32, i32,
                                                   i32, i32, vp]
+        lib.gitmi_debug_gemm_kv_emit.argtypes = [vp, i32, vp, vp, vp, i32, i32, i32, i32, i32, vp, vp, C.c_float, vp, vp, i32, i32, i32, vp]
+        lib.gitmi_debug_attention_cached.argtypes = [vp, vp, vp, vp, i32, i32, i32, vp]
+        lib.gitmi_debug_read_kv_cache.argtypes = [vp, i32, vp, vp, C.POINTER(C.c_int), vp]
     for name in EXPORTED_SYMBOLS + (EXPERIMENT_SYMBOLS if operands in _MEASUREMENT_LIBS else []):
         if name not in ("gitmi_last_error", "gitmi_destroy"):
             getattr(lib, name).restype = C.c_int
@@ -336,10 +340,10 @@
 
     def __init__(self, model_cfg, precision: str = "bf16", max_batch: int = 64, max_beams: int = 4,
                  max_frames: int = 1, max_text_len: int = 40, device: Optional[int] = None,
-                 max_image_hw: Optional[Tuple[int, int]] = None, max_context: int = 0):
+                 max_image_hw: Optional[Tuple[int, int]] = None, max_context: int = 0, library: Optional[str] = None):
         if not torch.cuda.is_available():
             raise GitmiError("no GPU visible: the GIT engine runs on MI355X (gfx950) only, there is no CPU fallback")
-        self.lib = load_library("f16" if precision in ("f16", "fp16") else "bf16")
+        self.lib = load_library(library or ("f16" if precision in ("f16", "fp16") else "bf16"))
         self.device = torch.cuda.current_device() if device is None else int(device)
         self.cfg = model_cfg
         self.precision = precision
@@ -761,6 +765,15 @@
         ht = raw.view(tdt)[:Rp * D].reshape(Rp, D)
         return hf, (from_frag(ht, R) if frag.value else ht[:R].contiguous())
 
+    def debug_read_kv_cache(self, layer: int, B: int, n_img: int) -> Tuple[torch.Tensor, torch.Tensor, bool]:
+        shape = (B, int(self.c.dec_heads), (n_img + 31) // 32 * 32, 64)
+        kf = torch.empty(shape, device=f"cuda:{self.device}", dtype=torch.int16)
+        vt = torch.empty_like(kf)
+        emitted = C.c_int()
+        self._ck(_experiment_only(self.lib, "gitmi_debug_read_kv_cache")(self._h, int(layer), kf.data_ptr(), vt.data_ptr(),
+                                                                         C.byref(emitted), _stream()))
+        return kf, vt, bool(emitted.value)
+
     def search_done_count(self) -> int:
         n = C.c_int()
         self._ck(self.lib.gitmi_search_done_count(self._h, C.byref(n), _stream()))
@@ -874,6 +887,24 @@
         int(N if ldc is None else ldc), int(M), int(N), int(K), int(act), _torch_dtype_code(A), out_code, int(bool(shared)),
         _ptr(ln_part), _ptr(colsum), float(ln_eps), _ptr(part_out), _ptr(res_part), _ptr(res_gamma), _ptr(res_beta), float(res_eps),
         _stream()), lib)
+
+
+def op_gemm_kv_emit(A: torch.Tensor, W: torch.Tensor, C: torch.Tensor, kf: torch.Tensor, vt: torch.Tensor, M: int, N: int, K: int,
+                    n_img: int, H: int, k_col0: int, *, ldc: Optional[int] = None, bias=None, shared: bool = False, ln_part=None,
+                    colsum=None, ln_eps: float = 1e-5) -> None:
+    lib = _exp_library(A.dtype, W.dtype, C.dtype, kf.dtype, vt.dtype)
+    _ck(_experiment_only(lib, "gitmi_debug_gemm_kv_emit")(
+        A.data_ptr(), int(K), W.data_ptr(), _ptr(bias), C.data_ptr(), int(N if ldc is None else ldc), int(M), int(N), int(K),
+        int(bool(shared)), _ptr(ln_part), _ptr(colsum), float(ln_eps), kf.data_ptr(), vt.data_ptr(), int(n_img), int(H), int(k_col0),
+        _stream()), lib)
+
+
+def op_attention_cached(qkv: torch.Tensor, kf: torch.Tensor, vt: torch.Tensor, B: int, N: int, H: int) -> torch.Tensor:
+    lib = _exp_library(qkv.dtype, kf.dtype, vt.dtype)
+    out = torch.empty(B * N, H * 64, device=qkv.device, dtype=qkv.dtype)
+    _ck(_experiment_only(lib, "gitmi_debug_attention_cached")(qkv.data_ptr(), kf.data_ptr(), vt.data_ptr(), out.data_ptr(), int(B),
+                                                              int(N), int(H), _stream()), lib)
+    return out
 
 
 def op_layernorm(x: torch.Tensor, gamma: torch.Tensor, beta: torch.Tensor, eps: float,
diff --git a/include/gitmi_experiment.h b/include/gitmi_experiment.h
--- a/include/gitmi_experiment.h
+++ b/include/gitmi_experiment.h
@@ -22,6 +22,12 @@
                            int M, int N, int K, int act, int in_dtype, int out_dtype, int shared, const float* ln_part,
                            const float* colsum, float ln_eps, float* part_out, const float* res_part, const float* res_gamma,
                            const float* res_beta, float res_eps, void* stream);
+
+int  gitmi_debug_gemm_kv_emit(const void* A, int lda, const void* W, const float* bias, void* C, int ldc, int M, int N, int K,
+                              int shared, const float* ln_part, const float* colsum, float ln_eps, void* kf, void* vt, int n_img,
+                              int H, int k_col0, void* stream);
+int  gitmi_debug_attention_cached(const void* qkv, const void* kf, const void* vt, void* out, int B, int N, int H, void* stream);
+int  gitmi_debug_read_kv_cache(gitmi_engine* e, int layer, void* kf_out, void* vt_out, int* emitted, void* stream);
 
 int  gitmi_debug_score_attn(const void* qkv, const void* img_kv, const int* image_of, void* out, int Q, int H, int N_img, int Lp,
                             int dtype, void* stream);
```
